# wasabipesto/nice

Hardware: AMD Instinct MI355X
Metric: numbers checked/sec per node, detailed+niceonly, 1e9 @ base 40 field (higher is better)
Workload: dtype u32; 1 GPU; extra-large: 1e+09 @ base 40, detailed + niceonly per step (benchmark.rs:60); base=40, field_start=1916284264916, field_size=1000000000, mode=both, niceonly_chunking=reference client (1e6 * clamp(ceil(size/1e11),1,1000)), parallelism=strong1, pipelined=True, pipeline_depth=2, full=False, probe_lib=False, gpu_max_hw_queues=4, gpu_max_hw_queues_exported=4

## Files before the change

### include/nice_hip.h

```cpp
#ifndef NICE_HIP_H
#define NICE_HIP_H

#include <stddef.h>
#include <stdint.h>

#ifdef __cplusplus
extern "C" {
#endif

#define NICE_OK 0
#define NICE_ERR_INVALID 1
#define NICE_ERR_HIP 2
#define NICE_ERR_CAPACITY 3
#define NICE_ERR_NO_DEVICE 4
#define NICE_ERR_MSD_OVERFLOW 5
#define NICE_ERR_BUSY 6

typedef struct {
    uint64_t number_lo;
    uint64_t number_hi;
    uint32_t num_uniques;
    uint32_t reserved;
} nice_number;

typedef struct nice_ctx nice_ctx;

int nice_ctx_create(const int *devices, int n_devices, nice_ctx **out);
void nice_ctx_destroy(nice_ctx *ctx);
int nice_ctx_synchronize(nice_ctx *ctx);
int nice_device_count(int *out);
const char *nice_last_error(void);

int nice_process_range_detailed(nice_ctx *ctx, uint64_t start_lo, uint64_t start_hi,
                                uint64_t end_lo, uint64_t end_hi, uint32_t base,
                                uint64_t *hist, nice_number *out, size_t cap, size_t *n_out);

#define NICE_FILTER_REFERENCE 0
#define NICE_FILTER_SOUND 1
#define NICE_MSD_FLOOR_ADAPTIVE UINT64_MAX
#define NICE_MSD_AUTO 0
#define NICE_MSD_HOST 1
#define NICE_MSD_DEVICE 2
typedef struct {
    uint64_t msd_floor;
    uint64_t chunk_size;
    int32_t threads;
    uint32_t stride_k;
    int32_t msd_where;
    uint32_t deal_stride;
    uint32_t deal_offset;
    uint32_t filter;
} nice_niceonly_opts;

typedef struct {
    uint64_t ranges;
    uint64_t range_numbers;
    uint64_t candidates;
    uint32_t launches;
    uint32_t square_ok;
    double msd_seconds;
    double total_seconds;
    uint64_t msd_floor;
    uint32_t msd_threads;
    uint32_t reruns;
} nice_niceonly_stats;

double nice_adaptive_floor_step(double floor, double msd_seconds, double total_seconds);
int nice_adaptive_floor(double *floor, uint32_t *warmup);

int nice_process_range_niceonly(nice_ctx *ctx, uint64_t start_lo, uint64_t start_hi,
                                uint64_t end_lo, uint64_t end_hi, uint32_t base,
                                nice_number *out, size_t cap, size_t *n_out);
int nice_process_range_niceonly_ex(nice_ctx *ctx, uint64_t start_lo, uint64_t start_hi,
                                   uint64_t end_lo, uint64_t end_hi, uint32_t base,
                                   const nice_niceonly_opts *opts, nice_number *out,
                                   size_t cap, size_t *n_out, nice_niceonly_stats *stats);
uint64_t nice_niceonly_prefix_rejected(void);

int nice_validate_detailed(uint32_t base, uint64_t size_lo, uint64_t size_hi, const uint64_t *hist,
                           const nice_number *list, size_t n);

int nice_cpu_process_range_detailed(uint64_t start_lo, uint64_t start_hi, uint64_t end_lo,
                                    uint64_t end_hi, uint32_t base, int32_t threads,
                                    uint64_t *hist, nice_number *out, size_t cap, size_t *n_out);
int nice_cpu_process_range_niceonly(uint64_t start_lo, uint64_t start_hi, uint64_t end_lo,
                                    uint64_t end_hi, uint32_t base, uint32_t stride_k,
                                    int32_t threads, nice_number *out, size_t cap, size_t *n_out);
int nice_cpu_process_range_niceonly_ex(uint64_t start_lo, uint64_t start_hi, uint64_t end_lo,
                                       uint64_t end_hi, uint32_t base, uint32_t stride_k,
                                       int32_t threads, uint32_t filter, nice_number *out, size_t cap,
                                       size_t *n_out);

int nice_detailed_submit(nice_ctx *ctx, uint64_t start_lo, uint64_t start_hi, uint64_t end_lo,
                         uint64_t end_hi, uint32_t base, int *ticket);
int nice_detailed_collect(nice_ctx *ctx, int ticket, uint64_t *hist, nice_number *out, size_t cap,
                          size_t *n_out);
int nice_niceonly_submit(nice_ctx *ctx, uint64_t start_lo, uint64_t start_hi, uint64_t end_lo,
                         uint64_t end_hi, uint32_t base, const nice_niceonly_opts *opts, int *ticket);
int nice_niceonly_collect(nice_ctx *ctx, int ticket, nice_number *out, size_t cap, size_t *n_out,
                          nice_niceonly_stats *stats);

typedef struct {
    double kernel_ms;
    uint32_t launches;
    uint32_t fd_kernel;
    uint64_t numbers;
    uint32_t sib_lanes;
    uint32_t sib_stride;
} nice_kernel_stats;
int nice_last_kernel_stats(nice_ctx *ctx, int device_index, nice_kernel_stats *out);
int nice_ctx_set_kernel_timing(nice_ctx *ctx, int enable);

uint32_t nice_host_threads(void);
int nice_debug_force_sib_stride(uint32_t L);
int nice_debug_fd_window(uint32_t base, uint32_t *w0, uint32_t *w);
int nice_debug_set_near_miss_cutoff(uint32_t base, uint32_t cutoff);
int nice_debug_set_nice_min(uint32_t base, uint32_t nice_min);
uint32_t nice_debug_cgroup_cpus(const char *root, const char *cgroup_path);
int nice_base_range(uint32_t base, uint64_t *start_lo, uint64_t *start_hi, uint64_t *end_lo,
                    uint64_t *end_hi);
uint32_t nice_near_miss_cutoff(uint32_t base);
uint64_t nice_gpu_batch_size(void);
uint64_t nice_processing_chunk_size(void);
int nice_gpu_supports_base(uint32_t base);
int nice_fd_kernel_base(uint32_t base);
int nice_niceonly_fast_base(uint32_t base);

int nice_msd_valid_ranges(uint64_t start_lo, uint64_t start_hi, uint64_t end_lo,
                          uint64_t end_hi, uint32_t base, uint64_t floor_size, uint64_t *out,
                          size_t cap, size_t *n_out);
int nice_msd_valid_ranges_ex(uint64_t start_lo, uint64_t start_hi, uint64_t end_lo,
                             uint64_t end_hi, uint32_t base, uint64_t floor_size, uint32_t filter,
                             uint64_t *out, size_t cap, size_t *n_out);
int nice_msd_skippable(uint64_t start_lo, uint64_t start_hi, uint64_t end_lo, uint64_t end_hi,
                       uint32_t base);
int nice_stride_table(uint32_t base, uint32_t k, uint64_t *modulus, uint32_t *residues,
                      size_t cap, size_t *n_out);

int nice_check_is_nice_inrange(uint32_t base, uint64_t n_lo, uint64_t n_hi);
int nice_check_unique_inrange(uint32_t base, uint64_t n_lo, uint64_t n_hi);
int nice_check_msd_skippable_inrange(uint32_t base, uint64_t start_lo, uint64_t start_hi,
                                     uint64_t end_lo, uint64_t end_hi);
int nice_check_prefix_reject_inrange(uint32_t base, uint64_t start_lo, uint64_t start_hi,
                                     uint64_t end_lo, uint64_t end_hi, uint64_t n_lo, uint64_t n_hi);
int nice_fd_segment_cuts(uint32_t base, uint64_t *out, size_t cap, size_t *n_out);

#define NICE_RANGES_PER_RANGE 0
#define NICE_RANGES_SUM 1
int nice_process_ranges_detailed(nice_ctx *ctx, uint32_t base, const uint64_t *bounds,
                                 size_t n_ranges, uint32_t flags, uint64_t *hist,
                                 nice_number *out, uint32_t *out_range, size_t cap,
                                 size_t *n_out);
typedef struct {
    uint32_t launches;
    uint32_t fallback_ranges;
    uint64_t numbers;
    double kernel_ms;
} nice_ranges_stats;
int nice_last_ranges_stats(nice_ctx *ctx, nice_ranges_stats *out);
int nice_cpu_process_ranges_detailed(uint32_t base, const uint64_t *bounds, size_t n_ranges,
                                     uint32_t flags, int32_t threads, uint64_t *hist,
                                     nice_number *out, uint32_t *out_range, size_t cap,
                                     size_t *n_out);
int nice_debug_ranges_plan(uint32_t base, const uint64_t *bounds, size_t n_ranges,
                           uint64_t *units, size_t cap, size_t *n_out);

int nice_debug_unique_counts(nice_ctx *ctx, const uint64_t *n_pairs, uint32_t count,
                             uint32_t base, uint32_t *out);
int nice_debug_is_nice(nice_ctx *ctx, const uint64_t *n_pairs, uint32_t count, uint32_t base,
                       uint32_t *out);
int nice_debug_unique_fast(nice_ctx *ctx, const uint64_t *n_pairs, uint32_t count, uint32_t base,
                           uint32_t *out);
int nice_debug_cube_count(nice_ctx *ctx, const uint64_t *n_pairs, uint32_t count, uint32_t base,
                          uint32_t *out);

#ifdef __cplusplus
}
#endif
#endif
```

### nice_amd/_lib.py

```python
from __future__ import annotations

import ctypes
import os
import subprocess

_HERE = os.path.dirname(os.path.abspath(__file__))
LIB_PATH = os.environ.get("NICE_LIB_PATH") or os.path.join(_HERE, "libnice_hip.so")

NICE_OK = 0
NICE_ERR_INVALID = 1
NICE_ERR_HIP = 2
NICE_ERR_CAPACITY = 3
NICE_ERR_NO_DEVICE = 4
NICE_ERR_MSD_OVERFLOW = 5
NICE_ERR_BUSY = 6
NICE_MSD_FLOOR_ADAPTIVE = (1 << 64) - 1
NICE_FILTER_REFERENCE = 0
NICE_FILTER_SOUND = 1
NICE_RANGES_PER_RANGE = 0
NICE_RANGES_SUM = 1

EXPORTS = (
    "nice_ctx_create", "nice_ctx_destroy", "nice_ctx_synchronize", "nice_device_count", "nice_last_error",
    "nice_process_range_detailed", "nice_process_range_niceonly",
    "nice_process_range_niceonly_ex", "nice_last_kernel_stats", "nice_base_range",
    "nice_near_miss_cutoff", "nice_gpu_batch_size", "nice_processing_chunk_size",
    "nice_gpu_supports_base", "nice_fd_kernel_base", "nice_niceonly_fast_base", "nice_msd_valid_ranges",
    "nice_msd_skippable", "nice_stride_table", "nice_debug_unique_counts",
    "nice_debug_is_nice", "nice_debug_unique_fast", "nice_check_is_nice_inrange", "nice_check_unique_inrange", "nice_check_msd_skippable_inrange",
    "nice_fd_segment_cuts", "nice_validate_detailed", "nice_detailed_submit",
    "nice_detailed_collect", "nice_niceonly_submit", "nice_niceonly_collect",
    "nice_cpu_process_range_detailed", "nice_cpu_process_range_niceonly",
    "nice_adaptive_floor_step", "nice_adaptive_floor", "nice_ctx_set_kernel_timing",
    "nice_host_threads", "nice_debug_cgroup_cpus", "nice_debug_force_sib_stride",
    "nice_niceonly_prefix_rejected", "nice_msd_valid_ranges_ex", "nice_cpu_process_range_niceonly_ex",
    "nice_check_prefix_reject_inrange",
    "nice_process_ranges_detailed", "nice_last_ranges_stats", "nice_cpu_process_ranges_detailed",
    "nice_debug_ranges_plan", "nice_debug_set_near_miss_cutoff", "nice_debug_fd_window",
    "nice_debug_set_nice_min", "nice_debug_cube_count",
)


class NiceLibraryError(RuntimeError):
    pass


class NiceError(RuntimeError):
    def __init__(self, code: int, msg: str):
        super().__init__(f"[{code}] {msg}")
        self.code = code


class nice_number(ctypes.Structure):
    _fields_ = [("number_lo", ctypes.c_uint64), ("number_hi", ctypes.c_uint64),
                ("num_uniques", ctypes.c_uint32), ("reserved", ctypes.c_uint32)]


class nice_niceonly_opts(ctypes.Structure):
    _fields_ = [("msd_floor", ctypes.c_uint64), ("chunk_size", ctypes.c_uint64),
                ("threads", ctypes.c_int32), ("stride_k", ctypes.c_uint32),
                ("msd_where", ctypes.c_int32), ("deal_stride", ctypes.c_uint32),
                ("deal_offset", ctypes.c_uint32), ("filter", ctypes.c_uint32)]


class nice_niceonly_stats(ctypes.Structure):
    _fields_ = [("ranges", ctypes.c_uint64), ("range_numbers", ctypes.c_uint64),
                ("candidates", ctypes.c_uint64), ("launches", ctypes.c_uint32),
                ("square_ok", ctypes.c_uint32), ("msd_seconds", ctypes.c_double),
                ("total_seconds", ctypes.c_double), ("msd_floor", ctypes.c_uint64),
                ("msd_threads", ctypes.c_uint32), ("reruns", ctypes.c_uint32)]


class nice_kernel_stats(ctypes.Structure):
    _fields_ = [("kernel_ms", ctypes.c_double), ("launches", ctypes.c_uint32),
                ("fd_kernel", ctypes.c_uint32), ("numbers", ctypes.c_uint64),
                ("sib_lanes", ctypes.c_uint32), ("sib_stride", ctypes.c_uint32)]


class nice_ranges_stats(ctypes.Structure):
    _fields_ = [("launches", ctypes.c_uint32), ("fallback_ranges", ctypes.c_uint32),
                ("numbers", ctypes.c_uint64), ("kernel_ms", ctypes.c_double)]


_lib = None


def build(force: bool = False) -> str:
    cmd = ["make", "-s", "-C", _HERE] + (["-B"] if force else [])
    subprocess.run(cmd, check=True)
    return LIB_PATH


def lib():
    global _lib
    if _lib is not None:
        return _lib
    if not os.path.exists(LIB_PATH):
        raise NiceLibraryError(
            f"{LIB_PATH} is missing: build it with `make -C nice_amd` "
            "(or __graft_entry__.build()); there is no CPU fallback")
    try:
        L = ctypes.CDLL(LIB_PATH)
    except OSError as e:
        raise NiceLibraryError(f"cannot load {LIB_PATH}: {e}") from e
    u64, u32, i32, sz = ctypes.c_uint64, ctypes.c_uint32, ctypes.c_int, ctypes.c_size_t
    P64, P32, PSZ = ctypes.POINTER(u64), ctypes.POINTER(u32), ctypes.POINTER(sz)
    PN = ctypes.POINTER(nice_number)
    vp = ctypes.c_void_p
    sig = {
        "nice_ctx_create": ([ctypes.POINTER(ctypes.c_int), i32, ctypes.POINTER(vp)], i32),
        "nice_ctx_destroy": ([vp], None),
        "nice_ctx_synchronize": ([vp], i32),
        "nice_device_count": ([ctypes.POINTER(ctypes.c_int)], i32),
        "nice_last_error": ([], ctypes.c_char_p),
        "nice_process_range_detailed": ([vp, u64, u64, u64, u64, u32, P64, PN, sz, PSZ], i32),
        "nice_process_range_niceonly": ([vp, u64, u64, u64, u64, u32, PN, sz, PSZ], i32),
        "nice_process_range_niceonly_ex": ([vp, u64, u64, u64, u64, u32,
                                            ctypes.POINTER(nice_niceonly_opts), PN, sz, PSZ,
                                            ctypes.POINTER(nice_niceonly_stats)], i32),
        "nice_last_kernel_stats": ([vp, i32, ctypes.POINTER(nice_kernel_stats)], i32),
        "nice_ctx_set_kernel_timing": ([vp, i32], i32),
        "nice_base_range": ([u32, P64, P64, P64, P64], i32),
        "nice_near_miss_cutoff": ([u32], u32),
        "nice_gpu_batch_size": ([], u64),
        "nice_processing_chunk_size": ([], u64),
        "nice_gpu_supports_base": ([u32], i32),
        "nice_fd_kernel_base": ([u32], i32),
        "nice_niceonly_fast_base": ([u32], i32),
        "nice_msd_valid_ranges": ([u64, u64, u64, u64, u32, u64, P64, sz, PSZ], i32),
        "nice_msd_valid_ranges_ex": ([u64, u64, u64, u64, u32, u64, u32, P64, sz, PSZ], i32),
        "nice_msd_skippable": ([u64, u64, u64, u64, u32], i32),
        "nice_stride_table": ([u32, u32, P64, P32, sz, PSZ], i32),
        "nice_debug_unique_counts": ([vp, P64, u32, u32, P32], i32),
        "nice_debug_is_nice": ([vp, P64, u32, u32, P32], i32),
        "nice_debug_unique_fast": ([vp, P64, u32, u32, P32], i32),
        "nice_check_is_nice_inrange": ([u32, u64, u64], i32),
        "nice_check_unique_inrange": ([u32, u64, u64], i32),
        "nice_check_msd_skippable_inrange": ([u32, u64, u64, u64, u64], i32),
        "nice_check_prefix_reject_inrange": ([u32, u64, u64, u64, u64, u64, u64], i32),
        "nice_fd_segment_cuts": ([u32, P64, sz, PSZ], i32),
        "nice_validate_detailed": ([u32, u64, u64, P64, PN, sz], i32),
        "nice_detailed_submit": ([vp, u64, u64, u64, u64, u32, ctypes.POINTER(i32)], i32),
        "nice_detailed_collect": ([vp, i32, P64, PN, sz, PSZ], i32),
        "nice_niceonly_submit": ([vp, u64, u64, u64, u64, u32, ctypes.POINTER(nice_niceonly_opts),
                                  ctypes.POINTER(i32)], i32),
        "nice_niceonly_collect": ([vp, i32, PN, sz, PSZ, ctypes.POINTER(nice_niceonly_stats)], i32),
        "nice_cpu_process_range_detailed": ([u64, u64, u64, u64, u32, i32, P64, PN, sz, PSZ], i32),
        "nice_cpu_process_range_niceonly": ([u64, u64, u64, u64, u32, u32, i32, PN, sz, PSZ], i32),
        "nice_cpu_process_range_niceonly_ex": ([u64, u64, u64, u64, u32, u32, i32, u32, PN, sz, PSZ], i32),
        "nice_niceonly_prefix_rejected": ([], u64),
        "nice_adaptive_floor_step": ([ctypes.c_double, ctypes.c_double, ctypes.c_double], ctypes.c_double),
        "nice_adaptive_floor": ([ctypes.POINTER(ctypes.c_double), P32], i32),
        "nice_host_threads": ([], u32),
        "nice_debug_cgroup_cpus": ([ctypes.c_char_p, ctypes.c_char_p], u32),
        "nice_debug_force_sib_stride": ([u32], i32),
        "nice_debug_set_near_miss_cutoff": ([u32, u32], i32),
        "nice_debug_fd_window": ([u32, P32, P32], i32),
        "nice_debug_set_nice_min": ([u32, u32], i32),
        "nice_debug_cube_count": ([vp, P64, u32, u32, P32], i32),
        "nice_process_ranges_detailed": ([vp, u32, P64, sz, u32, P64, PN, P32, sz, PSZ], i32),
        "nice_last_ranges_stats": ([vp, ctypes.POINTER(nice_ranges_stats)], i32),
        "nice_cpu_process_ranges_detailed": ([u32, P64, sz, u32, i32, P64, PN, P32, sz, PSZ], i32),
        "nice_debug_ranges_plan": ([u32, P64, sz, P64, sz, PSZ], i32),
    }
    for name, (args, res) in sig.items():
        fn = getattr(L, name)
        fn.argtypes = args
        fn.restype = res
    _lib = L
    return L


def check(rc: int):
    if rc != NICE_OK:
        msg = lib().nice_last_error()
        raise NiceError(rc, msg.decode() if msg else "")
```

### nice_amd/api.py

```python
from __future__ import annotations

import array
import ctypes
import threading
from dataclasses import dataclass
from typing import List, Optional, Sequence, Tuple

from . import _lib
from ._lib import check, lib
from .types import (DataToClient, DataToServer, FieldResults, FieldSize, NiceNumberSimple,
                    UniquesDistributionSimple)

CLIENT_VERSION = "3.2.15-mi355x"
MASK64 = (1 << 64) - 1


def _split(n: int):
    if n < 0 or n >> 128:
        raise ValueError("value must fit in u128")
    return n & MASK64, n >> 64


def _const(name):
    try:
        return int(getattr(lib(), name)())
    except _lib.NiceLibraryError:
        return None


GPU_BATCH_SIZE = 50_000_000
PROCESSING_CHUNK_SIZE = 1_000_000


def get_base_range_u128(base: int) -> Optional[FieldSize]:
    a, b, c, d = (ctypes.c_uint64() for _ in range(4))
    rc = lib().nice_base_range(base, a, b, c, d)
    if rc < 0:
        raise OverflowError(f"base {base}: range does not fit in u128")
    if rc == 0:
        return None
    return FieldSize(a.value | (b.value << 64), c.value | (d.value << 64))


def get_near_miss_cutoff(base: int) -> int:
    return int(lib().nice_near_miss_cutoff(base))


def gpu_supports_base(base: int) -> bool:
    return bool(lib().nice_gpu_supports_base(base))


def niceonly_fast_base(base: int) -> bool:
    return bool(lib().nice_niceonly_fast_base(base))


@dataclass
class StrideTable:
    base: int
    k: int
    modulus: int
    valid_residues: List[int]

    @classmethod
    def new(cls, base: int, k: int) -> "StrideTable":
        m = ctypes.c_uint64()
        n = ctypes.c_size_t()
        check(lib().nice_stride_table(base, k, m, None, 0, n))
        buf = (ctypes.c_uint32 * max(n.value, 1))()
        check(lib().nice_stride_table(base, k, m, buf, n.value, n))
        return cls(base, k, m.value, list(buf[: n.value]))


def get_valid_ranges(range_: FieldSize, base: int, floor_size: int = 250,
                     filter: str = "reference") -> List[FieldSize]:
    s, e = range_.range_start, range_.range_end
    f = _FILTERS[filter]
    n = ctypes.c_size_t()
    rc = lib().nice_msd_valid_ranges_ex(*_split(s), *_split(e), base, floor_size, f, None, 0, n)
    if rc not in (_lib.NICE_OK, _lib.NICE_ERR_CAPACITY):
        check(rc)
    buf = (ctypes.c_uint64 * (4 * max(n.value, 1)))()
    check(lib().nice_msd_valid_ranges_ex(*_split(s), *_split(e), base, floor_size, f, buf, n.value, n))
    return [FieldSize(buf[4 * i] | (buf[4 * i + 1] << 64), buf[4 * i + 2] | (buf[4 * i + 3] << 64))
            for i in range(n.value)]


def has_duplicate_msd_prefix(range_: FieldSize, base: int) -> bool:
    rc = lib().nice_msd_skippable(*_split(range_.range_start), *_split(range_.range_end), base)
    if rc < 0 or rc > 1:
        check(rc)
    return bool(rc)


@dataclass
class NiceonlyStats:
    ranges: int
    range_numbers: int
    candidates: int
    launches: int
    msd_seconds: float
    total_seconds: float
    square_ok: int = 0
    msd_floor: int = 0
    msd_threads: int = 0
    reruns: int = 0
    prefix_rejected: int = 0


_FILTERS = {"reference": _lib.NICE_FILTER_REFERENCE, "sound": _lib.NICE_FILTER_SOUND}


def _stats(st) -> NiceonlyStats:
    return NiceonlyStats(st.ranges, st.range_numbers, st.candidates, st.launches,
                         st.msd_seconds, st.total_seconds, st.square_ok, st.msd_floor,
                         st.msd_threads, st.reruns, int(lib().nice_niceonly_prefix_rejected()))


def host_threads() -> int:
    return int(lib().nice_host_threads())


def adaptive_floor_step(floor: float, msd_seconds: float, total_seconds: float) -> float:
    return lib().nice_adaptive_floor_step(floor, msd_seconds, total_seconds)


def adaptive_floor() -> Tuple[float, int]:
    f, w = ctypes.c_double(), ctypes.c_uint32()
    check(lib().nice_adaptive_floor(f, w))
    return f.value, w.value


@dataclass
class KernelStats:
    kernel_ms: float
    launches: int
    fd_kernel: bool
    numbers: int
    sib_lanes: int = 0
    sib_stride: int = 0


@dataclass
class RangesStats:
    launches: int
    fallback_ranges: int
    numbers: int
    kernel_ms: float


def _pack_ranges(ranges):
    pairs = [(r.range_start, r.range_end) if isinstance(r, FieldSize) else (int(r[0]), int(r[1]))
             for r in ranges]
    if any(s < 0 or e < 0 or s >> 128 or e >> 128 for s, e in pairs):
        raise ValueError("value must fit in u128")
    flat = array.array("Q", [x for s, e in pairs for x in (s & MASK64, s >> 64, e & MASK64, e >> 64)])
    if not pairs:
        flat = array.array("Q", [0, 0, 0, 0])
    return (ctypes.c_uint64 * len(flat)).from_buffer_copy(flat), len(pairs)


def _ranges_result(hist, nb, nrows, out, idx, n):
    full = memoryview(hist).cast("B").cast("Q").tolist()
    rows = [full[i * nb:(i + 1) * nb] for i in range(nrows)]
    return rows, [(out[i].number_lo | (out[i].number_hi << 64), out[i].num_uniques, idx[i])
                  for i in range(n)]


class GpuContext:

    def __init__(self, devices: Sequence[int] | int = 0):
        if isinstance(devices, int):
            devices = [devices]
        arr = (ctypes.c_int * len(devices))(*devices)
        h = ctypes.c_void_p()
        check(lib().nice_ctx_create(arr, len(devices), ctypes.byref(h)))
        self._h = h
        self.devices = list(devices)
        self._out = None
        self._out_cap = 0
        self._hist = {}

    @classmethod
    def new(cls, device_ordinal: int = 0) -> "GpuContext":
        return cls([device_ordinal])

    def close(self):
        if getattr(self, "_h", None):
            lib().nice_ctx_destroy(self._h)
            self._h = None

    def synchronize(self):
        check(lib().nice_ctx_synchronize(self._h))

    def __del__(self):
        try:
            self.close()
        except Exception:
            pass

    def _out_buf(self, cap):
        if cap > self._out_cap:
            self._out = (_lib.nice_number * cap)()
            self._out_cap = cap
        return self._out

    def set_kernel_timing(self, enable: bool):
        check(lib().nice_ctx_set_kernel_timing(self._h, 1 if enable else 0))

    def kernel_stats(self, device_index: int = 0) -> KernelStats:
        s = _lib.nice_kernel_stats()
        check(lib().nice_last_kernel_stats(self._h, device_index, s))
        return KernelStats(s.kernel_ms, s.launches, bool(s.fd_kernel), s.numbers, s.sib_lanes, s.sib_stride)

    def detailed_raw(self, start: int, end: int, base: int, cap: int = 0):
        hist = self._hist.get(base)
        if hist is None:
            hist = self._hist[base] = (ctypes.c_uint64 * (base + 1))()
        cap = max(cap, self._out_cap, 1024)
        while True:
            out = self._out_buf(cap)
            n = ctypes.c_size_t()
            rc = lib().nice_process_range_detailed(self._h, *_split(start), *_split(end), base,
                                                   hist, out, cap, n)
            if rc == _lib.NICE_ERR_CAPACITY and n.value > cap:
                cap = n.value
                continue
            check(rc)
            lst = [(out[i].number_lo | (out[i].number_hi << 64), out[i].num_uniques)
                   for i in range(n.value)]
            return list(hist), lst

    def detailed_submit(self, start: int, end: int, base: int) -> int:
        t = ctypes.c_int()
        check(lib().nice_detailed_submit(self._h, *_split(start), *_split(end), base, t))
        return t.value

    def detailed_collect(self, ticket: int, base: int, cap: int = 0):
        hist = self._hist.get(base)
        if hist is None:
            hist = self._hist[base] = (ctypes.c_uint64 * (base + 1))()
        cap = max(cap, self._out_cap, 1024)
        while True:
            out = self._out_buf(cap)
            n = ctypes.c_size_t()
            rc = lib().nice_detailed_collect(self._h, ticket, hist, out, cap, n)
            if rc == _lib.NICE_ERR_CAPACITY and n.value > cap:
                cap = n.value
                continue
            check(rc)
            return list(hist), [(out[i].number_lo | (out[i].number_hi << 64), out[i].num_uniques)
                                for i in range(n.value)]

    def detailed_ranges(self, ranges, base: int, sum: bool = False, cap: int = 0):
        bounds, n_ranges = _pack_ranges(ranges)
        nb = base + 1
        hist = (ctypes.c_uint64 * (nb * (1 if sum else max(n_ranges, 1))))()
        flags = _lib.NICE_RANGES_SUM if sum else _lib.NICE_RANGES_PER_RANGE
        cap = max(cap, 1024)
        while True:
            out, idx, n = _cpu_out(cap), (ctypes.c_uint32 * cap)(), ctypes.c_size_t()
            rc = lib().nice_process_ranges_detailed(self._h, base, bounds, n_ranges, flags, hist, out, idx,
                                                    cap, n)
            if rc == _lib.NICE_ERR_CAPACITY and n.value > cap:
                cap = n.value
                continue
            check(rc)
            return _ranges_result(hist, nb, 1 if sum else n_ranges, out, idx, n.value)

    def ranges_stats(self) -> "RangesStats":
        s = _lib.nice_ranges_stats()
        check(lib().nice_last_ranges_stats(self._h, s))
        return RangesStats(s.launches, s.fallback_ranges, s.numbers, s.kernel_ms)

    def niceonly_raw(self, start: int, end: int, base: int, msd_floor: int = 0,
                     chunk_size: int = 0, threads: int = 0, stride_k: int = 0,
                     msd_where: str = "auto", cap: int = 0, deal_stride: int = 0,
                     deal_offset: int = 0, filter: str = "reference"):
        opts = self._nice_opts(msd_floor, chunk_size, threads, stride_k, msd_where, deal_stride,
                               deal_offset, filter)
        st = _lib.nice_niceonly_stats()
        cap = max(cap, self._out_cap, 1024)
        while True:
            out = self._out_buf(cap)
            n = ctypes.c_size_t()
            rc = lib().nice_process_range_niceonly_ex(self._h, *_split(start), *_split(end), base,
                                                      opts, out, cap, n, st)
            if rc == _lib.NICE_ERR_CAPACITY and n.value > cap:
                cap = n.value
                continue
            check(rc)
            lst = [out[i].number_lo | (out[i].number_hi << 64) for i in range(n.value)]
            return lst, _stats(st)

    @staticmethod
    def _nice_opts(msd_floor=0, chunk_size=0, threads=0, stride_k=0, msd_where="auto",
                   deal_stride=0, deal_offset=0, filter="reference"):
        where = {"auto": 0, "host": 1, "device": 2}[msd_where]
        if filter not in _FILTERS:
            raise ValueError(f"filter must be one of {sorted(_FILTERS)}")
        if msd_floor == "adaptive":
            msd_floor = _lib.NICE_MSD_FLOOR_ADAPTIVE
        return _lib.nice_niceonly_opts(msd_floor, chunk_size, threads, stride_k, where,
                                       deal_stride, deal_offset, _FILTERS[filter])

    def niceonly_submit(self, start: int, end: int, base: int, **opts) -> int:
        t = ctypes.c_int()
        check(lib().nice_niceonly_submit(self._h, *_split(start), *_split(end), base,
                                         self._nice_opts(**opts), t))
        return t.value

    def niceonly_collect(self, ticket: int, cap: int = 0):
        st = _lib.nice_niceonly_stats()
        cap = max(cap, self._out_cap, 1024)
        while True:
            out = self._out_buf(cap)
            n = ctypes.c_size_t()
            rc = lib().nice_niceonly_collect(self._h, ticket, out, cap, n, st)
            if rc == _lib.NICE_ERR_CAPACITY and n.value > cap:
                cap = n.value
                continue
            check(rc)
            return ([out[i].number_lo | (out[i].number_hi << 64) for i in range(n.value)],
                    _stats(st))

    def both_raw(self, det_range, nice_range, base: int, **nice_opts):
        det = self.detailed_raw(*det_range, base) if det_range else (None, [])
        nice = self.niceonly_raw(*nice_range, base, **nice_opts) if nice_range else ([], None)
        return det, nice

    def debug_unique_counts(self, ns: Sequence[int], base: int) -> List[int]:
        arr = (ctypes.c_uint64 * (2 * max(len(ns), 1)))()
        for i, n in enumerate(ns):
            arr[2 * i], arr[2 * i + 1] = _split(n)
        out = (ctypes.c_uint32 * max(len(ns), 1))()
        check(lib().nice_debug_unique_counts(self._h, arr, len(ns), base, out))
        return list(out[: len(ns)])

    def debug_unique_fast(self, ns: Sequence[int], base: int) -> List[int]:
        arr = (ctypes.c_uint64 * (2 * max(len(ns), 1)))()
        for i, n in enumerate(ns):
            arr[2 * i], arr[2 * i + 1] = _split(n)
        out = (ctypes.c_uint32 * max(len(ns), 1))()
        check(lib().nice_debug_unique_fast(self._h, arr, len(ns), base, out))
        return list(out[: len(ns)])

    def debug_cube_count(self, ns: Sequence[int], base: int) -> List[int]:
        arr = (ctypes.c_uint64 * (2 * max(len(ns), 1)))()
        for i, n in enumerate(ns):
            arr[2 * i], arr[2 * i + 1] = _split(n)
        out = (ctypes.c_uint32 * max(len(ns), 1))()
        check(lib().nice_debug_cube_count(self._h, arr, len(ns), base, out))
        return list(out[: len(ns)])

    def debug_is_nice(self, ns: Sequence[int], base: int) -> List[bool]:
        arr = (ctypes.c_uint64 * (2 * max(len(ns), 1)))()
        for i, n in enumerate(ns):
            arr[2 * i], arr[2 * i + 1] = _split(n)
        out = (ctypes.c_uint32 * max(len(ns), 1))()
        check(lib().nice_debug_is_nice(self._h, arr, len(ns), base, out))
        return [bool(x) for x in out[: len(ns)]]


class BothModes:

    def __init__(self, device: int = 0, det_ctx: Optional[GpuContext] = None,
                 nice_ctx: Optional[GpuContext] = None):
        self.det = det_ctx if det_ctx is not None else GpuContext([device])
        self.nice = nice_ctx if nice_ctx is not None else GpuContext([device])
        self._own_nice = nice_ctx is None
        self._go = threading.Event()
        self._done = threading.Event()
        self._job = None
        self._res = None
        self._closed = False
        self._thread = threading.Thread(target=self._serve, name="nice-niceonly", daemon=True)
        self._thread.start()

    def _serve(self):
        while True:
            self._go.wait()
            self._go.clear()
            if self._closed:
                return
            args, kw = self._job
            try:
                self._res = (True, self.nice.niceonly_raw(*args, **kw))
            except BaseException as e:
                self._res = (False, e)
            self._done.set()

    def kernel_stats(self, device_index: int = 0) -> KernelStats:
        return self.det.kernel_stats(device_index)

    def detailed_raw(self, *a, **kw):
        return self.det.detailed_raw(*a, **kw)

    def niceonly_raw(self, *a, **kw):
        return self.nice.niceonly_raw(*a, **kw)

    def both_raw(self, det_range, nice_range, base: int, **nice_opts):
        if self._closed:
            raise RuntimeError("BothModes is closed")
        if not nice_range:
            return (self.det.detailed_raw(*det_range, base) if det_range else (None, [])), ([], None)
        self._job = ((*nice_range, base), nice_opts)
        self._done.clear()
        self._go.set()
        try:
            det = self.det.detailed_raw(*det_range, base) if det_range else (None, [])
        finally:
            self._done.wait()
        ok, nice = self._res
        self._res = None
        if not ok:
            raise nice
        return det, nice

    def close(self):
        if not self._closed:
            self._closed = True
            self._go.set()
            self._thread.join()
            if self._own_nice:
                self.nice.close()


def process_range_detailed_gpu(ctx: GpuContext, range_: FieldSize, base: int) -> FieldResults:
    hist, lst = ctx.detailed_raw(range_.range_start, range_.range_end, base)
    return FieldResults(
        distribution=[UniquesDistributionSimple(i, hist[i]) for i in range(1, base + 1)],
        nice_numbers=[NiceNumberSimple(n, u) for n, u in lst])


def process_range_niceonly_gpu(ctx: GpuContext, range_: FieldSize, base: int,
                               **opts) -> FieldResults:
    lst, _ = ctx.niceonly_raw(range_.range_start, range_.range_end, base, **opts)
    return FieldResults(distribution=[], nice_numbers=[NiceNumberSimple(n, base) for n in lst])


def process_detailed_gpu(ctx: GpuContext, claim: DataToClient, username: str) -> DataToServer:
    r = process_range_detailed_gpu(ctx, claim.field(), claim.base)
    return DataToServer(claim.claim_id, username, CLIENT_VERSION, r.distribution, r.nice_numbers)


def process_niceonly_gpu(ctx: GpuContext, claim: DataToClient, username: str) -> DataToServer:
    r = process_range_niceonly_gpu(ctx, claim.field(), claim.base)
    return DataToServer(claim.claim_id, username, CLIENT_VERSION, None, r.nice_numbers)


_default_ctx: Optional[GpuContext] = None
_default_lock = threading.Lock()


def default_context() -> GpuContext:
    global _default_ctx
    with _default_lock:
        if _default_ctx is None:
            _default_ctx = GpuContext(0)
        return _default_ctx


def process_range_detailed(range_: FieldSize, base: int) -> FieldResults:
    return process_range_detailed_gpu(default_context(), range_, base)


def process_range_niceonly(range_: FieldSize, base: int,
                           stride_table: Optional[StrideTable] = None) -> FieldResults:
    k = stride_table.k if stride_table is not None else 2
    size = range_.range_size
    return process_range_niceonly_gpu(default_context(), range_, base, stride_k=k,
                                      chunk_size=min(size, (1 << 64) - 1))


def _cpu_out(cap: int):
    return (_lib.nice_number * max(cap, 1))()


def process_range_detailed_cpu(range_: FieldSize, base: int, threads: int = 1) -> FieldResults:
    hist = (ctypes.c_uint64 * (base + 1))()
    cap = 1024
    while True:
        out, n = _cpu_out(cap), ctypes.c_size_t()
        rc = lib().nice_cpu_process_range_detailed(*_split(range_.range_start), *_split(range_.range_end),
                                                    base, threads, hist, out, cap, n)
        if rc == _lib.NICE_ERR_CAPACITY and n.value > cap:
            cap = n.value
            continue
        check(rc)
        break
    return FieldResults(
        distribution=[UniquesDistributionSimple(i, hist[i]) for i in range(1, base + 1)],
        nice_numbers=[NiceNumberSimple(out[i].number_lo | (out[i].number_hi << 64), out[i].num_uniques)
                      for i in range(n.value)])


def detailed_ranges_cpu(ranges, base: int, sum: bool = False, threads: int = 1):
    bounds, n_ranges = _pack_ranges(ranges)
    nb = base + 1
    hist = (ctypes.c_uint64 * (nb * (1 if sum else max(n_ranges, 1))))()
    flags = _lib.NICE_RANGES_SUM if sum else _lib.NICE_RANGES_PER_RANGE
    cap = 1024
    while True:
        out, idx, n = _cpu_out(cap), (ctypes.c_uint32 * cap)(), ctypes.c_size_t()
        rc = lib().nice_cpu_process_ranges_detailed(base, bounds, n_ranges, flags, threads, hist, out, idx,
                                                     cap, n)
        if rc == _lib.NICE_ERR_CAPACITY and n.value > cap:
            cap = n.value
            continue
        check(rc)
        return _ranges_result(hist, nb, 1 if sum else n_ranges, out, idx, n.value)


def _ranges_field_results(rows, lst, base: int) -> List[FieldResults]:
    per = [[] for _ in rows]
    for n, u, i in lst:
        per[i].append(NiceNumberSimple(n, u))
    return [FieldResults(distribution=[UniquesDistributionSimple(i, row[i]) for i in range(1, base + 1)],
                         nice_numbers=nn) for row, nn in zip(rows, per)]


def process_ranges_detailed_gpu(ctx: GpuContext, ranges, base: int) -> List[FieldResults]:
    return _ranges_field_results(*ctx.detailed_ranges(ranges, base), base)


def process_ranges_detailed_cpu(ranges, base: int, threads: int = 1) -> List[FieldResults]:
    return _ranges_field_results(*detailed_ranges_cpu(ranges, base, threads=threads), base)


def process_range_niceonly_cpu(range_: FieldSize, base: int,
                               stride_table: Optional[StrideTable] = None,
                               threads: int = 1, filter: str = "reference") -> FieldResults:
    k = stride_table.k if stride_table is not None else 2
    cap = 256
    while True:
        out, n = _cpu_out(cap), ctypes.c_size_t()
        rc = lib().nice_cpu_process_range_niceonly_ex(*_split(range_.range_start), *_split(range_.range_end),
                                                       base, k, threads, _FILTERS[filter], out, cap, n)
        if rc == _lib.NICE_ERR_CAPACITY and n.value > cap:
            cap = n.value
            continue
        check(rc)
        break
    return FieldResults(distribution=[], nice_numbers=[
        NiceNumberSimple(out[i].number_lo | (out[i].number_hi << 64), base) for i in range(n.value)])
```

### nice_amd/csrc/abi_detailed.cpp

```cpp
#include <cstring>

#include "abi_internal.hpp"

using namespace nice::abi;
using nice::u128;

namespace {

inline bool spin_wait() { return nice::probe_knob("NICE_SPIN", 1) != 0; }

int enqueue_detailed(Device &d, Slot &sl, u128 s, u128 e, uint32_t base, bool *finished) {
    nice::DetailedLaunch p{};
    p.base = base;
    p.cutoff = effective_cutoff(base);
    p.hist = sl.d_state;
    p.out = nice::NumOut{sl.det.n, sl.det.u, sl.d_count, sl.det.cap};
    p.launches = &sl.launches;
    p.sib = sl.sib;
    for (const Slot &o : d.slot)
        if (&o != &sl && o.inflight) p.overlapped = 1;
    *finished = false;
    uint32_t tag = 0;
    auto launch = [&](u128 a, u128 b, bool fd) -> int {
        if (a >= b) return NICE_OK;
        u128 cnt = b - a;
        while (cnt) {
            uint64_t c = cnt > ((u128)1 << 62) ? (1ull << 62) : (uint64_t)cnt;
            p.start_lo = lo64(a);
            p.start_hi = hi64(a);
            p.count = c;
            const bool last = a + c == e;
            p.fin = last && fd ? nice::FieldFinish{sl.d_fin, sl.d_done, sl.seq, tag}
                               : nice::FieldFinish{nullptr, nullptr, 0, 0};
            if (nice::probe_set("NICE_FD2_NOFIN")) p.fin = nice::FieldFinish{nullptr, nullptr, 0, 0};
            hipError_t err = fd ? nice::launch_detailed_fd2(p, d.num_cus, sl.stream)
                                : nice::launch_detailed_generic(p, d.num_cus, sl.stream);
            if (!fd) sl.launches++;
            if (err != hipSuccess)
                return fail(NICE_ERR_HIP, std::string("detailed launch: ") + hipGetErrorString(err));
            if (last) {
                *finished = fd && p.fin.out_mapped;
                sl.tag = *finished ? p.fin.tag : 0u;
                sl.tag_words = base + 1;
            }
            a += c;
            cnt -= c;
        }
        return NICE_OK;
    };
    u128 rs = 0, re = 0;
    const bool fd_base = nice::fd2_supported(base);
    const bool fd = fd_base && nice::base_range_cached(base, rs, re) == 1;
    const bool small_fd = fd && s >= rs && e <= re && e - s < 20000000;
    p.hist_copies = small_fd ? 16 : nice::kHistCopies;
    if (small_fd && !nice::probe_set("NICE_FD2_UNTAGGED")) tag = (uint32_t)sl.seq | 0x80000000u;
    sl.tag = 0;
    if (!fd) return launch(s, e, false);
    int rc;
    if ((rc = launch(s, std::min(e, rs), false))) return rc;
    if ((rc = launch(std::max(s, rs), std::min(e, re), true))) return rc;
    return launch(std::max(s, re), e, false);
}

bool published(const Slot &sl) {
    if (!sl.tag) return __atomic_load_n(&sl.h_fin[nice::kFinSeq], __ATOMIC_ACQUIRE) == sl.seq;
    if ((uint32_t)(__atomic_load_n(&sl.h_fin[nice::kFinCount], __ATOMIC_ACQUIRE) >> 32) != sl.tag) return false;
    for (uint32_t b = 0; b < sl.tag_words; b++)
        if ((uint32_t)(__atomic_load_n(&sl.h_fin[b], __ATOMIC_ACQUIRE) >> 32) != sl.tag) return false;
    return true;
}

int wait_field(Slot &sl) {
    if (!sl.fin_seq || !spin_wait()) {
        const hipError_t q = field_sync(sl);
        if (q != hipSuccess) return fail(NICE_ERR_HIP, std::string("detailed field: ") + hipGetErrorString(q));
        return NICE_OK;
    }
    for (uint32_t i = 1;; i++) {
        if (published(sl)) return NICE_OK;
        if ((i & 4095) == 0 || i > kSpinPolls) {
            const hipError_t q = field_query(sl);
            if (q == hipSuccess) {
                if (published(sl)) return NICE_OK;
                return fail(NICE_ERR_HIP, "detailed field completed without publishing its results");
            }
            if (q != hipErrorNotReady) return fail(NICE_ERR_HIP, std::string("detailed field: ") + hipGetErrorString(q));
        }
        backoff(i);
    }
}

int enqueue_detailed_shard(Device &d, Slot &sl, u128 s, u128 e, uint32_t base, bool timing) {
    HIPCHK(hipSetDevice(d.id));
    if (d.stats_slot == (int)(&sl - d.slot)) {
        int rc = resolve_stats(d);
        if (rc) return rc;
    }
    sl.seq++;
    sl.launches = 0;
    sl.sib[0] = sl.sib[1] = 0;
    if (sl.dirty) HIPCHK(hipMemsetAsync(sl.d_state, 0, kStateBytes, sl.stream));
    sl.dirty = true;
    sl.timed = timing;
    sl.marked = false;
    if (timing) HIPCHK(hipEventRecord(sl.ev0, sl.stream));
    bool finished = false;
    int rc = enqueue_detailed(d, sl, s, e, base, &finished);
    if (rc) return rc;
    sl.inflight = true;
    if (timing) HIPCHK(hipEventRecord(sl.ev1, sl.stream));
    sl.fin_seq = finished;
    if (!finished) {
        HIPCHK(nice::launch_detailed_finish(sl.d_state, sl.d_count, sl.d_fin, sl.stream));
        HIPCHK(hipEventRecord(sl.ev_done, sl.stream));
    } else if (!timing && !sl.own_stream) {
        HIPCHK(hipEventRecord(sl.ev_done, sl.stream));
        sl.marked = true;
    }
    return NICE_OK;
}

int detailed_submit(nice_ctx *ctx, std::unique_lock<std::mutex> &lock, u128 s, u128 e, uint32_t base,
                    bool wait, int *ticket) {
    int t = -1;
    if (int rc = acquire_slot(ctx, lock, ctx->det, ctx->det_next, wait, "detailed", &t)) return rc;
    DetJob &job = ctx->det[t];
    const size_t nd = ctx->devs.size();
    const u128 size = e - s;
    job.bounds.assign(nd + 1, 0);
    for (size_t i = 0; i <= nd; i++) job.bounds[i] = s + size / nd * i + std::min<u128>(i, size % nd);
    for (size_t i = 0; i < nd; i++) {
        if (job.bounds[i] >= job.bounds[i + 1]) continue;
        int rc = enqueue_detailed_shard(ctx->devs[i], ctx->devs[i].slot[t], job.bounds[i], job.bounds[i + 1], base,
                                        ctx->timing);
        if (rc) return rc;
    }
    job.active = true;
    job.collected = false;
    job.owner = std::this_thread::get_id();
    job.s = s;
    job.e = e;
    job.base = base;
    ctx->det_next = (t + 1) % slots_used();
    *ticket = t;
    return NICE_OK;
}

int detailed_submit_args(nice_ctx *ctx, uint64_t start_lo, uint64_t start_hi, uint64_t end_lo, uint64_t end_hi,
                         uint32_t base, bool wait, int *ticket) {
    if (!ctx || !ticket) return fail(NICE_ERR_INVALID, "null argument");
    if (base < 2 || base > 128) return fail(NICE_ERR_INVALID, "base must be in 2..=128");
    const u128 s = mk(start_lo, start_hi), e = mk(end_lo, end_hi);
    if (s >= e)
        return fail(NICE_ERR_INVALID, "Range has invalid bounds, range_start must be < range_end");
    std::unique_lock<std::mutex> lock(ctx->mu);
    return detailed_submit(ctx, lock, s, e, base, wait, ticket);
}

uint32_t shard_finished(Device &d, Slot &sl, int t) {
    sl.dirty = false;
    sl.inflight = false;
    d.stats_slot = t;
    d.last.launches = sl.launches;
    d.last.sib_lanes = sl.sib[0];
    d.last.sib_stride = sl.sib[1];
    return (uint32_t)sl.h_fin[nice::kFinCount];
}

int recompute_listed(nice_ctx *ctx, const DetJob &job, const std::vector<size_t> &off) {
    const size_t nd = ctx->devs.size();
    std::vector<std::vector<uint32_t>> u(nd);
    std::vector<std::vector<uint64_t>> pairs(nd);
    struct Drain {
        nice_ctx *ctx;
        std::vector<char> q;
        ~Drain() {
            for (size_t j = 0; j < q.size(); j++)
                if (q[j]) {
                    (void)hipSetDevice(ctx->devs[j].id);
                    (void)hipStreamSynchronize(ctx->devs[j].aux);
                }
        }
    } drain{ctx, std::vector<char>(nd, 0)};
    for (size_t i = 0; i < nd; i++) {
        const size_t n = off[i + 1] - off[i];
        if (!n) continue;
        Device &d = ctx->devs[i];
        HIPCHK(hipSetDevice(d.id));
        if (!d.aux) HIPCHK(hipStreamCreateWithFlags(&d.aux, hipStreamNonBlocking));
        pairs[i].resize(2 * n);
        for (size_t q = 0; q < n; q++) {
            pairs[i][2 * q] = lo64(job.all[off[i] + q].n);
            pairs[i][2 * q + 1] = hi64(job.all[off[i] + q].n);
        }
        if (d.chk_cap < n) {
            const size_t c = std::max<size_t>(n, 4096);
            if (int rc = grow_device(d.chk_n, d.chk_cap, c, c * 16)) return rc;
            if (int rc = grow_device(d.chk_u, d.chk_cap, c, c * 4)) return rc;
        }
        u[i].resize(n);
        drain.q[i] = 1;
        hipError_t err = hipMemcpyAsync(d.chk_n, pairs[i].data(), n * 16, hipMemcpyHostToDevice, d.aux);
        if (err == hipSuccess) err = nice::launch_unique_counts(d.chk_n, (uint32_t)n, job.base, d.chk_u, d.aux);
        if (err == hipSuccess) err = hipMemcpyAsync(u[i].data(), d.chk_u, n * 4, hipMemcpyDeviceToHost, d.aux);
        if (err != hipSuccess) return fail(NICE_ERR_HIP, std::string("self-check: ") + hipGetErrorString(err));
    }
    for (size_t i = 0; i < nd; i++) {
        if (u[i].empty()) continue;
        Device &d = ctx->devs[i];
        HIPCHK(hipSetDevice(d.id));
        const hipError_t err = hipStreamSynchronize(d.aux);
        drain.q[i] = 0;
        if (err != hipSuccess) return fail(NICE_ERR_HIP, std::string("self-check: ") + hipGetErrorString(err));
        for (size_t q = 0; q < u[i].size(); q++)
            if (u[i][q] != job.all[off[i] + q].u)
                return fail(NICE_ERR_HIP, "self-check: unique count of a listed number does not recompute");
    }
    return NICE_OK;
}

int detailed_gather(nice_ctx *ctx, DetJob &job, int t) {
    const uint32_t base = job.base;
    const size_t nd = ctx->devs.size();
    job.total.assign(base + 1, 0);
    job.all.clear();
    std::vector<size_t> off(nd + 1, 0);
    for (size_t i = 0; i < nd; i++) {
        off[i] = job.all.size();
        Device &d = ctx->devs[i];
        Slot &sl = d.slot[t];
        d.last = nice_kernel_stats{};
        d.stats_slot = -1;
        if (job.bounds[i] >= job.bounds[i + 1]) continue;
        HIPCHK(hipSetDevice(d.id));
        int rc = wait_field(sl);
        if (rc) return rc;
        d.last.numbers = (uint64_t)(job.bounds[i + 1] - job.bounds[i]);
        d.last.fd_kernel = nice::fd2_supported(base) ? 1u : 0u;
        uint32_t cnt = shard_finished(d, sl, t);
        if (cnt > sl.det.cap) {
            rc = ensure_listbuf(d, sl.det, cnt, true);
            if (!rc) rc = enqueue_detailed_shard(d, sl, job.bounds[i], job.bounds[i + 1], base, sl.timed);
            if (!rc) rc = wait_field(sl);
            if (rc) return rc;
            cnt = shard_finished(d, sl, t);
            if (cnt > sl.det.cap) return fail(NICE_ERR_HIP, "near-miss list overflow after resize");
        }
        for (uint32_t b = 0; b <= base; b++) job.total[b] += sl.tag ? (uint32_t)sl.h_fin[b] : sl.h_fin[b];
        if (cnt) {
            HIPCHK(field_sync(sl));
            std::vector<uint64_t> nbuf((size_t)cnt * 2);
            std::vector<uint32_t> ubuf(cnt);
            HIPCHK(hipMemcpy(nbuf.data(), sl.det.n, (size_t)cnt * 16, hipMemcpyDeviceToHost));
            HIPCHK(hipMemcpy(ubuf.data(), sl.det.u, (size_t)cnt * 4, hipMemcpyDeviceToHost));
            for (uint32_t q = 0; q < cnt; q++) job.all.push_back({mk(nbuf[2 * q], nbuf[2 * q + 1]), ubuf[q]});
        }
    }
    off[nd] = job.all.size();
    int rc = validate_detailed(base, effective_cutoff(base), job.e - job.s, job.total.data(), job.all.size(),
                               [&](size_t i) { return job.all[i]; });
    if (!rc && !job.all.empty()) rc = recompute_listed(ctx, job, off);
    if (rc) return rc;
    std::sort(job.all.begin(), job.all.end(), [](const Entry &a, const Entry &b) { return a.n < b.n; });
    return NICE_OK;
}

void detailed_drop(nice_ctx *ctx, int t) {
    ctx->det[t].active = false;
    for (auto &d : ctx->devs) d.slot[t].dirty = true, d.slot[t].inflight = false;
}

int detailed_collect(nice_ctx *ctx, int t, uint64_t *hist, nice_number *out, size_t cap, size_t *n_out) {
    if (t < 0 || t >= kSlots || !ctx->det[t].active)
        return fail(NICE_ERR_INVALID, "no detailed field in flight under this ticket");
    DetJob &job = ctx->det[t];
    if (!job.collected) {
        int rc = detailed_gather(ctx, job, t);
        if (rc) {
            detailed_drop(ctx, t);
            return rc;
        }
        job.collected = true;
    }
    std::memcpy(hist, job.total.data(), (job.base + 1) * 8);
    int rc = emit_list(job.all, out, cap, n_out);
    if (rc == NICE_ERR_CAPACITY) return rc;
    job.active = false;
    job.all = {};
    return rc;
}

int detailed_collect_locked(nice_ctx *ctx, int ticket, uint64_t *hist, nice_number *out, size_t cap,
                            size_t *n_out) {
    std::unique_lock<std::mutex> lock(ctx->mu);
    if (ticket < 0 || ticket >= kSlots || !ctx->det[ticket].active)
        return fail(NICE_ERR_INVALID, "no detailed field in flight under this ticket");
    DetJob &job = ctx->det[ticket];
    if (job.waiting) return fail(NICE_ERR_INVALID, "another thread is collecting this detailed field");
    if (!job.collected) {
        job.waiting = true;
        lock.unlock();
        int rc = NICE_OK;
        for (size_t i = 0; i < ctx->devs.size() && !rc; i++) {
            if (job.bounds[i] >= job.bounds[i + 1]) continue;
            const hipError_t err = hipSetDevice(ctx->devs[i].id);
            rc = err != hipSuccess ? fail(NICE_ERR_HIP, hipGetErrorString(err)) : wait_field(ctx->devs[i].slot[ticket]);
        }
        lock.lock();
        job.waiting = false;
        if (rc) {
            detailed_drop(ctx, ticket);
            return rc;
        }
    }
    return detailed_collect(ctx, ticket, hist, out, cap, n_out);
}

}

extern "C" {

int nice_detailed_submit(nice_ctx *ctx, uint64_t start_lo, uint64_t start_hi, uint64_t end_lo,
                         uint64_t end_hi, uint32_t base, int *ticket) {
    return detailed_submit_args(ctx, start_lo, start_hi, end_lo, end_hi, base, false, ticket);
}

int nice_detailed_collect(nice_ctx *ctx, int ticket, uint64_t *hist, nice_number *out, size_t cap,
                          size_t *n_out) {
    if (!ctx || !hist) return fail(NICE_ERR_INVALID, "null argument");
    const int rc = detailed_collect_locked(ctx, ticket, hist, out, cap, n_out);
    ctx->freed.notify_all();
    return rc;
}

int nice_process_range_detailed(nice_ctx *ctx, uint64_t start_lo, uint64_t start_hi,
                                uint64_t end_lo, uint64_t end_hi, uint32_t base, uint64_t *hist,
                                nice_number *out, size_t cap, size_t *n_out) {
    int t = -1;
    int rc = detailed_submit_args(ctx, start_lo, start_hi, end_lo, end_hi, base, true, &t);
    if (rc) return rc;
    rc = nice_detailed_collect(ctx, t, hist, out, cap, n_out);
    if (rc == NICE_ERR_CAPACITY) {
        {
            std::lock_guard<std::mutex> lock(ctx->mu);
            ctx->det[t].active = false;
            ctx->det[t].all = {};
        }
        ctx->freed.notify_all();
    }
    return rc;
}

}
```

### nice_amd/csrc/abi_hooks.cpp

```cpp
#include "abi_internal.hpp"
#include "niceonly_bases.h"
#include "radix_fast.hpp"

using namespace nice::abi;
using nice::u128;

namespace {

#define NICE_FAST_BASES(X) NICE_NICEONLY_BASES(X)

bool fast_base_range(uint32_t base, u128 &rs, u128 &re) {
    return nice::niceonly_fast_base(base) && nice::base_range_cached(base, rs, re) == 1;
}

template <int B>
int prefix_reject_host(u128 s, u128 l, u128 n) {
    constexpr int MW = nice::Radix<B>::MW;
    uint32_t pm[MW] = {}, low[MW];
    const uint32_t multi = l > s ? 1u : 0u;
    if (multi && nice::msd_prefix_masks<B>(lo64(s), hi64(s), lo64(l), hi64(l), pm))
        for (int w = 0; w < MW; w++) pm[w] = ~0u;
    const uint32_t dup = nice::low_digit_mask(B, (uint32_t)(n % ((uint32_t)B * B)), low, MW);
    return nice::prefix_rejects<MW>(pm, multi, low, dup) ? 1 : 0;
}

template <class Launch>
int debug_per_n(nice_ctx *ctx, const uint64_t *n_pairs, uint32_t count, uint32_t *out, Launch launch) {
    if (count == 0) return NICE_OK;
    Device &d = ctx->devs[0];
    HIPCHK(hipSetDevice(d.id));
    uint64_t *dn;
    uint32_t *du;
    HIPCHK(hipMalloc(&dn, (size_t)count * 16));
    HIPCHK(hipMalloc(&du, (size_t)count * 4));
    HIPCHK(hipMemcpy(dn, n_pairs, (size_t)count * 16, hipMemcpyHostToDevice));
    HIPCHK(launch(dn, du, d.slot[0].stream));
    HIPCHK(hipStreamSynchronize(d.slot[0].stream));
    HIPCHK(hipMemcpy(out, du, (size_t)count * 4, hipMemcpyDeviceToHost));
    HIPCHK(hipFree(dn));
    HIPCHK(hipFree(du));
    return NICE_OK;
}

}

extern "C" {

int nice_validate_detailed(uint32_t base, uint64_t size_lo, uint64_t size_hi, const uint64_t *hist,
                           const nice_number *list, size_t n) {
    if (base < 2 || base > 128 || !hist || (n && !list)) return fail(NICE_ERR_INVALID, "bad args");
    const int rc = validate_detailed(base, nice::near_miss_cutoff(base), mk(size_lo, size_hi), hist, n, [&](size_t i) {
        return Entry{mk(list[i].number_lo, list[i].number_hi), list[i].num_uniques};
    });
    return rc ? NICE_ERR_INVALID : NICE_OK;
}

int nice_debug_unique_counts(nice_ctx *ctx, const uint64_t *n_pairs, uint32_t count,
                             uint32_t base, uint32_t *out) {
    if (!ctx || base < 2 || base > 128) return fail(NICE_ERR_INVALID, "bad args");
    return debug_per_n(ctx, n_pairs, count, out, [&](const uint64_t *dn, uint32_t *du, hipStream_t s) {
        return nice::launch_unique_counts(dn, count, base, du, s);
    });
}

int nice_debug_is_nice(nice_ctx *ctx, const uint64_t *n_pairs, uint32_t count, uint32_t base,
                       uint32_t *out) {
    if (!ctx || base < 2 || base > 128) return fail(NICE_ERR_INVALID, "bad args");
    return debug_per_n(ctx, n_pairs, count, out, [&](const uint64_t *dn, uint32_t *du, hipStream_t s) {
        return nice::launch_is_nice(dn, count, base, du, s);
    });
}

int nice_debug_unique_fast(nice_ctx *ctx, const uint64_t *n_pairs, uint32_t count, uint32_t base,
                           uint32_t *out) {
    u128 rs, re;
    if (!ctx || !fast_base_range(base, rs, re))
        return fail(NICE_ERR_INVALID, "base without a niceonly fast path");
    for (uint32_t i = 0; i < count; i++) {
        const u128 n = mk(n_pairs[2 * i], n_pairs[2 * i + 1]);
        if (n < rs || n >= re) return fail(NICE_ERR_INVALID, "n outside the base's valid range");
    }
    return debug_per_n(ctx, n_pairs, count, out, [&](const uint64_t *dn, uint32_t *du, hipStream_t s) {
        return nice::launch_unique_fast(dn, count, base, du, s);
    });
}

int nice_debug_cube_count(nice_ctx *ctx, const uint64_t *n_pairs, uint32_t count, uint32_t base,
                          uint32_t *out) {
    u128 rs, re;
    if (!ctx || !fast_base_range(base, rs, re))
        return fail(NICE_ERR_INVALID, "base without a niceonly fast path");
    for (uint32_t i = 0; i < count; i++) {
        const u128 n = mk(n_pairs[2 * i], n_pairs[2 * i + 1]);
        if (n < rs || n >= re) return fail(NICE_ERR_INVALID, "n outside the base's valid range");
    }
    return debug_per_n(ctx, n_pairs, count, out, [&](const uint64_t *dn, uint32_t *du, hipStream_t s) {
        return nice::launch_cube_count(dn, count, base, du, s);
    });
}

int nice_check_is_nice_inrange(uint32_t base, uint64_t lo, uint64_t hi) {
    u128 rs, re;
    const u128 n = mk(lo, hi);
    if (!fast_base_range(base, rs, re) || n < rs || n >= re)
        return fail(NICE_ERR_INVALID, "n outside the base's valid range (or base without a niceonly fast path)");
    switch (base) {
#define X(b) case b: return nice::is_nice_fast<b>(lo, hi) ? 1 : 0;
        NICE_FAST_BASES(X)
#undef X
    default: return NICE_ERR_INVALID;
    }
}

int nice_check_unique_inrange(uint32_t base, uint64_t lo, uint64_t hi) {
    u128 rs, re;
    const u128 n = mk(lo, hi);
    if (!fast_base_range(base, rs, re) || n < rs || n >= re)
        return fail(NICE_ERR_INVALID, "n outside the base's valid range (or base without a niceonly fast path)");
    switch (base) {
#define X(b) case b: return (int)nice::unique_fast<b>(lo, hi);
        NICE_FAST_BASES(X)
#undef X
    default: return NICE_ERR_INVALID;
    }
}

int nice_check_msd_skippable_inrange(uint32_t base, uint64_t slo, uint64_t shi, uint64_t elo,
                                     uint64_t ehi) {
    u128 rs, re;
    const u128 s = mk(slo, shi), e = mk(elo, ehi);
    if (!fast_base_range(base, rs, re) || s < rs || e > re || s >= e)
        return fail(NICE_ERR_INVALID, "range outside the base's valid range (or base without a niceonly fast path)");
    if (e - s == 1) return 0;
    const u128 l = e - 1;
    const uint64_t llo = lo64(l), lhi = hi64(l);
    switch (base) {
#define X(b) case b: return nice::msd_skippable_fast<b>(slo, shi, llo, lhi) ? 1 : 0;
        NICE_FAST_BASES(X)
#undef X
    default: return NICE_ERR_INVALID;
    }
}

int nice_check_prefix_reject_inrange(uint32_t base, uint64_t slo, uint64_t shi, uint64_t elo, uint64_t ehi,
                                     uint64_t nlo, uint64_t nhi) {
    u128 rs, re;
    const u128 s = mk(slo, shi), e = mk(elo, ehi), n = mk(nlo, nhi);
    if (!fast_base_range(base, rs, re) || s < rs || e > re || n < s || n >= e)
        return fail(NICE_ERR_INVALID, "leaf or n outside the base's valid range (or base without a niceonly fast path)");
    switch (base) {
#define X(b) case b: return prefix_reject_host<b>(s, e - 1, n);
        NICE_FAST_BASES(X)
#undef X
    default: return NICE_ERR_INVALID;
    }
}

int nice_fd_segment_cuts(uint32_t base, uint64_t *out, size_t cap, size_t *n_out) {
    std::vector<u128> c(8);
    const size_t n = nice::fd2_cuts(base, c.data(), c.size());
    for (size_t i = 0; i < n && i < cap; i++) {
        out[2 * i] = lo64(c[i]);
        out[2 * i + 1] = hi64(c[i]);
    }
    if (n_out) *n_out = n;
    return NICE_OK;
}

int nice_msd_skippable(uint64_t slo, uint64_t shi, uint64_t elo, uint64_t ehi, uint32_t base) {
    if (base < 2 || base > 128 || mk(slo, shi) >= mk(elo, ehi)) return fail(NICE_ERR_INVALID, "bad args");
    return nice::make_msd(base)->skippable(mk(slo, shi), mk(elo, ehi)) ? 1 : 0;
}

int nice_msd_valid_ranges(uint64_t slo, uint64_t shi, uint64_t elo, uint64_t ehi, uint32_t base,
                          uint64_t floor_size, uint64_t *out, size_t cap, size_t *n_out) {
    return nice_msd_valid_ranges_ex(slo, shi, elo, ehi, base, floor_size, NICE_FILTER_REFERENCE, out, cap, n_out);
}

int nice_msd_valid_ranges_ex(uint64_t slo, uint64_t shi, uint64_t elo, uint64_t ehi, uint32_t base,
                             uint64_t floor_size, uint32_t filter, uint64_t *out, size_t cap, size_t *n_out) {
    if (base < 2 || base > 128 || mk(slo, shi) >= mk(elo, ehi) || filter > NICE_FILTER_SOUND)
        return fail(NICE_ERR_INVALID, "bad args");
    std::vector<std::pair<u128, u128>> rs;
    nice::make_msd(base)->ranges(mk(slo, shi), mk(elo, ehi), floor_size, rs, filter == NICE_FILTER_SOUND);
    size_t n = rs.size();
    for (size_t i = 0; i < n && i < cap; i++) {
        out[4 * i] = lo64(rs[i].first);
        out[4 * i + 1] = hi64(rs[i].first);
        out[4 * i + 2] = lo64(rs[i].second);
        out[4 * i + 3] = hi64(rs[i].second);
    }
    *n_out = n;
    return n > cap ? fail(NICE_ERR_CAPACITY, "range list exceeds capacity") : NICE_OK;
}

int nice_stride_table(uint32_t base, uint32_t k, uint64_t *modulus, uint32_t *residues,
                      size_t cap, size_t *n_out) {
    if (base < 3 || base > 128 || k > 3) return fail(NICE_ERR_INVALID, "bad args");
    auto t = g_stride.get(base, k);
    *modulus = t->modulus;
    *n_out = t->residues.size();
    for (size_t i = 0; i < std::min(cap, t->residues.size()); i++) residues[i] = t->residues[i];
    return t->residues.size() > cap && residues ? fail(NICE_ERR_CAPACITY, "capacity") : NICE_OK;
}

int nice_debug_force_sib_stride(uint32_t L) {
    if (L && (L % 2 == 0 || L > 255))
        return fail(NICE_ERR_INVALID, "sibling lane stride must be odd and <= 255 (0: the production pick)");
    nice::fd2_force_sib_stride(L);
    return NICE_OK;
}

int nice_debug_fd_window(uint32_t base, uint32_t *w0, uint32_t *w) {
    if (!w0 || !w) return fail(NICE_ERR_INVALID, "null argument");
    if (!nice::fd2_window(base, w0, w)) return fail(NICE_ERR_INVALID, "base has no FD kernel");
    return NICE_OK;
}

int nice_debug_set_near_miss_cutoff(uint32_t base, uint32_t cutoff) {
    uint32_t w0 = 0, w = 0;
    if (!nice::fd2_window(base, &w0, &w)) return fail(NICE_ERR_INVALID, "base has no FD kernel");
    if (cutoff && (cutoff + 1 < w0 + w || cutoff >= base))
        return fail(NICE_ERR_INVALID, "cutoff must be 0 (production) or in [" + std::to_string(w0 + w - 1) + ", " +
                                          std::to_string(base - 1) + "]");
    g_cutoff_override[base].store(cutoff, std::memory_order_relaxed);
    return NICE_OK;
}

int nice_debug_set_nice_min(uint32_t base, uint32_t nice_min) {
    if (!nice::niceonly_fast_base(base)) return fail(NICE_ERR_INVALID, "base without a niceonly fast path");
    if (nice_min > base)
        return fail(NICE_ERR_INVALID, "nice_min must be 0 (production) or in [1, " + std::to_string(base) + "]");
    g_nice_min_override[base].store(nice_min, std::memory_order_relaxed);
    return NICE_OK;
}

}
```

### nice_amd/csrc/abi_internal.hpp

```cpp
#pragma once

#include <hip/hip_runtime.h>
#include <sched.h>

#include <algorithm>
#include <atomic>
#include <chrono>
#include <condition_variable>
#include <map>
#include <memory>
#include <mutex>
#include <string>
#include <thread>
#include <vector>

#include "../../include/nice_hip.h"
#include "host_math.hpp"
#include "host_parallel.hpp"
#include "kernels.h"
#include "probe.hpp"

namespace nice {
namespace abi __attribute__((visibility("hidden"))) {

constexpr size_t kStateBytes = (size_t)kHistCopies * kHistBins * 8 + (1 + kDoneWords) * 4;
constexpr int kSlots = 3;

constexpr uint32_t kInitialListCap = 1u << 20;
constexpr uint32_t kNiceCap = 1u << 16;

inline int slots_used() { return std::max(1, std::min(kSlots, (int)probe_knob("NICE_SLOTS", kSlots))); }

int fail(int code, const std::string &msg);

#define HIPCHK(expr)                                                                    \
    do {                                                                                \
        hipError_t e_ = (expr);                                                         \
        if (e_ != hipSuccess)                                                           \
            return fail(NICE_ERR_HIP, std::string(#expr) + ": " + hipGetErrorString(e_)); \
    } while (0)

inline u128 mk(uint64_t lo, uint64_t hi) { return ((u128)hi << 64) | lo; }
inline uint64_t lo64(u128 v) { return (uint64_t)v; }
inline uint64_t hi64(u128 v) { return (uint64_t)(v >> 64); }

struct LeafBuf {
    Leaf *h = nullptr, *d = nullptr;
    uint32_t cap = 0;
    hipEvent_t done = nullptr;
    bool pending = false;
};

struct MsdBuf {
    MsdNode *q[2] = {nullptr, nullptr};
    ChunkNode *scratch = nullptr;
    void *wscratch = nullptr;
    size_t wscratch_bytes = 0;
    Leaf *leaves = nullptr;
    LeafMask *leaf_masks = nullptr;
    uint32_t *counters = nullptr;
    uint32_t q_cap = 0, leaf_cap = 0, mask_cap = 0;
    uint64_t scratch_nodes = 0;
    bool dirty = true;
};

struct ListBuf {
    uint64_t *n = nullptr;
    uint32_t *u = nullptr;
    uint32_t cap = 0;
};

struct Slot {
    hipStream_t stream = nullptr;
    bool own_stream = false, own_nstream = false;
    hipStream_t nstream = nullptr;
    uint64_t *d_state = nullptr;
    uint32_t *d_count = nullptr;
    uint32_t *d_done = nullptr;
    uint32_t *d_nice_count = nullptr;
    uint64_t *h_fin = nullptr;
    uint64_t *d_fin = nullptr;
    ListBuf det, nice;
    hipEvent_t ev0 = nullptr, ev1 = nullptr, ev_done = nullptr, nice_done = nullptr;
    hipEvent_t nt0 = nullptr, nt1 = nullptr;
    uint32_t *h_msd = nullptr;
    uint32_t *h_nice = nullptr;
    uint32_t *d_msd_mapped = nullptr, *d_nice_mapped = nullptr;
    uint32_t *d_nice_done = nullptr;
    bool dirty = true;
    bool inflight = false;
    bool timed = false;
    bool marked = false;
    uint64_t seq = 0;
    uint32_t launches = 0;
    uint32_t sib[2] = {0, 0};
    bool fin_seq = false;
    uint32_t tag = 0;
    uint32_t tag_words = 0;
    MsdBuf msd;
};

struct Device {
    int id = 0;
    int num_cus = 0;
    hipStream_t aux = nullptr;
    uint64_t *chk_n = nullptr;
    uint32_t *chk_u = nullptr;
    size_t chk_cap = 0;
    Slot slot[kSlots];
    std::map<uint32_t, uint32_t *> residues;
    std::map<uint32_t, uint32_t *> ranks;
    std::map<uint32_t, uint32_t *> lowtabs;
    LeafBuf desc[2];
    int desc_next = 0;
    nice_kernel_stats last{};
    int stats_slot = -1;
};

struct Entry {
    u128 n;
    uint32_t u;
};

struct DetJob {
    bool active = false, collected = false;
    bool waiting = false;
    std::thread::id owner;
    u128 s = 0, e = 0;
    uint32_t base = 0;
    std::vector<u128> bounds;
    std::vector<uint64_t> total;
    std::vector<Entry> all;
};
struct NiceJob {
    bool active = false, collected = false;
    bool waiting = false;
    std::thread::id owner;
    u128 s = 0, e = 0;
    uint32_t base = 0;
    nice_niceonly_opts opts{};
    bool has_opts = false;
    bool on_device = false;
    bool empty = false;
    std::vector<char> used;
    nice_niceonly_stats st{};
    std::chrono::steady_clock::time_point t0;
    std::vector<Entry> all;
    bool adapt = false;
    uint32_t reruns = 0;
    uint64_t rejected = 0;
    uint32_t nice_min = 0;
};

struct RangesDev {
    hipStream_t stream = nullptr;
    void *h_desc = nullptr, *d_desc = nullptr;
    size_t desc_cap = 0;
    uint64_t *d_rows = nullptr;
    size_t rows_cap = 0;
    uint32_t *d_count = nullptr;
    ListBuf list;
    uint32_t *chk_u = nullptr;
    uint32_t chk_cap = 0;
    hipEvent_t ev0 = nullptr, ev1 = nullptr;
};
struct RangesState {
    std::vector<RangesDev> dev;
    nice_ranges_stats stats{};
    bool kept = false;
    uint32_t base = 0, flags = 0;
    std::vector<uint64_t> bounds, hist;
    std::vector<Entry> list;
    std::vector<uint32_t> list_range;
};

}
}

struct nice_ctx {
    std::mutex ranges_mu;
    nice::abi::RangesState ranges;
    std::vector<nice::abi::Device> devs;
    std::mutex mu;
    std::condition_variable freed;
    bool timing = true;
    nice::abi::DetJob det[nice::abi::kSlots];
    nice::abi::NiceJob nice[nice::abi::kSlots];
    int det_next = 0, nice_next = 0;
    std::vector<std::thread::id> blocked;
};

namespace nice {
namespace abi __attribute__((visibility("hidden"))) {

template <class Job>
int free_slot(const Job *jobs, int next) {
    const int n = slots_used();
    for (int i = 0; i < n; i++) {
        const int t = (next + i) % n;
        if (!jobs[t].active) return t;
    }
    return -1;
}

template <class Job>
int acquire_slot(nice_ctx *ctx, std::unique_lock<std::mutex> &lock, const Job *jobs, int next, bool wait,
                 const char *mode, int *slot) {
    const std::thread::id me = std::this_thread::get_id();
    auto blocked = [&](std::thread::id id) {
        return id == me || std::find(ctx->blocked.begin(), ctx->blocked.end(), id) != ctx->blocked.end();
    };
    auto unblock = [&] {
        auto it = std::find(ctx->blocked.begin(), ctx->blocked.end(), me);
        if (it != ctx->blocked.end()) {
            ctx->blocked.erase(it);
            ctx->freed.notify_all();
        }
    };
    for (;;) {
        const int t = free_slot(jobs, next);
        if (t >= 0) {
            unblock();
            *slot = t;
            return NICE_OK;
        }
        bool freeable = false;
        for (int i = 0; i < slots_used(); i++)
            freeable |= jobs[i].active && (jobs[i].waiting || !blocked(jobs[i].owner));
        if (!wait || !freeable) {
            unblock();
            return fail(NICE_ERR_BUSY, std::string("three ") + mode +
                                           " fields already in flight on this context; collect one first");
        }
        if (std::find(ctx->blocked.begin(), ctx->blocked.end(), me) == ctx->blocked.end()) {
            ctx->blocked.push_back(me);
            ctx->freed.notify_all();
        }
        ctx->freed.wait(lock);
    }
}

template <class T, class C>
int grow_device(T *&p, C &cap, C new_cap, size_t bytes, hipStream_t drain = nullptr) {
    if (drain) HIPCHK(hipStreamSynchronize(drain));
    if (p) HIPCHK(hipFree(p));
    p = nullptr;
    cap = 0;
    HIPCHK(hipMalloc(&p, bytes));
    cap = new_cap;
    return NICE_OK;
}
template <class T, class C>
int grow_pinned(T *&p, C &cap, C new_cap, size_t bytes) {
    if (p) HIPCHK(hipHostFree(p));
    p = nullptr;
    cap = 0;
    HIPCHK(hipHostMalloc(&p, bytes, hipHostMallocDefault));
    cap = new_cap;
    return NICE_OK;
}

int ensure_listbuf(Device &d, ListBuf &l, uint32_t cap, bool with_u);

inline void put_entry(nice_number &o, const Entry &e) {
    o.number_lo = lo64(e.n);
    o.number_hi = hi64(e.n);
    o.num_uniques = e.u;
    o.reserved = 0;
}

int emit_list(std::vector<Entry> &all, nice_number *out, size_t cap, size_t *n_out);

inline std::atomic<uint32_t> g_cutoff_override[129];

inline uint32_t effective_cutoff(uint32_t base) {
    const uint32_t c = base <= 128 ? g_cutoff_override[base].load(std::memory_order_relaxed) : 0u;
    return c ? c : near_miss_cutoff(base);
}

inline std::atomic<uint32_t> g_nice_min_override[129];

template <class Get>
int validate_detailed(uint32_t base, uint32_t cutoff, u128 size, const uint64_t *hist, size_t n, Get get) {
    u128 sum = 0;
    for (uint32_t b = 0; b <= base; b++) sum += hist[b];
    if (sum != size)
        return fail(NICE_ERR_HIP, "self-check: distribution total does not equal the field size");
    std::vector<uint64_t> per(base + 1, 0);
    for (size_t i = 0; i < n; i++) {
        const uint32_t u = get(i).u;
        if (u <= cutoff || u > base)
            return fail(NICE_ERR_HIP, "self-check: listed number " + std::to_string(i) +
                                          " has num_uniques " + std::to_string(u) +
                                          " at or below the cutoff");
        per[u]++;
    }
    u128 above = 0;
    for (uint32_t u = cutoff + 1; u <= base; u++) {
        if (per[u] != hist[u])
            return fail(NICE_ERR_HIP, "self-check: " + std::to_string(per[u]) +
                                          " listed numbers with " + std::to_string(u) +
                                          " uniques, distribution claims " + std::to_string(hist[u]));
        above += hist[u];
    }
    if (above != (u128)n) return fail(NICE_ERR_HIP, "self-check: list length does not match the distribution");
    return NICE_OK;
}

struct StrideCache {
    std::mutex mu;
    std::map<std::pair<uint32_t, uint32_t>, std::shared_ptr<StrideTable>> tables;
    std::shared_ptr<StrideTable> get(uint32_t base, uint32_t k) {
        std::lock_guard<std::mutex> g(mu);
        auto key = std::make_pair(base, k);
        auto it = tables.find(key);
        if (it != tables.end()) return it->second;
        auto t = std::make_shared<StrideTable>(base, k);
        tables[key] = t;
        return t;
    }
};
inline StrideCache g_stride;

constexpr uint32_t kSpinPolls = 1u << 14, kYieldPolls = 1u << 11;

inline void backoff(uint32_t i) {
    if (i < kSpinPolls) {
        __builtin_ia32_pause();
    } else if (i < kSpinPolls + kYieldPolls) {
        sched_yield();
    } else {
        const uint32_t k = std::min<uint32_t>((i - kSpinPolls - kYieldPolls) / 8, 3);
        std::this_thread::sleep_for(std::chrono::microseconds(std::min(200u, 20u << (2 * k))));
    }
}

inline hipError_t sync_event(hipEvent_t ev) {
    for (uint32_t i = 0;; i++) {
        const hipError_t q = hipEventQuery(ev);
        if (q != hipErrorNotReady) return q;
        backoff(i);
    }
}

inline hipEvent_t done_event(const Slot &sl) {
    if (!sl.fin_seq) return sl.ev_done;
    return sl.timed ? sl.ev1 : (sl.marked ? sl.ev_done : nullptr);
}

inline hipError_t field_query(const Slot &sl) {
    const hipEvent_t ev = done_event(sl);
    return ev ? hipEventQuery(ev) : hipStreamQuery(sl.stream);
}

inline hipError_t field_sync(const Slot &sl) {
    for (uint32_t i = 0;; i++) {
        const hipError_t q = field_query(sl);
        if (q != hipErrorNotReady) return q;
        backoff(i);
    }
}

int resolve_stats(Device &d);

void ranges_dev_free(Device &d, RangesDev &r);

}
}
```

### nice_amd/csrc/fd2_cfg.hpp

```cpp
#pragma once

#include <algorithm>
#include <type_traits>

#include "layout.h"

namespace nice {
namespace fd2 {

constexpr int log2ceil(unsigned v) { int t = 0; while ((1u << t) < v) t++; return t; }
constexpr int ilog2(unsigned v) { int t = 0; while ((2u << t) <= v) t++; return t; }

constexpr bool split_exact(unsigned base, unsigned es, unsigned long long m) {
    for (unsigned v = 0; v < base * base; v++)
        if (((unsigned long long)es * v * m) >> 32 != v / base) return false;
    return true;
}


constexpr int window_w(int b) {
    return b == 40 ? 15 : b == 50 ? 18 : b == 80 ? 28 : b <= 45 ? 15 : b <= 61 ? 18 : b <= 70 ? 20 : 28;
}
constexpr int window_w0(int b) {
    switch (b) {
    case 40: return 18;
    case 42: return 19;
    case 43: return 20;
    case 44: case 45: case 47: return 21;
    case 48: return 22;
    case 49: return 23;
    case 50: return 21;
    case 52: return 24;
    case 53: return 25;
    case 54: case 55: return 26;
    case 57: return 27;
    case 58: return 28;
    case 59: case 60: return 29;
    case 62: case 63: return 30;
    case 64: return 31;
    case 65: return 32;
    case 67: return 33;
    case 68: return 34;
    case 80: return 33;
    default: return b * 61 / 100 - window_w(b) / 2;
    }
}

struct Digits {
    int d2, d3, dn;
};
constexpr Digits digits_of(int base) {
    const int k = base / 5, r5 = base % 5;
    return Digits{r5 == 0 ? 2 * k : (r5 == 4 ? 2 * k + 2 : 2 * k + 1),
                  r5 == 0 ? 3 * k : (r5 == 2 ? 3 * k + 1 : 3 * k + 2), r5 == 0 ? k : k + 1};
}

constexpr int tchunk_of(int base) { return base <= 45 ? 80 : (base <= 58 ? 160 : 240); }

constexpr int state_regs(int base) {
    const Digits d = digits_of(base);
    return (d.d2 + 1) / 2 + (d.d3 + 1) / 2 + 2 * ((d.dn + 1) / 2) + 1 + (base + 31) / 32;
}
constexpr int state_waves(int base) {
    const int r = state_regs(base);
    return r <= 31 ? 8 : (r <= 38 ? 6 : (r <= 46 ? 5 : 4));
}

constexpr bool fits64(unsigned base, int digits) {
    unsigned long long v = 1;
    for (int i = 0; i < digits; i++) {
        if (v > ~0ull / base) return false;
        v *= base;
    }
    return true;
}

constexpr int valu_limbs(int base) {
    switch (base) {
    case 43: case 44: case 45: case 48: case 50: case 54: case 55: return 1;
    case 53: case 58: case 65: return 2;
    case 67: case 68: case 80: return 256;
    case 59: case 63: case 64: return 1024 + 2;
    case 60: return 1024 + 17;
    case 62: return 1024 + 1;
    default: return 0;
    }
}

constexpr int valu_limbs_big(int base, int nd, int ne) {
    if (base == 40) return ne == 8 ? 2048 | 1 : 0;
    if (base == 50 || base == 53 || base == 60) return valu_limbs(base) | 2048;
    if ((base + 31) / 32 != 3) return valu_limbs(base);
    if (base == 80 && ne == 17) return 256 | 2048 | 4;
    return 256 | 2048 | 3;
}

constexpr int lds_bytes(int base, int wg) {
    const int mw = (base + 31) / 32, b2 = base * base;
    const bool split = mw == 3 && (valu_limbs(base) & 512) != 0;
    const int es = mw == 1 ? 4 : (mw == 2 || split ? 8 : 16);
    int t = 0;
    while ((1 << t) < b2) t++;
    const int ebt = es * ((1 << t) - b2);
    if (split) {
        const int a = (4 * (base + 1) + 15) / 16 * 16, h = (ebt / 2 + 15) / 16 * 16;
        const int t2 = a > h ? a : h;
        const int tb0 = (t2 + 4 * b2 + 15) / 16 * 16, tbe = (ebt + 15) / 16 * 16;
        const int tb = tb0 > tbe ? tb0 : tbe;
        return (tb + b2 * es + 15) / 16 * 16 + window_w(base) * (wg / 2) * 4;
    }
    const int tb0 = (window_w(base) * (wg / 2) * 4 + 4 * (base + 1) + 15) / 16 * 16;
    const int tb = tb0 >= ebt ? tb0 : (ebt + 15) / 16 * 16;
    const int db = base - 32;
    const bool lsd_w1 = mw == 2 && db > 0 && db + (db > 20 ? 4 : 10) <= 30;
    const bool lsdx = mw == 2 && db > 0 && !lsd_w1 && (valu_limbs(base) & 1024) != 0;
    return tb + (b2 * es + 15) / 16 * 16 + (lsd_w1 || lsdx ? (2 * b2 * es + 15) / 16 * 16 : 0) +
           (lsdx ? (2 * b2 + 15) / 16 * 16 : 0);
}
constexpr int waves_at(int base, int wg) {
    const int lds = (163840 / lds_bytes(base, wg)) * (wg / 64) / 4;
    const int cap = lds < state_waves(base) ? lds : state_waves(base);
    return cap / (wg / 256) * (wg / 256);
}
constexpr int rounds_wg(int base) { return waves_at(base, 1024) > waves_at(base, 512) ? 1024 : 512; }
constexpr int big_wg(int base) { return waves_at(base, 1024) >= waves_at(base, 512) ? 1024 : 512; }

constexpr bool one_wg_per_cu(int base, int wg) { return waves_at(base, wg) == wg / 256; }

constexpr int sib_waves(int base, int m) { return m <= 1 ? state_waves(base) : (m <= 3 ? 6 : 5); }

template <int BASE_, int ND_, int NE_, int NE2_, int PROBE_ = 0, int WG_ = 512, int VD_ = 0, int LG_ = -1,
          int PERS_ = -1, int SIB_ = 1>
struct Cfg {
    static constexpr int BASE = BASE_;
    static constexpr int PROBE = PROBE_;
    static constexpr int ND = ND_, NE = NE_, NE2 = NE2_;
    static constexpr int D2 = digits_of(BASE).d2, D3 = digits_of(BASE).d3, DN = digits_of(BASE).dn;
    static constexpr bool N64 = fits64(BASE, DN);
    static constexpr bool OLDINIT = (VD_ & 65536) != 0;
    static constexpr bool C64 = !N64 && (WG_ >= 1024 || OLDINIT || PERS_ > 0);
    static constexpr int NS = cdiv(D2, 2), NC = cdiv(D3, 2), NX = cdiv(DN, 2);
    static constexpr int SL = ND + 1, CL = NE + 1, EL = NE2 + 1;
    static constexpr int S_TOPD = D2 - 2 * (NS - 1), C_TOPD = D3 - 2 * (NC - 1);
    static constexpr u32 B = (u32)BASE * BASE;
    static constexpr int T = log2ceil(B);
    static constexpr u32 BT = (1u << T) - B;
    static constexpr int MW = (BASE + 31) / 32;
    static constexpr bool SPLIT = MW == 3 && (VD_ & 512) != 0;
    static constexpr int ES = MW == 1 ? 4 : (MW == 2 || SPLIT ? 8 : 16);
    static constexpr int SH = T + ilog2(ES);
    static constexpr u32 ESB = ES * B, EBT = ES * BT;
    static constexpr int WG = WG_;
    static constexpr int TCHUNK = tchunk_of(BASE);
    static constexpr int NBINS = BASE + 1;
    static constexpr int W = window_w(BASE);
    static constexpr int W0 = window_w0(BASE);
    static constexpr int HQ = 2;
    static constexpr int HROW = WG / HQ;
    static constexpr int HIST_BYTES = W * HROW * 4;
    static constexpr int T2 = SPLIT ? std::max((4 * NBINS + 15) / 16 * 16, ((int)EBT / 2 + 15) / 16 * 16) : 0;
    static constexpr int TB0 = SPLIT ? (T2 + 4 * (int)B + 15) / 16 * 16 : (HIST_BYTES + 4 * NBINS + 15) / 16 * 16;
    static constexpr bool NOTAB = (VD_ & 32768) != 0;
    static constexpr int TB = NOTAB || TB0 >= (int)EBT ? TB0 : ((int)EBT + 15) / 16 * 16;
    static constexpr int OUTL = SPLIT ? 0 : HIST_BYTES;
    static constexpr int TC0 = (SPLIT ? T2 : TB) / 16 * 16;
    static constexpr int DB = BASE - 32;
    static constexpr bool TIGHT = DB > 20;
    static constexpr bool LSD_W1 = MW == 2 && DB > 0 && DB + (TIGHT ? 4 : 10) <= 30 && (VD_ & (16384 | 32768)) == 0;
    static constexpr bool LSDX = MW == 2 && DB > 0 && !LSD_W1 && (VD_ & 1024) != 0;
    static constexpr bool LSD = LSD_W1 || LSDX;
    static constexpr int TL = TB + (NOTAB ? 0 : ((int)(B * ES) + 15) / 16 * 16);
    static constexpr int LDE = (SIB_ > 1 && BASE_ >= 46) ? (int)B + 256 : 2 * (int)B;
    static constexpr int TK = TL + (LSD ? ((int)(LDE * ES) + 15) / 16 * 16 : 0);
    static constexpr int TEND = SPLIT ? (TB + (int)(B * ES) + 15) / 16 * 16
                                      : TK + (LSDX ? ((int)(2 * B) + 15) / 16 * 16 : 0);
    static constexpr int HB = SPLIT ? TEND : 0;
    static constexpr int NCOLD = SIB_ > 1 ? NC - CL : 0;
    static constexpr int COLD = TEND;
    static constexpr int COLD_BYTES = (SIB_ * NCOLD * WG_ * 2 + 15) / 16 * 16;
    static constexpr int LDS_BYTES = SPLIT ? HB + HIST_BYTES : TEND + COLD_BYTES;
    static constexpr int TAB_BYTES = TEND - TC0;
    static constexpr int ZA = SPLIT ? TC0 : TB;
    static constexpr int LO = LSD ? 1 : 0;
    static constexpr u32 DMASK = (1u << (DB > 0 && DB < 32 ? DB : 0)) - 1;
    static constexpr u32 FLAG_D1 = LSDX ? 1u << 6 : 1u << 30, FLAG_N3 = LSDX ? 1u << 7 : 1u << 31;
    static constexpr int F0 = LSDX ? 0 : TIGHT ? DB : (DB + 3) / 4 * 4;
    static constexpr int FC = LSDX ? 1 : TIGHT ? DB + 1 : F0 + 4;
    static constexpr int F0W = TIGHT ? 1 : 4, FCW = TIGHT ? 3 : 6;
    static constexpr int NN = NX + 1;
    static constexpr u32 DC = ES * B;
    static constexpr u32 MAGIC = (u32)(((1ull << 32) + DC - 1) / DC);
    static constexpr unsigned long long TMAX = (unsigned long long)ES * (5ull * B + 4);
    static constexpr bool C1 = ((unsigned long long)MAGIC * DC - (1ull << 32)) * (TMAX / ES) < (1ull << 32);
    static constexpr u32 MAGICB = (u32)(((1ull << 32) + B - 1) / B);
    static constexpr int VD = VD_;
    static constexpr int VDC = VD % 16, VDS = (VD / 16) % 16;
    static constexpr int VDB = (VD & 2048) ? 1 : 0;
    static constexpr bool VDLOW = (VD & 4096) != 0;
    static constexpr bool vd_s(int q) {
        if (NOTAB) return true;
        return VDLOW ? (q > LO && q <= LO + VDS && q < SL) : (q >= SL - VDB - VDS && q < SL - VDB);
    }
    static constexpr bool vd_c(int q) {
        if (NOTAB) return true;
        return VDLOW ? (q > LO && q <= LO + VDC && q < CL) : (q >= CL - VDB - VDC && q < CL - VDB);
    }
    static constexpr int LG = LG_ >= 0 ? LG_ : (SIB_ > 1 ? 100 : (MW == 3 && WG >= 1024 ? 8 : 0));
    static constexpr int SIB = SIB_;
    static constexpr bool PERS = SIB_ > 1 ? false : PERS_ >= 0 ? PERS_ != 0 : (WG >= 1024 && one_wg_per_cu(BASE, WG));
    using NoPers = Cfg<BASE_, ND_, NE_, NE2_, PROBE_, (PERS_ < 0 ? rounds_wg(BASE_) : WG_), VD_, LG_, 0>;
    using NoSib = std::conditional_t<(BASE_ >= 46),
                                     Cfg<BASE_, ND_, NE_, NE2_, PROBE_, big_wg(BASE_), valu_limbs_big(BASE_, ND_, NE_)>,
                                     Cfg<BASE_, ND_, NE_, NE2_, PROBE_, rounds_wg(BASE_), valu_limbs_big(BASE_, ND_, NE_), -1, 0>>;
    static constexpr int LGW = SIB_ > 1 ? 0 : (LG_ >= 0 ? LG_ : (MW == 3 && WG_ >= 1024 ? 8 : 0));
    static constexpr bool VDL = ((VD & 256) != 0 || NOTAB) && !LSD;
    static constexpr u32 MAGIC_D = (u32)(((1ull << 32) + ES * BASE - 1) / (ES * BASE));
    static_assert(VD == 0 || (MW >= 2 && split_exact(BASE, ES, MAGIC_D)), "VALU digit split");
    static_assert(VDC <= NE + 1 - (MW <= 2 ? 1 : 0) && VDS <= ND + 1 && (VD & ~0x1ffff) == 0 &&
                      ((VD & 1024) == 0 || LSDX),
                  "VALU-decoded limbs");
    static constexpr int WPE0 = (163840 / LDS_BYTES) * (WG / 64) / 4;
    static constexpr int WREG = (VD_ & 32768) && MW == 3 ? 2 : (VD_ & (16384 | 32768)) ? 4 : sib_waves(BASE, SIB);
    static constexpr int WPE1 = WPE0 < WREG ? WPE0 : WREG;
    static constexpr int WGK = WPE1 * 256 / WG;
    static constexpr int WPE = WGK > 0 ? (WGK * (WG / 64) + 3) / 4 : (WG / 64 + 3) / 4;
    static_assert(WPE >= 1, "LDS: not even one workgroup fits");
    static_assert(SL < NS && CL < NC && EL <= NE, "FD layout needs cached high limbs");
    static_assert(ND <= NX + 1 && NE2 <= NX + 1 && NE <= NS + 1, "difference limb counts");
    static_assert(S_TOPD >= 1 && C_TOPD >= 1, "top limb");
    static_assert((NOTAB || TB >= (int)EBT) && (NOTAB || TB - (int)EBT < 65536) && (!LSD || LSDX || TL < 65536),
                  "LDS offsets");
    static_assert(!NOTAB || (!LSD && !SPLIT && SIB_ == 1), "table-free kernel: regular lanes, no low-digit table");
    static_assert(!PERS || N64 || C64, "persistent grid: init() only (init_at is the rounds path's)");
    static_assert(!SPLIT || (T2 >= (int)EBT / 2 && T2 < 65536 && T2 + 4 * (int)B <= TB && 4 * NBINS <= TC0 &&
                             ES == 8 && TB < 65536),
                  "split layout");
    static_assert(LDS_BYTES <= 163840, "LDS");
    static_assert(TB % 16 == 0 && TAB_BYTES % 16 == 0 && HB % 16 == 0, "16-byte table copy");
    static_assert(W0 >= 0 && W0 + W <= NBINS, "window");
    static_assert(!LSD || (ES == 8 && (LSDX ? TIGHT && FC + FCW <= 6 : FC + FCW <= 30)), "low-digit entry layout");
    static_assert(C1 || ((unsigned long long)MAGICB * B - (1ull << 32)) * (TMAX / ES) < (1ull << 32),
                  "C-limb carry magic");
    static_assert(NN <= SL && NE >= NS, "C += 3S + N3 layout");
    static_assert(3 * ES <= 64, "inline-constant multiplier");
    static_assert(SIB == 1 || (LSD && MW == 2 && LO == 1 && SL >= 3 && CL >= 3 && ND >= 2 && NN >= 2),
                  "sibling lanes share limb 1: low-digit-table bases only");
    static_assert((unsigned long long)NX * B * B + 2ull * B < (1ull << 32), "32-bit init columns");
};

template <int B_, int ND_, int NE_, int NE2_>
using BatchCfg = std::conditional_t<(valu_limbs(B_) & 1024) == 0,
                                    Cfg<B_, ND_, NE_, NE2_, 0, 512, valu_limbs(B_), 0, 0>,
                                    Cfg<B_, ND_, NE_, NE2_, 0, big_wg(B_), valu_limbs_big(B_, ND_, NE_), 0, 0>>;

}
}
```

### nice_amd/csrc/fd2_detailed.hip

```cpp
#include <stdlib.h>

#include <map>
#include <mutex>

#include "fd2_combos.h"
#include "fd2_launch.hpp"

namespace nice {
namespace fd2 {

NICE_PROBE_ONLY(u64 *g_stamps = nullptr; u64 g_last_launch[6] = {};)
std::atomic<uint32_t> g_force_sib_stride{0};

struct Combo {
    int nd, ne, ne2;
};

static int limbs_of(const Nat &x, const std::vector<Nat> &pw) {
    int k = 0;
    while (k < (int)pw.size() && x.cmp(pw[k]) >= 0) k++;
    return k;
}

static Combo combo_at(uint32_t base, u128 e, const std::vector<Nat> &pw) {
    Nat n = Nat::from(e);
    Nat d1 = n;
    d1.mul_small(2);
    Nat one = Nat::from(1);
    auto add = [](Nat a, const Nat &b) {
        a.l.resize(std::max(a.l.size(), b.l.size()) + 1, 0);
        uint64_t c = 0;
        for (size_t i = 0; i < a.l.size(); i++) {
            uint64_t t = (uint64_t)a.l[i] + (i < b.l.size() ? b.l[i] : 0) + c;
            a.l[i] = (uint32_t)t;
            c = t >> 32;
        }
        a.trim();
        return a;
    };
    d1 = add(d1, one);
    Nat n3 = n;
    n3.mul_small(3);
    Nat e1 = add(add(n3.mul(n), n3), one);
    Nat e2 = n;
    e2.mul_small(6);
    e2 = add(e2, Nat::from(6));
    (void)base;
    return Combo{limbs_of(d1, pw), limbs_of(e1, pw), limbs_of(e2, pw)};
}

struct BaseThresholds {
    std::vector<Nat> pw;
    std::vector<u128> cuts;
    std::vector<Combo> combos;
};

static const BaseThresholds &thresholds(uint32_t base) {
    static std::mutex mu;
    static BaseThresholds cache[129];
    static bool have[129] = {};
    std::lock_guard<std::mutex> g(mu);
    BaseThresholds &t = cache[base];
    if (have[base]) return t;
    const uint32_t B = base * base;
    for (int k = 0; k < 40; k++) t.pw.push_back(Nat::pow(B, k));
    u128 rs = 0, re = 0;
    base_range(base, rs, re);
    u128 a = rs;
    Combo cur = combo_at(base, a + 1, t.pw);
    t.combos.push_back(cur);
    while (true) {
        Combo last = combo_at(base, re, t.pw);
        if (last.nd == cur.nd && last.ne == cur.ne && last.ne2 == cur.ne2) break;
        u128 lo = a + 1, hi = re;
        while (lo < hi) {
            u128 mid = lo + (hi - lo) / 2;
            Combo c = combo_at(base, mid, t.pw);
            if (c.nd == cur.nd && c.ne == cur.ne && c.ne2 == cur.ne2) lo = mid + 1;
            else hi = mid;
        }
        t.cuts.push_back(lo - 1);
        a = lo - 1;
        cur = combo_at(base, lo, t.pw);
        t.combos.push_back(cur);
    }
    have[base] = true;
    return t;
}

hipError_t launch_part0(const DetailedLaunch &, int, int, int, bool, int, hipStream_t);
hipError_t launch_part1(const DetailedLaunch &, int, int, int, bool, int, hipStream_t);
hipError_t launch_part2(const DetailedLaunch &, int, int, int, bool, int, hipStream_t);
hipError_t launch_part3(const DetailedLaunch &, int, int, int, bool, int, hipStream_t);
hipError_t launch_part4(const DetailedLaunch &, int, int, int, bool, int, hipStream_t);
hipError_t launch_part5(const DetailedLaunch &, int, int, int, bool, int, hipStream_t);
static_assert(FD2_NPARTS == 6, "launch_part declarations");

static hipError_t launch_segment(const DetailedLaunch &p, const Combo &c, int num_cus, hipStream_t s) {
    const int probe = (int)probe_knob("NICE_FD2_PROBE", 0);
#include NICE_PROBE_INC("fd2_detailed_probe_dispatch.inc")
    const bool force512 = probe_knob("NICE_FD2_WG512", 0) != 0;
    const u64 small = probe_knob("NICE_FD2_SMALL", 10000000ull);
    const bool wg512 = force512 || p.count < small || (probe == 20 && p.base == 80);
    using Fn = hipError_t (*)(const DetailedLaunch &, int, int, int, bool, int, hipStream_t);
    static const Fn parts[FD2_NPARTS] = {launch_part0, launch_part1, launch_part2,
                                         launch_part3, launch_part4, launch_part5};
    const hipError_t e = parts[fd2_part_of((int)p.base)](p, c.nd, c.ne, c.ne2, wg512, num_cus, s);
    return e == hipErrorNotFound ? hipErrorInvalidValue : e;
}

}

void fd2_force_sib_stride(uint32_t L) { fd2::g_force_sib_stride.store(L, std::memory_order_relaxed); }

bool fd2_supported(uint32_t base) {
    switch (base) {
#define X(b) case b:
        FD2_BASES(X)
#undef X
        return true;
    default: return false;
    }
}

bool fd2_window(uint32_t base, uint32_t *w0, uint32_t *w) {
    switch (base) {
#define X(b) case b: *w0 = fd2::window_w0(b), *w = fd2::window_w(b); return true;
        FD2_BASES(X)
#undef X
    default: return false;
    }
}

size_t fd2_cuts(uint32_t base, unsigned __int128 *out, size_t cap) {
    if (!fd2_supported(base)) return 0;
    const fd2::BaseThresholds &t = fd2::thresholds(base);
    for (size_t i = 0; i < t.cuts.size() && i < cap; i++) out[i] = t.cuts[i];
    return t.cuts.size();
}

hipError_t launch_detailed_fd2(const DetailedLaunch &p, int num_cus, hipStream_t s) {
    if (!fd2_supported(p.base)) return hipErrorInvalidValue;
    const fd2::BaseThresholds &t = fd2::thresholds(p.base);
    u128 a = ((u128)p.start_hi << 64) | p.start_lo;
    const u128 e = a + p.count;
    DetailedLaunch q = p;
    if (p.hist_copies < kHistCopies) q.hist_copies = (uint32_t)probe_knob("NICE_FD2_COPIES", p.hist_copies);
    if (q.hist_copies < 1 || q.hist_copies > kHistCopies) q.hist_copies = kHistCopies;
    for (size_t i = 0; i <= t.cuts.size() && a < e; i++) {
        u128 stop = i < t.cuts.size() && t.cuts[i] < e ? t.cuts[i] : e;
        if (stop <= a) continue;
        q.start_lo = (uint64_t)a;
        q.start_hi = (uint64_t)(a >> 64);
        q.count = (uint64_t)(stop - a);
        q.fin = stop == e ? p.fin : FieldFinish{nullptr, nullptr, 0, 0};
        hipError_t err = fd2::launch_segment(q, t.combos[i], num_cus, s);
        if (err != hipSuccess) return err;
        a = stop;
    }
    return hipSuccess;
}

namespace fd2 {
using BatchFn = hipError_t (*)(const BatchLaunch &, int, int, int, const void *, uint32_t, hipStream_t);
hipError_t launch_batch_part0(const BatchLaunch &, int, int, int, const void *, uint32_t, hipStream_t);
hipError_t launch_batch_part1(const BatchLaunch &, int, int, int, const void *, uint32_t, hipStream_t);
hipError_t launch_batch_part2(const BatchLaunch &, int, int, int, const void *, uint32_t, hipStream_t);
hipError_t launch_batch_part3(const BatchLaunch &, int, int, int, const void *, uint32_t, hipStream_t);
hipError_t launch_batch_part4(const BatchLaunch &, int, int, int, const void *, uint32_t, hipStream_t);
hipError_t launch_batch_part5(const BatchLaunch &, int, int, int, const void *, uint32_t, hipStream_t);
static_assert(FD2_NPARTS == 6, "launch_batch_part declarations");
}

uint32_t fd2_batch_wg(uint32_t base) {
    return (fd2::valu_limbs((int)base) & 1024) ? (uint32_t)fd2::big_wg((int)base) : 512u;
}

uint32_t fd2_batch_chunk(uint32_t base) { return (uint32_t)fd2::tchunk_of((int)base) + 1; }

void fd2_batch_plan(uint32_t base, u128 a, u128 e, uint32_t row, std::vector<BatchUnit> &out) {
    const fd2::BaseThresholds &t = fd2::thresholds(base);
    const u64 wg = fd2_batch_wg(base), tchunk = fd2_batch_chunk(base);
    for (size_t i = 0; i <= t.cuts.size() && a < e; i++) {
        const u128 stop = i < t.cuts.size() && t.cuts[i] < e ? t.cuts[i] : e;
        if (stop <= a) continue;
        const u128 cnt = stop - a;
        const fd2::BatchTile tile = fd2::batch_tile(cnt, wg, tchunk);
        const u64 chunk = tile.chunk, tail = tile.tail;
        u128 units = tile.units;
        u128 n = a;
        while (units) {
            const u64 lanes = units < wg ? (u64)units : wg;
            out.push_back(BatchUnit{(u64)n, (u64)(n >> 64), (uint32_t)lanes, (uint32_t)chunk, row, (uint32_t)i});
            n += (u128)lanes * chunk;
            units -= lanes;
        }
        if (tail) out.push_back(BatchUnit{(u64)n, (u64)(n >> 64), (uint32_t)tail, 1u, row, (uint32_t)i});
        a = stop;
    }
}

hipError_t launch_detailed_fd2_batch(const BatchLaunch &p, hipStream_t s) {
    if (!fd2_supported(p.base) || !p.n_units || p.n_units > 0x7fffffffull) return hipErrorInvalidValue;
    const fd2::BaseThresholds &t = fd2::thresholds(p.base);
    const size_t nc = t.combos.size();
    const u32 B = p.base * p.base;
    const int dn = fd2::digits_of((int)p.base).dn, nx = cdiv(dn, 2);
    const bool digits = !fd2::fits64(p.base, dn) && fd2_batch_wg(p.base) < 1024;
    std::vector<size_t> first(nc + 1, 0);
    for (size_t i = 0; i < p.n_units; i++) {
        if (p.units[i].combo >= nc) return hipErrorInvalidValue;
        first[p.units[i].combo + 1]++;
    }
    for (size_t c = 0; c < nc; c++) first[c + 1] += first[c];
    std::vector<size_t> at(first.begin(), first.end() - 1);
    fd2::Fd2Unit *h = (fd2::Fd2Unit *)p.h_desc;
    static_assert(sizeof(fd2::Fd2Unit) == kBatchDescBytes, "descriptor size");
    for (size_t i = 0; i < p.n_units; i++) {
        const BatchUnit &u = p.units[i];
        fd2::Fd2Unit &d = h[at[u.combo]++];
        d.lo = u.lo;
        d.hi = u.hi;
        d.lanes = u.lanes;
        d.chunk = u.chunk;
        d.row = u.row;
        d.pad = 0;
        for (int k = 0; k < fd2::kXDigits; k++) d.xs[k] = 0;
        if (digits) fd2::host_digits(((u128)u.hi << 64) | u.lo, B, d.xs, nx);
    }
    hipError_t err = hipMemcpyAsync(p.d_desc, p.h_desc, p.n_units * kBatchDescBytes, hipMemcpyHostToDevice, s);
    if (err != hipSuccess) return err;
    static const fd2::BatchFn parts[FD2_NPARTS] = {fd2::launch_batch_part0, fd2::launch_batch_part1,
                                                   fd2::launch_batch_part2, fd2::launch_batch_part3,
                                                   fd2::launch_batch_part4, fd2::launch_batch_part5};
    for (size_t c = 0; c < nc; c++) {
        const size_t n = first[c + 1] - first[c];
        if (!n) continue;
        const fd2::Combo &cb = t.combos[c];
        err = parts[fd2_part_of((int)p.base)](p, cb.nd, cb.ne, cb.ne2,
                                              (const fd2::Fd2Unit *)p.d_desc + first[c], (uint32_t)n, s);
        if (err != hipSuccess) return err == hipErrorNotFound ? hipErrorInvalidValue : err;
    }
    return hipSuccess;
}

}

#include NICE_PROBE_INC("fd2_detailed_probe_exports.inc")
```

### nice_amd/csrc/fd2_kernel.hpp

```cpp
#pragma once
#include "fd2_cfg.hpp"
#include "kernels.h"
#include "nice_device.hpp"
#include "probe.hpp"

namespace nice {
namespace fd2 {
template <u32 K>
__device__ __forceinline__ u32 mad_u24(u32 a, u32 c) {
    static_assert(K <= 64, "inline constant");
    u32 r;
    asm("v_mad_u32_u24 %0, %1, %2, %3" : "=v"(r) : "v"(a), "n"(K), "v"(c));
    return r;
}

template <int K>
__device__ __forceinline__ u32 mad_i24s(u32 a, u32 c) {
    u32 r;
    asm("v_mad_i32_i24 %0, %1, %2, %3" : "=v"(r) : "v"(a), "s"(K), "v"(c));
    return r;
}

__device__ __forceinline__ u32 bcnt_acc(u32 x, u32 acc) {
    u32 r;
    asm("v_bcnt_u32_b32 %0, %1, %2" : "=v"(r) : "v"(x), "s"(acc));
    return r;
}

template <class P>
struct State {
    u32 S[P::NS];
    u32 C[P::NC];
    u32 D1[P::ND];
    u32 N3[P::NN];
    u32 r8;
    u32 rc;
    u32 hi[P::MW];
};

template <class P>
__device__ __forceinline__ void or_entry(const unsigned char *p, u32 (&m)[P::MW]) {
    if constexpr (P::MW == 1) {
        m[0] |= *(const u32 *)p;
    } else if constexpr (P::MW == 2 || P::SPLIT) {
        uint2 v = *(const uint2 *)p;
        m[0] |= v.x;
        m[1] |= v.y;
    } else {
        uint4 v = *(const uint4 *)p;
        m[0] |= v.x;
        m[1] |= v.y;
        m[2] |= v.z;
        asm volatile("" ::"v"(v.w));
    }
}

template <class P, int OFF1, int OFF2>
__device__ __forceinline__ void or_lookup(const unsigned char *smem, u32 stored, u32 (&m)[P::MW]) {
    or_entry<P>(smem + OFF1 + stored, m);
    if constexpr (P::SPLIT) m[2] |= *(const u32 *)(smem + OFF2 + (stored >> 1));
}

template <class P>
__device__ __forceinline__ void lookup_group_end(u32 (&m)[P::MW]) {
#pragma unroll
    for (int w = 0; w < P::MW; w++) asm volatile("" : "+v"(m[w]));
    __builtin_amdgcn_sched_barrier(0);
}

template <class P>
__device__ __forceinline__ void or_valu(u32 vs, u32 (&m)[P::MW]) {
    const u32 q = __umulhi(vs, P::MAGIC_D);
    const u32 r = mad_i24s<-P::BASE>(q, vs / (u32)P::ES);
    if constexpr (P::MW == 2) {
        const u64 bits = (1ull << q) | (1ull << r);
        m[0] |= (u32)bits;
        m[1] |= (u32)(bits >> 32);
    } else {
        const u64 bq = 1ull << (q & 63), br = 1ull << (r & 63);
        const u32 wq = __builtin_amdgcn_ubfe(q, 6, 1) << (q & 31), wr = __builtin_amdgcn_ubfe(r, 6, 1) << (r & 31);
        m[0] |= ((u32)bq ^ wq) | ((u32)br ^ wr);
        m[1] |= (u32)(bq >> 32) | (u32)(br >> 32);
        m[2] |= wq | wr;
    }
}

template <class P>
__device__ __forceinline__ void or_plain(const unsigned char *smem, u32 v, int digits, u32 (&m)[P::MW]) {
    if (digits == 2) {
        if constexpr (P::NOTAB) or_valu<P>(v * P::ES, m);
        else or_lookup<P, P::TB, P::T2>(smem, v * P::ES, m);
    } else {
#pragma unroll
        for (int w = 0; w < P::MW; w++) m[w] |= (v >> 5) == (u32)w ? 1u << (v & 31) : 0u;
    }
}

template <class P>
__device__ __forceinline__ void recompute_hi(State<P> &st, const unsigned char *smem) {
#pragma unroll
    for (int w = 0; w < P::MW; w++) st.hi[w] = 0;
#pragma unroll
    for (int i = P::SL; i < P::NS; i++) or_plain<P>(smem, st.S[i], i == P::NS - 1 ? P::S_TOPD : 2, st.hi);
#pragma unroll
    for (int i = P::CL; i < P::NC; i++) or_plain<P>(smem, st.C[i], i == P::NC - 1 ? P::C_TOPD : 2, st.hi);
}

template <class P, int N, int M>
__device__ __forceinline__ void normalize64(const u64 (&acc)[N], u32 (&out)[M]) {
    u64 cy = 0;
#pragma unroll
    for (int t = 0; t < M; t++) {
        u64 v = (t < N ? acc[t] : 0) + cy;
        out[t] = (u32)(v % P::B);
        cy = v / P::B;
    }
}

template <class P, class A, int N, int M>
__device__ __forceinline__ void normalize(const A (&acc)[N], u32 (&out)[M]) {
    A cy = 0;
#pragma unroll
    for (int t = 0; t < M; t++) {
        const A v = (t < N ? acc[t] : (A)0) + cy;
        cy = v / P::B;
        out[t] = (u32)(v - cy * P::B);
    }
}

template <class P>
__device__ __forceinline__ void init_digits(u32 (&X)[P::NX], u64 n_lo, u64 n_hi) {
    constexpr u32 B = P::B;
    if constexpr (P::N64) {
        (void)n_hi;
        constexpr u64 B2 = (u64)B * B;
        u64 v = n_lo;
#pragma unroll
        for (int j = 0; j < P::NX; j += 2) {
            const u64 q = v / B2;
            const u32 r = (u32)(v - q * B2);
            X[j] = r % B;
            if (j + 1 < P::NX) X[j + 1] = r / B;
            v = q;
        }
    } else {
        u32 w[4] = {(u32)n_lo, (u32)(n_lo >> 32), (u32)n_hi, (u32)(n_hi >> 32)};
#pragma unroll
        for (int j = 0; j < P::NX; j++) {
            u64 rem = 0;
#pragma unroll
            for (int q = 3; q >= 0; q--) {
                u64 cur = (rem << 32) | w[q];
                w[q] = (u32)(cur / B);
                rem = cur % B;
            }
            X[j] = (u32)rem;
        }
    }
}

template <class P>
__device__ __forceinline__ void init_plain(State<P> &st, const u32 (&X)[P::NX]) {
    using A = u32;
    if constexpr (P::C64) {
        st.r8 = X[0] * P::ES + (P::LSDX ? (u32)P::TL : 0u);
        st.rc = X[0] + (u32)P::TK;
        {
            u64 acc[2 * P::NX];
#pragma unroll
            for (int t = 0; t < 2 * P::NX; t++) acc[t] = 0;
#pragma unroll
            for (int i = 0; i < P::NX; i++)
#pragma unroll
                for (int j = 0; j < P::NX; j++) acc[i + j] += (u64)X[i] * X[j];
            normalize64<P>(acc, st.S);
        }
        {
            u64 acc[P::NS + P::NX];
#pragma unroll
            for (int t = 0; t < P::NS + P::NX; t++) acc[t] = 0;
#pragma unroll
            for (int i = 0; i < P::NS; i++)
#pragma unroll
                for (int j = 0; j < P::NX; j++) acc[i + j] += (u64)st.S[i] * X[j];
            normalize64<P>(acc, st.C);
        }
        {
            u64 acc[P::NX];
#pragma unroll
            for (int t = 0; t < P::NX; t++) acc[t] = 2ull * X[t] + (t == 0 ? 1 : 0);
            normalize64<P>(acc, st.D1);
        }
        {
            u64 acc[P::NX];
#pragma unroll
            for (int t = 0; t < P::NX; t++) acc[t] = 3ull * X[t] + (t == 0 ? 1 : 0);
            normalize64<P>(acc, st.N3);
        }
    } else {
        st.r8 = X[0] * P::ES + (P::LSDX ? (u32)P::TL : 0u);
        st.rc = X[0] + (u32)P::TK;
        {
            A acc[2 * P::NX];
#pragma unroll
            for (int t = 0; t < 2 * P::NX; t++) acc[t] = 0;
#pragma unroll
            for (int i = 0; i < P::NX; i++)
#pragma unroll
                for (int j = 0; j < P::NX; j++) acc[i + j] += (A)X[i] * X[j];
            normalize<P>(acc, st.S);
        }
        {
            A acc[P::NS + P::NX];
#pragma unroll
            for (int t = 0; t < P::NS + P::NX; t++) acc[t] = 0;
#pragma unroll
            for (int i = 0; i < P::NS; i++)
#pragma unroll
                for (int j = 0; j < P::NX; j++) acc[i + j] += (A)st.S[i] * X[j];
            normalize<P>(acc, st.C);
        }
        {
            A acc[P::NX];
#pragma unroll
            for (int t = 0; t < P::NX; t++) acc[t] = 2 * (A)X[t] + (t == 0 ? 1 : 0);
            normalize<P>(acc, st.D1);
        }
        {
            A acc[P::NX];
#pragma unroll
            for (int t = 0; t < P::NX; t++) acc[t] = 3 * (A)X[t] + (t == 0 ? 1 : 0);
            normalize<P>(acc, st.N3);
        }
    }
}

template <class P>
__device__ __forceinline__ void init_scale(State<P> &st) {
    if constexpr (P::LSD) st.S[0] = st.C[0] = st.D1[0] = st.N3[0] = 0;
#pragma unroll
    for (int i = 0; i < P::SL; i++) st.S[i] = (st.S[i] + P::BT) * P::ES;
#pragma unroll
    for (int i = 0; i < P::CL; i++) st.C[i] *= P::ES;
#pragma unroll
    for (int i = 0; i < P::ND; i++) st.D1[i] *= P::ES;
#pragma unroll
    for (int i = 0; i < P::NN; i++) st.N3[i] = st.N3[i] * P::ES - (i < P::SL ? 3 * P::EBT : 0u);
}

template <class P>
__device__ __forceinline__ void init(State<P> &st, u64 n_lo, u64 n_hi) {
    u32 X[P::NX];
    init_digits<P>(X, n_lo, n_hi);
    init_plain<P>(st, X);
    init_scale<P>(st);
}

template <class P>
__device__ __forceinline__ void digits_plus(u32 (&X)[P::NX], const u32 *xb, u64 off) {
    constexpr u32 B = P::B;
    constexpr u64 B2 = (u64)B * B;
    const u64 q = off / B2;
    const u32 r = (u32)(off - q * B2), qq = (u32)q;
    const u32 o[4] = {r % B, r / B, qq % B, qq / B};
    u32 c = 0;
#pragma unroll
    for (int i = 0; i < P::NX; i++) {
        const u32 t = xb[i] + (i < 4 ? o[i] : 0u) + c;
        c = t >= B ? 1u : 0u;
        X[i] = t - c * B;
    }
}

template <class P>
__device__ __forceinline__ void init_at(State<P> &st, const u32 *xb, u64 off, u64 n_lo, u64 n_hi) {
    if constexpr (P::N64 || P::C64) {
        (void)xb;
        (void)off;
        init<P>(st, n_lo, n_hi);
    } else {
        (void)n_lo;
        (void)n_hi;
        u32 X[P::NX];
        digits_plus<P>(X, xb, off);
        init_plain<P>(st, X);
        init_scale<P>(st);
    }
}

template <class P, int N>
__device__ __forceinline__ void carry_scaled(u32 (&x)[N], int from) {
    u32 c = 1;
#pragma unroll
    for (int i = 0; i < N; i++) {
        if (i < from) continue;
        u32 v = x[i] + c * P::ES;
        c = v >= P::ESB;
        x[i] = c ? 0u : v;
    }
}
template <class P, int N>
__device__ __forceinline__ void carry_plain(u32 (&x)[N], int from) {
    u32 c = 1;
#pragma unroll
    for (int i = 0; i < N; i++) {
        if (i < from) continue;
        u32 v = x[i] + c;
        c = v == P::B;
        x[i] = c ? 0u : v;
    }
}

template <class P>
__device__ __forceinline__ void carry_n3(State<P> &st) {
    u32 c = 1;
#pragma unroll
    for (int i = 1; i < P::NN; i++) {
        const u32 off = i < P::SL ? 3 * P::EBT : 0u;
        u32 v = st.N3[i] + off + c * P::ES;
        c = v >= P::ESB;
        st.N3[i] = (c ? 0u : v) - off;
    }
}

template <class P>
__device__ __forceinline__ void rare(State<P> &st, const unsigned char *smem, u32 d1w, u32 n3w, bool cS,
                                     bool cC) {
    if (d1w) carry_scaled<P>(st.D1, 1);
    if (n3w) carry_n3<P>(st);
    if (cS) {
        st.S[P::SL - 1] -= P::ESB;
        carry_plain<P>(st.S, P::SL);
    }
    if (cC) {
        st.C[P::CL - 1] -= P::DC;
        carry_plain<P>(st.C, P::CL);
    }
    if (cS | cC) recompute_hi<P>(st, smem);
}

template <class P>
__device__ __forceinline__ void step(State<P> &st, const unsigned char *smem, u32 w1) {
    constexpr u32 ES = P::ES;
    constexpr int L0 = P::LO;
    constexpr int CT = P::CL - 1, ST = P::SL - 1;
    static_assert(CT >= P::NS && CT >= P::NN && ST >= P::ND, "top limbs take carries only");
    u32 cC = 0;
    if constexpr (P::LSD) cC = __builtin_amdgcn_ubfe(w1, P::FC, P::FCW);
#pragma unroll
    for (int i = L0; i < CT; i++) {
        u32 t;
        if (P::TIGHT && i == L0) t = mad_u24<ES>(cC, st.C[i]);
        else t = st.C[i] + cC;
        if (i > L0 && i < P::NN) asm("" : "+v"(t));
        if (i < P::NN) t += st.N3[i];
        else if (i < P::SL) t -= 3 * P::EBT;
        if (i < P::SL) t = mad_u24<3>(st.S[i], t);
        else if (i < P::NS) t = mad_u24<3 * ES>(st.S[i], t);
        const u32 c = P::C1 ? __umulhi(t, P::MAGIC) : __umulhi(t / ES, P::MAGICB);
        st.C[i] = t - c * P::DC;
        cC = c * ES;
    }
    st.C[CT] += cC;
    u32 cS = 0;
    if constexpr (P::LSD) cS = __builtin_amdgcn_ubfe(w1, P::F0, P::F0W);
#pragma unroll
    for (int i = L0; i < ST; i++) {
        u32 t;
        if (P::TIGHT && i == L0) t = mad_u24<ES>(cS, st.S[i] + (i < P::ND ? st.D1[i] : 0u));
        else t = st.S[i] + (i < P::ND ? st.D1[i] : 0u) + cS;
        cS = (t >> P::T) & ES;
        st.S[i] = t - cS * P::B;
    }
    st.S[ST] += cS;
    st.r8 += ES;
    if constexpr (P::LSDX) st.rc += 1;
    const bool topS = st.S[ST] >= (1u << P::SH), topC = st.C[CT] >= P::DC;
    if constexpr (P::LSD) {
        if (w1 >= P::FLAG_D1 || topS || topC)
            rare<P>(st, smem, w1 & P::FLAG_D1, w1 & P::FLAG_N3, topS, topC);
    } else {
        st.D1[0] += 2 * ES;
        st.N3[0] += 3 * ES;
        const u32 d1w = st.D1[0] >= P::ESB, n3w = st.N3[0] + 3 * P::EBT >= P::ESB;
        if (d1w || n3w || topS || topC) {
            if (d1w) st.D1[0] -= P::ESB;
            if (n3w) st.N3[0] -= P::ESB;
            rare<P>(st, smem, d1w, n3w, topS, topC);
        }
    }
}

template <class P>
__global__ void fd2_tables_kernel(unsigned char *tb) {
    const u32 e = blockIdx.x * blockDim.x + threadIdx.x;
    if (e >= P::B) return;
    u32 v[4] = {0, 0, 0, 0};
    auto mark = [&](u32 x) {
        u32 d0 = x % P::BASE, d1 = x / P::BASE;
        v[d0 >> 5] |= 1u << (d0 & 31);
        v[d1 >> 5] |= 1u << (d1 & 31);
    };
    auto put = [&](unsigned char *p) {
        if constexpr (P::ES == 4) *(u32 *)p = v[0];
        else if constexpr (P::ES == 8) *(uint2 *)p = make_uint2(v[0], v[1]);
        else *(uint4 *)p = make_uint4(v[0], v[1], v[2], v[3]);
    };
    mark(e);
    put(tb + (P::TB - P::TC0) + e * P::ES);
    if constexpr (P::SPLIT) *(u32 *)(tb + (P::T2 - P::TC0) + 4 * e) = v[2];
    if constexpr (P::LSD) {
        v[0] = v[1] = v[2] = v[3] = 0;
        const u32 B = P::B;
        const u32 s0 = (u32)((u64)e * e % B), c0 = (u32)((u64)s0 * e % B);
        mark(s0);
        mark(c0);
        const u32 d1 = (2 * e + 1) % B, n3 = (3 * e + 1) % B;
        u32 f = 0;
        f |= d1 + 2 >= B ? P::FLAG_D1 : 0u;
        f |= n3 + 3 >= B ? P::FLAG_N3 : 0u;
        const u32 sc = s0 + d1 >= B ? 1u : 0u, cc = (c0 + 3 * s0 + n3) / B;
        f |= (P::TIGHT ? sc : P::ES * sc) << P::F0;
        f |= (P::TIGHT ? cc : P::ES * cc) << P::FC;
        if constexpr (P::LSDX) {
            tb[(P::TK - P::TC0) + e] = (unsigned char)f;
            tb[(P::TK - P::TC0) + e + P::B] = (unsigned char)f;
        } else {
            v[1] |= f;
        }
        put(tb + (P::TL - P::TC0) + e * P::ES);
        if ((int)(e + P::B) < P::LDE) put(tb + (P::TL - P::TC0) + (e + P::B) * P::ES);
    }
}

constexpr u32 kStampGroups = 65536, kStampWords = 32;
#define FD2_STAMP_P(p, k)                                                                        \
    do {                                                                                         \
        if (kProbes && (p) && threadIdx.x == 0 && blockIdx.x < kStampGroups) {                   \
            (p)[kStampWords * (u64)blockIdx.x + 2 * (k)] = __builtin_amdgcn_s_memrealtime();     \
            (p)[kStampWords * (u64)blockIdx.x + 2 * (k) + 1] = __builtin_amdgcn_s_memtime();     \
        }                                                                                        \
    } while (0)
#define FD2_STAMP(a, k) FD2_STAMP_P((a).stamps, k)

struct Fd2Args {
    u64 *stamps;
    u64 start_lo, start_hi;
    u64 tail_lo, tail_hi;
    u32 nunits, chunk;
    u32 tail_count, main_blocks;
    u32 cutoff;
    u32 ncopies;
    u32 wave_cap;
    u64 sib_lo, sib_hi, edge_lo, edge_hi;
    u32 sib_chunk, sib_upb, sib_units, sib_blocks;
    u32 edge_chunk, edge_units, edge_blocks;
    u32 xs[12], xt[12];
    u64 *hist;
    NumOut out;
    const uint4 *tabs;
    FieldFinish fin;
};

template <int WG>
__device__ __forceinline__ void field_finish(const FieldFinish &fin, u64 *hist, u32 ncopies, u32 nbins, u32 *count,
                                             unsigned char *smem, u64 *stamps) {
    (void)stamps;
    __shared__ u32 last;
    asm volatile("s_waitcnt vmcnt(0)" ::: "memory");
    __syncthreads();
    if (threadIdx.x == 0) last = last_block_arrive(fin.done);
    __syncthreads();
    if (!last) return;
    FD2_STAMP_P(stamps, 7);
    unsigned long long *acc = (unsigned long long *)smem;
    for (u32 b = threadIdx.x; b < kHistBins; b += WG) acc[b] = 0;
    __syncthreads();
    constexpr u32 PER = (kHistCopies * kHistBins + WG - 1) / WG;
    const u32 NE = ncopies * nbins;
    const u32 nmiss = threadIdx.x == 0 ? __hip_atomic_load(count, __ATOMIC_RELAXED, __HIP_MEMORY_SCOPE_AGENT) : 0;
    u64 v[PER];
    u32 at[PER];
#pragma unroll
    for (u32 k = 0; k < PER; k++) {
        const u32 e = threadIdx.x + k * WG;
        const u32 c = e / nbins, b = e - c * nbins;
        at[k] = c * kHistBins + b;
        v[k] = e < NE ? __hip_atomic_load(&hist[at[k]], __ATOMIC_RELAXED, __HIP_MEMORY_SCOPE_AGENT) : 0;
    }
#pragma unroll
    for (u32 k = 0; k < PER; k++) {
        if (v[k]) {
            atomicAdd(&acc[at[k] % kHistBins], (unsigned long long)v[k]);
            __hip_atomic_store(&hist[at[k]], (u64)0, __ATOMIC_RELAXED, __HIP_MEMORY_SCOPE_AGENT);
        }
    }
    __syncthreads();
    FD2_STAMP_P(stamps, 8);
    done_reset(fin.done);
    if (fin.tag) {
        const u64 t = (u64)fin.tag << 32;
        for (u32 b = threadIdx.x; b < nbins; b += WG) fin.out_mapped[b] = t | (u32)acc[b];
        if (threadIdx.x == 0) {
            fin.out_mapped[kFinCount] = t | nmiss;
            __hip_atomic_store(count, 0u, __ATOMIC_RELAXED, __HIP_MEMORY_SCOPE_AGENT);
        }
        FD2_STAMP_P(stamps, 9);
        return;
    }
    for (u32 b = threadIdx.x; b < kHistBins; b += WG) fin.out_mapped[b] = acc[b];
    if (threadIdx.x == 0) {
        fin.out_mapped[kFinCount] = nmiss;
        __hip_atomic_store(count, 0u, __ATOMIC_RELAXED, __HIP_MEMORY_SCOPE_AGENT);
    }
    asm volatile("s_waitcnt vmcnt(0)" ::: "memory");
    __syncthreads();
    FD2_STAMP_P(stamps, 9);
    if (threadIdx.x == 0)
        __hip_atomic_store(&fin.out_mapped[kFinSeq], fin.seq, __ATOMIC_RELEASE, __HIP_MEMORY_SCOPE_SYSTEM);
}

template <class P>
__device__ __forceinline__ void walk_chunk(State<P> &st, const unsigned char *smem, u32 chunk, u64 n0_lo,
                                           u64 n0_hi, u32 hbase, u32 hinc, u32 *outl, u32 cutoff,
                                           const NumOut &out, u32 &probe_acc) {
    recompute_hi<P>(st, smem);
    const u32 r80 = st.r8;
    for (u32 i = 0; i < chunk; i++) {
        u32 m[P::MW], w1 = 0;
#pragma unroll
        for (int w = 0; w < P::MW; w++) m[w] = st.hi[w];
        if constexpr (P::PROBE & 1) {
            m[0] |= st.r8;
            w1 = st.r8 & 0xff;
#pragma unroll
            for (int q = P::LO; q < P::SL; q++) m[q & 1] |= st.S[q];
#pragma unroll
            for (int q = P::LO; q < P::CL; q++) m[q & 1] |= st.C[q];
        } else {
            if constexpr (P::LSD) {
                const uint2 v = *(const uint2 *)(smem + (P::LSDX ? 0 : P::TL) + st.r8);
                m[0] |= v.x;
                if constexpr (P::LSDX) {
                    m[1] |= v.y;
                    w1 = smem[st.rc];
                } else {
                    m[1] |= v.y & P::DMASK;
                    w1 = v.y;
                }
            }
#pragma unroll
            for (int q = P::LO; q < P::SL; q++) {
                if ((P::PROBE & 4) && q == 1) { m[0] |= st.S[q] & 0xffu; continue; }
                if (P::vd_s(q) || (P::VDL && q == 0)) or_valu<P>(st.S[q] - P::EBT, m);
                else or_lookup<P, P::TB - (int)P::EBT, P::T2 - (int)P::EBT / 2>(smem, st.S[q], m);
                if (P::LGW && (q - P::LO + 1) % P::LGW == 0) lookup_group_end<P>(m);
            }
#pragma unroll
            for (int q = P::LO; q < P::CL; q++) {
                if ((P::PROBE & 4) && q == 1) { m[1] |= st.C[q] & 0xffu; continue; }
                if (P::vd_c(q) || (P::VDL && q == 0)) or_valu<P>(st.C[q], m);
                else or_lookup<P, P::TB, P::T2>(smem, st.C[q], m);
                if (P::LGW && (P::SL + q - 2 * P::LO + 1) % P::LGW == 0) lookup_group_end<P>(m);
            }
        }
        u32 uw = bcnt_acc(m[0], (u32)(-P::W0));
#pragma unroll
        for (int w = 1; w < P::MW; w++) uw += __popc(m[w]);
        if (uw < (u32)P::W) {
            if constexpr (P::PROBE & 2) probe_acc++;
            else atomicAdd((u32 *)(smem + uw * (P::HROW * 4) + hbase), hinc);
        } else {
            const u32 u = uw + P::W0;
            atomicAdd(&outl[u], 1u);
            if (u > cutoff) {
                u64 lo = n0_lo, hi = n0_hi;
                add_u128(lo, hi, (st.r8 - r80) / P::ES);
                u32 pos = atomicAdd(out.count, 1u);
                if (pos < out.cap) {
                    out.n[2 * (u64)pos] = lo;
                    out.n[2 * (u64)pos + 1] = hi;
                    out.u[pos] = u;
                }
            }
        }
        step<P>(st, smem, w1);
    }
}


template <class P>
__device__ __forceinline__ u32 c_limb(State<P> &st, int i, u32 cC) {
    u32 t = st.C[i] + cC;
    if (i < P::NN) asm("" : "+v"(t));
    if (i < P::NN) t += st.N3[i];
    else if (i < P::SL) t -= 3 * P::EBT;
    if (i < P::SL) t = mad_u24<3>(st.S[i], t);
    else if (i < P::NS) t += st.S[i];
    const u32 c = P::C1 ? __umulhi(t, P::MAGIC) : __umulhi(t / P::ES, P::MAGICB);
    st.C[i] = t - c * P::DC;
    return c * P::ES;
}

template <class P>
__device__ __forceinline__ u32 s_limb(State<P> &st, int i, u32 cS) {
    const u32 t = st.S[i] + (i < P::ND ? st.D1[i] : 0u) + cS;
    const u32 c = (t >> P::T) & P::ES;
    st.S[i] = t - c * P::B;
    return c;
}

template <class P>
__device__ __forceinline__ unsigned short *cold_slot(const unsigned char *smem, int j, int k) {
    return (unsigned short *)(smem + P::COLD) + ((u32)(j * P::NCOLD + k) * P::WG + threadIdx.x);
}

template <class P>
__device__ __forceinline__ void sib_hi(State<P> &st, int j, const unsigned char *smem) {
#pragma unroll
    for (int w = 0; w < P::MW; w++) st.hi[w] = 0;
#pragma unroll
    for (int i = P::SL; i < P::NS; i++)
        or_plain<P>(smem, st.S[i] / (3 * P::ES), i == P::NS - 1 ? P::S_TOPD : 2, st.hi);
#pragma unroll
    for (int k = 0; k < P::NCOLD; k++)
        or_plain<P>(smem, *cold_slot<P>(smem, j, k), P::CL + k == P::NC - 1 ? P::C_TOPD : 2, st.hi);
}

template <class P>
__device__ __forceinline__ void sib_derive(State<P> &sj, const State<P> &s0, const u32 (&X)[P::NX], u32 j) {
    {
        u32 acc[P::NS];
#pragma unroll
        for (int t = 0; t < P::NS; t++)
            acc[t] = s0.S[t] + (t >= 2 && t - 2 < P::NX ? 2 * j * X[t - 2] : 0u) + (t == 4 ? j * j : 0u);
        normalize<P>(acc, sj.S);
    }
    {
        u32 acc[P::NC];
#pragma unroll
        for (int t = 0; t < P::NC; t++)
            acc[t] = s0.C[t] + (t >= 2 && t - 2 < P::NS ? 3 * j * s0.S[t - 2] : 0u) +
                     (t >= 4 && t - 4 < P::NX ? 3 * j * j * X[t - 4] : 0u) + (t == 6 ? j * j * j : 0u);
        normalize<P>(acc, sj.C);
    }
    {
        u32 acc[P::ND];
#pragma unroll
        for (int t = 0; t < P::ND; t++) acc[t] = s0.D1[t] + (t == 2 ? 2 * j : 0u);
        normalize<P>(acc, sj.D1);
    }
    {
        u32 acc[P::NN];
#pragma unroll
        for (int t = 0; t < P::NN; t++) acc[t] = s0.N3[t] + (t == 2 ? 3 * j : 0u);
        normalize<P>(acc, sj.N3);
    }
    sj.r8 = s0.r8;
    sj.rc = s0.rc;
}

template <class P>
__device__ __forceinline__ void sib_park(State<P> &st, int j, const unsigned char *smem) {
#pragma unroll
    for (int i = P::SL; i < P::NS; i++) st.S[i] *= 3 * P::ES;
#pragma unroll
    for (int k = 0; k < P::NCOLD; k++) *cold_slot<P>(smem, j, k) = (unsigned short)st.C[P::CL + k];
}

template <class P>
__device__ __forceinline__ void rare_sib(State<P> (&st)[P::SIB], const unsigned char *smem,
                                      const bool (&cS)[P::SIB], const bool (&cC)[P::SIB]) {
    constexpr int L = P::LO;
    if (st[0].D1[L] >= P::ESB) {
        st[0].D1[L] -= P::ESB;
#pragma unroll
        for (int j = 0; j < P::SIB; j++) carry_scaled<P>(st[j].D1, L + 1);
    }
    {
        const u32 off1 = L < P::SL ? 3 * P::EBT : 0u;
        if (st[0].N3[L] + off1 >= P::ESB) {
            st[0].N3[L] -= P::ESB;
#pragma unroll
            for (int j = 0; j < P::SIB; j++) {
                u32 cc = 1;
#pragma unroll
                for (int i = L + 1; i < P::NN; i++) {
                    const u32 off = i < P::SL ? 3 * P::EBT : 0u;
                    const u32 w = st[j].N3[i] + off + cc * P::ES;
                    cc = w >= P::ESB;
                    st[j].N3[i] = (cc ? 0u : w) - off;
                }
            }
        }
    }
#pragma unroll
    for (int j = 0; j < P::SIB; j++) {
        if (cS[j]) {
            st[j].S[P::SL - 1] -= P::ESB;
            u32 c = 1;
#pragma unroll
            for (int i = P::SL; i < P::NS; i++) {
                const u32 v = st[j].S[i] + c * 3 * P::ES;
                c = v >= 3 * P::ESB;
                st[j].S[i] = c ? 0u : v;
            }
        }
        if (cC[j]) {
            st[j].C[P::CL - 1] -= P::DC;
            u32 c = 1;
#pragma unroll
            for (int k = 0; k < P::NCOLD; k++) {
                unsigned short *slot = cold_slot<P>(smem, j, k);
                const u32 v = *slot + c;
                c = v == P::B;
                *slot = (unsigned short)(c ? 0u : v);
            }
        }
        if (cS[j] | cC[j]) sib_hi<P>(st[j], j, smem);
    }
}

template <class P>
__device__ __forceinline__ void sib_shared_step(State<P> &s0, u32 w1, u32 &cC, u32 &cS, bool &wrap);

template <class P>
__device__ __forceinline__ void step_sib(State<P> (&st)[P::SIB], const unsigned char *smem, u32 w1) {
    constexpr int L = P::LO;
    constexpr int CT = P::CL - 1, ST = P::SL - 1;
    u32 cC, cS;
    bool any;
    sib_shared_step<P>(st[0], w1, cC, cS, any);
    bool topS[P::SIB], topC[P::SIB];
#pragma unroll
    for (int j = 0; j < P::SIB; j++) {
        u32 c = cC;
#pragma unroll
        for (int i = L + 1; i < CT; i++) c = c_limb<P>(st[j], i, c);
        st[j].C[CT] += c;
        u32 cs = cS;
#pragma unroll
        for (int i = L + 1; i < ST; i++) cs = s_limb<P>(st[j], i, cs);
        st[j].S[ST] += cs;
        topS[j] = st[j].S[ST] >= (1u << P::SH);
        topC[j] = st[j].C[CT] >= P::DC;
        any |= topS[j] | topC[j];
    }
    if (any) rare_sib<P>(st, smem, topS, topC);
}

template <class P>
__device__ __forceinline__ void sib_shared_step(State<P> &s0, u32 w1, u32 &cC, u32 &cS, bool &wrap) {
    constexpr u32 ES = P::ES;
    constexpr int L = P::LO;
    static_assert(L < P::ND && L < P::NN && P::FLAG_D1 == (1u << 30) && P::FLAG_N3 == (1u << 31),
                  "sibling lanes: shared D1 / N3 limb and the low-digit entry's wrap flags");
    cC = __builtin_amdgcn_ubfe(w1, P::FC, P::FCW);
    {
        u32 t = P::TIGHT ? mad_u24<ES>(cC, s0.C[L]) : s0.C[L] + cC;
        if (L < P::NN) t += s0.N3[L];
        else t -= 3 * P::EBT;
        t = mad_u24<3>(s0.S[L], t);
        const u32 c = P::C1 ? __umulhi(t, P::MAGIC) : __umulhi(t / ES, P::MAGICB);
        s0.C[L] = t - c * P::DC;
        cC = c * ES;
    }
    cS = __builtin_amdgcn_ubfe(w1, P::F0, P::F0W);
    {
        const u32 d = L < P::ND ? s0.D1[L] : 0u;
        const u32 t = P::TIGHT ? mad_u24<ES>(cS, s0.S[L] + d) : s0.S[L] + d + cS;
        cS = (t >> P::T) & ES;
        s0.S[L] = t - cS * P::B;
    }
    s0.r8 += ES;
    s0.D1[L] += (w1 >> (30 - ilog2(ES))) & ES;
    s0.N3[L] += (w1 >> (31 - ilog2(ES))) & ES;
    wrap = (s0.D1[L] >= P::ESB) | (s0.N3[L] + (L < P::SL ? 3 * P::EBT : 0u) >= P::ESB);
}

template <class P>
__device__ __forceinline__ bool sib_upper_step(State<P> &st, u32 cC, u32 cS, bool &topS, bool &topC) {
    constexpr int L = P::LO;
    constexpr int CT = P::CL - 1, ST = P::SL - 1;
#pragma unroll
    for (int i = L + 1; i < CT; i++) cC = c_limb<P>(st, i, cC);
    st.C[CT] += cC;
#pragma unroll
    for (int i = L + 1; i < ST; i++) cS = s_limb<P>(st, i, cS);
    st.S[ST] += cS;
    topS = st.S[ST] >= (1u << P::SH);
    topC = st.C[CT] >= P::DC;
    return topS | topC;
}

template <class P>
struct SibLook {
    uint2 s[P::SL], c[P::CL];
};

template <class P>
__device__ __forceinline__ void sib_issue(const State<P> &st, const unsigned char *smem, SibLook<P> &e) {
#pragma unroll
    for (int q = P::LO + 1; q < P::SL; q++)
        if (!P::vd_s(q)) e.s[q] = *(const uint2 *)(smem + (P::TB - (int)P::EBT) + st.S[q]);
#pragma unroll
    for (int q = P::LO + 1; q < P::CL; q++)
        if (!P::vd_c(q)) e.c[q] = *(const uint2 *)(smem + P::TB + st.C[q]);
}

template <class P>
__device__ __forceinline__ void sib_consume(const State<P> &st, const SibLook<P> &e, u32 (&m)[P::MW]) {
#pragma unroll
    for (int q = P::LO + 1; q < P::SL; q++) {
        if (P::vd_s(q)) {
            or_valu<P>(st.S[q] - P::EBT, m);
        } else {
            m[0] |= e.s[q].x;
            m[1] |= e.s[q].y;
        }
    }
#pragma unroll
    for (int q = P::LO + 1; q < P::CL; q++) {
        if (P::vd_c(q)) {
            or_valu<P>(st.C[q], m);
        } else {
            m[0] |= e.c[q].x;
            m[1] |= e.c[q].y;
        }
    }
}

template <class P>
__device__ __forceinline__ void or_limb(const State<P> &st, const unsigned char *smem, bool isS, int q,
                                        u32 (&m)[P::MW]) {
    if (isS) {
        if (P::vd_s(q)) or_valu<P>(st.S[q] - P::EBT, m);
        else or_lookup<P, P::TB - (int)P::EBT, P::T2 - (int)P::EBT / 2>(smem, st.S[q], m);
    } else {
        if (P::vd_c(q)) or_valu<P>(st.C[q], m);
        else or_lookup<P, P::TB, P::T2>(smem, st.C[q], m);
    }
}

struct SibUnit {
    bool active;
    u32 chunk;
    u64 lo, hi;
};
template <class P>
__device__ __forceinline__ SibUnit sib_unit(const Fd2Args &a) {
    const bool edge = blockIdx.x >= a.sib_blocks;
    const u32 sunit = (edge ? blockIdx.x - a.sib_blocks : blockIdx.x) * P::WG + threadIdx.x;
    const u32 upb = edge ? 1u : a.sib_upb;
    SibUnit u;
    u.active = sunit < (edge ? a.edge_units : a.sib_units);
    u.chunk = edge ? a.edge_chunk : a.sib_chunk;
    const u32 q = sunit / upb, k = sunit - q * upb;
    u.lo = edge ? a.edge_lo : a.sib_lo;
    u.hi = edge ? a.edge_hi : a.sib_hi;
    add_u128(u.lo, u.hi, (u64)q * ((u64)P::SIB * P::B * P::B) + (u64)k * u.chunk);
    return u;
}

template <class P>
__device__ __forceinline__ void sib_record(u32 u, int j, u32 i, const Fd2Args &a, u32 *outl, u32 cutoff,
                                           const NumOut &out);

template <class P>
__device__ __forceinline__ void sib_count(const u32 (&m)[P::MW], int j, u32 i, const unsigned char *smem,
                                          const Fd2Args &a, u32 hbase, u32 hinc, u32 *outl, u32 cutoff,
                                          const NumOut &out) {
    u32 uw = bcnt_acc(m[0], (u32)(-P::W0));
#pragma unroll
    for (int w = 1; w < P::MW; w++) uw += __popc(m[w]);
    if (uw < (u32)P::W) {
        atomicAdd((u32 *)(smem + uw * (P::HROW * 4) + hbase), hinc);
    } else {
        sib_record<P>(uw + P::W0, j, i, a, outl, cutoff, out);
    }
}

template <class P>
__device__ __forceinline__ void sib_record(u32 u, int j, u32 i, const Fd2Args &a, u32 *outl, u32 cutoff,
                                           const NumOut &out) {
    {
        atomicAdd(&outl[u], 1u);
        if (u > cutoff) {
            const SibUnit su = sib_unit<P>(a);
            u64 lo = su.lo, hi = su.hi;
            u32 ii = i;
            asm volatile("" : "+v"(ii));
            add_u128(lo, hi, (u64)j * ((u64)P::B * P::B) + ii);
            u32 pos = atomicAdd(out.count, 1u);
            if (pos < out.cap) {
                out.n[2 * (u64)pos] = lo;
                out.n[2 * (u64)pos + 1] = hi;
                out.u[pos] = u;
            }
        }
    }
}

template <class P>
__device__ __forceinline__ void walk_sib_pipe(State<P> (&st)[P::SIB], const unsigned char *smem, const Fd2Args &a,
                                              u32 chunk, u32 hbase, u32 hinc, u32 *outl, u32 cutoff,
                                              const NumOut &out) {
    constexpr int L = P::LO;
    constexpr int M = P::SIB;
#pragma unroll
    for (int j = 0; j < M; j++) sib_hi<P>(st[j], j, smem);
    for (u32 i = 0; i < chunk; i++) {
        SibLook<P> e[M];
        const uint2 vlo = *(const uint2 *)(smem + P::TL + st[0].r8);
        uint2 vs, vc;
        u32 mv[P::MW] = {};
        if (P::vd_s(L)) or_valu<P>(st[0].S[L] - P::EBT, mv);
        else vs = *(const uint2 *)(smem + (P::TB - (int)P::EBT) + st[0].S[L]);
        if (P::vd_c(L)) or_valu<P>(st[0].C[L], mv);
        else vc = *(const uint2 *)(smem + P::TB + st[0].C[L]);
        sib_issue<P>(st[0], smem, e[0]);
        __builtin_amdgcn_sched_barrier(0);
        const u32 w1 = vlo.y;
        u32 cC, cS;
        bool any;
        sib_shared_step<P>(st[0], w1, cC, cS, any);
        if (M > 1) sib_issue<P>(st[1], smem, e[1]);
        __builtin_amdgcn_sched_barrier(0);
        u32 m0[P::MW];
        bool topS[M], topC[M];
#pragma unroll
        for (int j = 0; j < M; j++) {
            if (j == 0) {
                m0[0] = vlo.x | mv[0] | (P::vd_s(L) ? 0u : vs.x) | (P::vd_c(L) ? 0u : vc.x);
                m0[1] = (vlo.y & P::DMASK) | mv[1] | (P::vd_s(L) ? 0u : vs.y) | (P::vd_c(L) ? 0u : vc.y);
            }
            u32 m[P::MW];
#pragma unroll
            for (int w = 0; w < P::MW; w++) m[w] = m0[w] | st[j].hi[w];
            sib_consume<P>(st[j], e[j], m);
            if constexpr ((P::PROBE & 16) != 0) {
                any |= (m[0] ^ m[1]) == 0x5a5a5a5au;
            } else {
                sib_count<P>(m, j, i, smem, a, hbase, hinc, outl, cutoff, out);
            }
            any |= sib_upper_step<P>(st[j], cC, cS, topS[j], topC[j]);
            if (j + 2 < M) sib_issue<P>(st[j + 2], smem, e[j + 2]);
            __builtin_amdgcn_sched_barrier(0);
        }
        if ((P::PROBE & 8) == 0 && any) rare_sib<P>(st, smem, topS, topC);
    }
}

template <class P>
__device__ __forceinline__ void walk_sib(State<P> (&st)[P::SIB], const unsigned char *smem, const Fd2Args &a,
                                         u32 chunk, u32 hbase, u32 hinc, u32 *outl, u32 cutoff, const NumOut &out) {
    if constexpr (P::LG >= 100) {
        walk_sib_pipe<P>(st, smem, a, chunk, hbase, hinc, outl, cutoff, out);
        return;
    }
    constexpr int L = P::LO;
#pragma unroll
    for (int j = 0; j < P::SIB; j++) sib_hi<P>(st[j], j, smem);
    const u32 r80 = st[0].r8;
    for (u32 i = 0; i < chunk; i++) {
        u32 m0[P::MW];
        const uint2 v = *(const uint2 *)(smem + P::TL + st[0].r8);
        const u32 w1 = v.y;
        m0[0] = v.x;
        m0[1] = v.y & P::DMASK;
        or_limb<P>(st[0], smem, true, L, m0);
        or_limb<P>(st[0], smem, false, L, m0);
#pragma unroll
        for (int j = 0; j < P::SIB; j++) {
            u32 m[P::MW];
#pragma unroll
            for (int w = 0; w < P::MW; w++) m[w] = m0[w] | st[j].hi[w];
#pragma unroll
            for (int q = L + 1; q < P::SL; q++) {
                or_limb<P>(st[j], smem, true, q, m);
                if (P::LG > 1 && (q - L) % P::LG == 0) lookup_group_end<P>(m);
            }
#pragma unroll
            for (int q = L + 1; q < P::CL; q++) {
                or_limb<P>(st[j], smem, false, q, m);
                if (P::LG > 1 && (P::SL - L - 1 + q - L) % P::LG == 0) lookup_group_end<P>(m);
            }
            if (P::LG) lookup_group_end<P>(m);
            u32 uw = bcnt_acc(m[0], (u32)(-P::W0));
#pragma unroll
            for (int w = 1; w < P::MW; w++) uw += __popc(m[w]);
            if (uw < (u32)P::W) {
                atomicAdd((u32 *)(smem + uw * (P::HROW * 4) + hbase), hinc);
            } else {
                const u32 u = uw + P::W0;
                atomicAdd(&outl[u], 1u);
                if (u > cutoff) {
                    const SibUnit su = sib_unit<P>(a);
                    u64 lo = su.lo, hi = su.hi;
                    add_u128(lo, hi, (u64)j * ((u64)P::B * P::B) + (st[0].r8 - r80) / P::ES);
                    u32 pos = atomicAdd(out.count, 1u);
                    if (pos < out.cap) {
                        out.n[2 * (u64)pos] = lo;
                        out.n[2 * (u64)pos + 1] = hi;
                        out.u[pos] = u;
                    }
                }
            }
        }
        step_sib<P>(st, smem, w1);
    }
}

template <class P>
__device__ __forceinline__ void fd2_load_tables(unsigned char *smem, const uint4 *tabs, u32 tid) {
    constexpr u32 N16 = (u32)(P::TAB_BYTES / 16);
    const u32 lane = tid & 63, w64 = tid & ~63u;
    for (u32 i0 = w64; i0 < N16; i0 += P::WG)
        if (i0 + lane < N16)
            __builtin_amdgcn_global_load_lds((__attribute__((address_space(1))) void *)(tabs + i0 + lane),
                                             (__attribute__((address_space(3))) void *)(smem + P::TC0 + 16 * i0),
                                             16, 0, 0);
    uint4 *h4 = (uint4 *)smem;
    for (u32 i = tid; i < (u32)(P::ZA / 16); i += P::WG) h4[i] = make_uint4(0, 0, 0, 0);
    if constexpr (P::SPLIT)
        for (u32 i = tid; i < (u32)(P::HIST_BYTES / 16); i += P::WG)
            h4[P::HB / 16 + i] = make_uint4(0, 0, 0, 0);
}

template <class P>
__device__ __forceinline__ void fd2_flush(const unsigned char *smem, u64 *hist_rows, u32 row_out, u32 tid) {
    const u32 *hist = (const u32 *)(smem + P::HB);
    const u32 *outl = (const u32 *)(smem + P::OUTL);
    const u32 lane = tid & 63, wave = tid >> 6;
    u64 *hist_out = hist_rows + row_out * kHistBins;
    constexpr u32 NWAVE = P::WG / 64, RPW = (P::W + NWAVE - 1) / NWAVE;
    u32 rs[RPW];
#pragma unroll
    for (u32 k = 0; k < RPW; k++) {
        const u32 row = wave + k * NWAVE;
        u32 s = 0;
        if (row < (u32)P::W) {
#pragma unroll
            for (int q = 0; q < P::HROW / 64; q++) {
                const u32 v = hist[row * P::HROW + lane + 64 * q];
                if constexpr (P::HQ == 2) s += (v & 0xffffu) + (v >> 16);
                else s += (v & 0xffu) + ((v >> 8) & 0xffu) + ((v >> 16) & 0xffu) + (v >> 24);
            }
        }
        rs[k] = s;
    }
#pragma unroll
    for (int o = 32; o >= 1; o >>= 1)
#pragma unroll
        for (u32 k = 0; k < RPW; k++) rs[k] += __shfl_xor(rs[k], o);
#pragma unroll
    for (u32 k = 0; k < RPW; k++) {
        const u32 row = wave + k * NWAVE;
        if (lane == 0 && row < (u32)P::W && rs[k])
            atomicAdd((unsigned long long *)&hist_out[P::W0 + row], (unsigned long long)rs[k]);
    }
    if (tid < (u32)P::NBINS && outl[tid])
        atomicAdd((unsigned long long *)&hist_out[tid], (unsigned long long)outl[tid]);
}

__device__ __forceinline__ void pers_unit(const Fd2Args &a, u32 b, u32 mb, u32 lane, bool &active, u64 &lo,
                                          u64 &hi, u32 &chunk) {
    if (b < mb) {
        const u32 unit = 64 * b + lane;
        active = unit < a.nunits;
        lo = a.start_lo;
        hi = a.start_hi;
        add_u128(lo, hi, (u64)unit * a.chunk);
        chunk = a.chunk;
    } else {
        const u32 idx = 64 * (b - mb) + lane;
        active = idx < a.tail_count;
        lo = a.tail_lo;
        hi = a.tail_hi;
        add_u128(lo, hi, (u64)idx);
        chunk = 1;
    }
}

template <class P>
__device__ __forceinline__ void fd2_body(const Fd2Args &a) {
    __shared__ __attribute__((aligned(16))) unsigned char smem[P::LDS_BYTES];
    u32 *hist = (u32 *)(smem + P::HB);
    u32 *outl = (u32 *)(smem + P::OUTL);
    const u32 tid = threadIdx.x;
    const NumOut out = a.out;
    const u32 cutoff = a.cutoff;
    const u32 sib_end = P::SIB > 1 ? a.sib_blocks + a.edge_blocks : 0u;
    const bool sib_part = P::SIB > 1 && blockIdx.x < sib_end;
    const u32 bid = blockIdx.x - sib_end;
    const bool main_part = bid < a.main_blocks;
    const u64 start_lo = main_part ? a.start_lo : a.tail_lo;
    const u64 start_hi = main_part ? a.start_hi : a.tail_hi;
    const u32 nunits = main_part ? a.nunits : a.tail_count;
    const u32 chunk = main_part ? a.chunk : 1u;
    const u32 blk = main_part ? bid : bid - a.main_blocks;
    FD2_STAMP(a, 0);

    {
        constexpr u32 N16 = (u32)(P::TAB_BYTES / 16);
        const u32 lane = tid & 63, w64 = tid & ~63u;
        for (u32 i0 = w64; i0 < N16; i0 += P::WG)
            if (i0 + lane < N16)
                __builtin_amdgcn_global_load_lds((__attribute__((address_space(1))) void *)(a.tabs + i0 + lane),
                                                 (__attribute__((address_space(3))) void *)(smem + P::TC0 + 16 * i0),
                                                 16, 0, 0);
        uint4 *h4 = (uint4 *)smem;
        for (u32 i = tid; i < (u32)(P::ZA / 16); i += P::WG) h4[i] = make_uint4(0, 0, 0, 0);
        if constexpr (P::SPLIT)
            for (u32 i = tid; i < (u32)(P::HIST_BYTES / 16); i += P::WG)
                h4[P::HB / 16 + i] = make_uint4(0, 0, 0, 0);
    }
    const u32 lane_id = tid & 63;
    u32 unit = blk * P::WG + tid;
    bool active = unit < nunits;
    u64 n0_lo = start_lo, n0_hi = start_hi;
    u32 chunk_l = chunk;
    __shared__ u32 pers_next;
    u32 pmb = 0, pnk = 0, pk = 0;
    u64 n0_off = 0;
    const bool n0_tail = !main_part;
    if constexpr (P::PERS) {
        pmb = (a.nunits + 63) / 64;
        const u32 nb = pmb + (a.tail_count + 63) / 64, G = gridDim.x;
        pnk = nb > blockIdx.x ? (nb - blockIdx.x + G - 1) / G : 0;
        pk = tid >> 6;
        if (tid == 0) pers_next = P::WG / 64;
        if (pk < pnk) pers_unit(a, blockIdx.x + G * pk, pmb, lane_id, active, n0_lo, n0_hi, chunk_l);
        else active = false;
    } else {
        n0_off = (u64)unit * chunk;
        add_u128(n0_lo, n0_hi, n0_off);
    }
    const u32 hbase = P::HB + tid % P::HROW * 4;
    static_assert(P::HROW % 64 == 0, "window row of whole waves");
    const u32 hinc = __builtin_amdgcn_readfirstlane(1u << (32 / P::HQ * (tid / P::HROW)));
    u32 probe_acc = 0;
    bool sib_done = false;
    if constexpr (P::SIB > 1) {
        if (sib_part) {
            State<P> sst[P::SIB];
            const SibUnit su = sib_unit<P>(a);
            if (su.active) {
                u32 X[P::NX];
                init_digits<P>(X, su.lo, su.hi);
                init_plain<P>(sst[0], X);
#pragma unroll
                for (int j = 1; j < P::SIB; j++) sib_derive<P>(sst[j], sst[0], X, (u32)j);
#pragma unroll
                for (int j = 0; j < P::SIB; j++) {
                    init_scale<P>(sst[j]);
                    sib_park<P>(sst[j], j, smem);
                }
            }
            asm volatile("s_waitcnt vmcnt(0)" ::: "memory");
            __syncthreads();
            if (su.active) walk_sib<P>(sst, smem, a, su.chunk, hbase, hinc, outl, cutoff, out);
            sib_done = true;
        }
    }
    State<P> st;
    if constexpr (P::PERS || P::N64 || P::C64) {
        if (!sib_done && active) init<P>(st, n0_lo, n0_hi);
    } else {
        if (!sib_done && active) init_at<P>(st, n0_tail ? a.xt : a.xs, n0_off, n0_lo, n0_hi);
    }
    if (!sib_done) {
        asm volatile("s_waitcnt vmcnt(0)" ::: "memory");
        __syncthreads();
    }
    FD2_STAMP(a, 1);
    FD2_STAMP(a, 2);
    if constexpr (P::SIB > 1) {
        if (!sib_done && active)
            walk_chunk<P>(st, smem, chunk, n0_lo, n0_hi, hbase, hinc, outl, cutoff, out, probe_acc);
    } else if constexpr (!P::PERS) {
        if (active) {
            walk_chunk<P>(st, smem, chunk, n0_lo, n0_hi, hbase, hinc, outl, cutoff, out, probe_acc);
        }
    } else {
        u32 k = pk, taken = 0;
        bool act = active;
        u64 m_lo = n0_lo, m_hi = n0_hi;
        u32 ch = chunk_l;
        while (k < pnk) {
            if (taken) {
                pers_unit(a, blockIdx.x + gridDim.x * k, pmb, lane_id, act, m_lo, m_hi, ch);
                if (act) init<P>(st, m_lo, m_hi);
            }
            if (act) walk_chunk<P>(st, smem, ch, m_lo, m_hi, hbase, hinc, outl, cutoff, out, probe_acc);
            if (++taken >= a.wave_cap) break;
            u32 nk = 0;
            if (lane_id == 0) nk = atomicAdd(&pers_next, 1u);
            k = __builtin_amdgcn_readfirstlane(__shfl(nk, 0));
        }
    }
    if constexpr ((P::PROBE & 2) != 0) atomicAdd(&outl[P::W0], probe_acc);
    FD2_STAMP(a, 3);
    __syncthreads();
    FD2_STAMP(a, 4);
    const u32 lane = tid & 63, wave = tid >> 6;
    u64 *hist_out = a.hist + (blockIdx.x % a.ncopies) * kHistBins;
    constexpr u32 NWAVE = P::WG / 64, RPW = (P::W + NWAVE - 1) / NWAVE;
    u32 rs[RPW];
#pragma unroll
    for (u32 k = 0; k < RPW; k++) {
        const u32 row = wave + k * NWAVE;
        u32 s = 0;
        if (row < (u32)P::W) {
#pragma unroll
            for (int q = 0; q < P::HROW / 64; q++) {
                const u32 v = hist[row * P::HROW + lane + 64 * q];
                if constexpr (P::HQ == 2) s += (v & 0xffffu) + (v >> 16);
                else s += (v & 0xffu) + ((v >> 8) & 0xffu) + ((v >> 16) & 0xffu) + (v >> 24);
            }
        }
        rs[k] = s;
    }
#pragma unroll
    for (int o = 32; o >= 1; o >>= 1)
#pragma unroll
        for (u32 k = 0; k < RPW; k++) rs[k] += __shfl_xor(rs[k], o);
#pragma unroll
    for (u32 k = 0; k < RPW; k++) {
        const u32 row = wave + k * NWAVE;
        if (lane == 0 && row < (u32)P::W && rs[k])
            atomicAdd((unsigned long long *)&hist_out[P::W0 + row], (unsigned long long)rs[k]);
    }
    if (tid < (u32)P::NBINS && outl[tid])
        atomicAdd((unsigned long long *)&hist_out[tid], (unsigned long long)outl[tid]);
    FD2_STAMP(a, 5);
    if (a.fin.out_mapped) {
        __syncthreads();
        field_finish<P::WG>(a.fin, a.hist, a.ncopies, P::NBINS, out.count, smem, a.stamps);
    }
    FD2_STAMP(a, 6);
}

template <class P>
__global__ void __launch_bounds__(P::WG) __attribute__((amdgpu_waves_per_eu(P::WPE, P::WPE)))
fd2_kernel(Fd2Args a) {
    fd2_body<P>(a);
}

constexpr int kXDigits = 12;
struct Fd2Unit {
    u64 lo, hi;
    u32 lanes;
    u32 chunk;
    u32 row;
    u32 pad;
    u32 xs[kXDigits];
};
static_assert(sizeof(Fd2Unit) == 80, "descriptor layout");

struct Fd2BatchArgs {
    const Fd2Unit *units;
    u64 *hist;
    u32 ncopies;
    u32 cutoff;
    NumOut out;
    const uint4 *tabs;
};

template <class P>
__global__ void __launch_bounds__(P::WG) __attribute__((amdgpu_waves_per_eu(P::WPE, P::WPE)))
fd2_batch_kernel(Fd2BatchArgs a) {
    static_assert(!P::PERS && P::SIB == 1 && P::PROBE == 0, "batch kernel: rounds, regular lanes");
    static_assert(!(P::MW == 3 && P::WG >= 1024) && P::LGW == 0, "BatchCfg spells out the default lookup groups");
    __shared__ __attribute__((aligned(16))) unsigned char smem[P::LDS_BYTES];
    u32 *outl = (u32 *)(smem + P::OUTL);
    const u32 tid = threadIdx.x;
    const Fd2Unit *__restrict__ d = a.units + blockIdx.x;
    const u64 start_lo = d->lo, start_hi = d->hi;
    const u32 lanes = d->lanes, chunk = d->chunk;
    const u32 row = a.ncopies ? blockIdx.x % a.ncopies : d->row;
    u32 xs[P::NX];
    if constexpr (!P::N64 && !P::C64) {
#pragma unroll
        for (int i = 0; i < P::NX; i++) xs[i] = d->xs[i];
    }
    const NumOut out = a.out;
    const u32 cutoff = a.cutoff;
    fd2_load_tables<P>(smem, a.tabs, tid);
    const bool active = tid < lanes;
    const u64 n0_off = (u64)tid * chunk;
    u64 n0_lo = start_lo, n0_hi = start_hi;
    add_u128(n0_lo, n0_hi, n0_off);
    const u32 hbase = P::HB + tid % P::HROW * 4;
    const u32 hinc = __builtin_amdgcn_readfirstlane(1u << (32 / P::HQ * (tid / P::HROW)));
    u32 probe_acc = 0;
    State<P> st;
    if constexpr (P::N64 || P::C64) {
        if (active) init<P>(st, n0_lo, n0_hi);
    } else {
        if (active) init_at<P>(st, xs, n0_off, n0_lo, n0_hi);
    }
    asm volatile("s_waitcnt vmcnt(0)" ::: "memory");
    __syncthreads();
    if (active) walk_chunk<P>(st, smem, chunk, n0_lo, n0_hi, hbase, hinc, outl, cutoff, out, probe_acc);
    __syncthreads();
    fd2_flush<P>(smem, a.hist, row, tid);
}

}
}
```

### nice_amd/csrc/fd2_launch.hpp

```cpp
#pragma once
#include <stdlib.h>

#include <atomic>
#include <map>
#include <mutex>

#include "fd2_kernel.hpp"
#include "fd2_plan.hpp"
#include "host_math.hpp"

namespace nice {
namespace fd2 {

NICE_PROBE_ONLY(extern u64 *g_stamps; extern u64 g_last_launch[6];)
extern std::atomic<uint32_t> g_force_sib_stride;

template <class P>
static hipError_t fd2_tables(hipStream_t s, const uint4 **out) {
    if constexpr (P::TAB_BYTES == 0) {
        (void)s;
        *out = nullptr;
        return hipSuccess;
    }
    static std::mutex mu;
    static std::map<int, unsigned char *> have;
    int dev = 0;
    hipError_t e = hipGetDevice(&dev);
    if (e != hipSuccess) return e;
    std::lock_guard<std::mutex> g(mu);
    auto it = have.find(dev);
    if (it == have.end()) {
        unsigned char *t = nullptr;
        if ((e = hipMalloc(&t, P::TAB_BYTES)) != hipSuccess) return e;
        if ((e = hipMemsetAsync(t, 0, P::TAB_BYTES, s)) != hipSuccess) return e;
        hipLaunchKernelGGL(fd2_tables_kernel<P>, dim3((P::B + 255) / 256), dim3(256), 0, s, t);
        if ((e = hipGetLastError()) != hipSuccess) return e;
        if ((e = hipStreamSynchronize(s)) != hipSuccess) return e;
        it = have.emplace(dev, t).first;
    }
    *out = (const uint4 *)it->second;
    return hipSuccess;
}

template <class P>
static int fd2_occupancy() {
    static const int per_cu_q = [] {
        int v = 0;
        return hipOccupancyMaxActiveBlocksPerMultiprocessor(&v, (const void *)fd2_kernel<P>, P::WG, 0) == hipSuccess
                   ? v : -1;
    }();
    return per_cu_q;
}

template <class P>
static PlanKnobs<P> fd2_knobs() {
    PlanKnobs<P> k;
    k.tchunk = probe_knob("NICE_FD2_TCHUNK", k.tchunk);
    k.min_chunk = probe_knob("NICE_FD2_MINCHUNK", k.min_chunk);
    k.sib_chunk = probe_knob("NICE_FD2_SIBCHUNK", k.sib_chunk);
    k.sib_rounds = probe_knob("NICE_FD2_SIBROUNDS", k.sib_rounds);
    return k;
}

static inline void fd2_regular_parts(Fd2Args &a, u64 lo, u64 hi, u64 nunits, u64 chunk, u64 tail, u64 main_blocks) {
    a.start_lo = a.tail_lo = lo;
    a.start_hi = a.tail_hi = hi;
    add_u128(a.tail_lo, a.tail_hi, nunits * chunk);
    a.nunits = (u32)nunits;
    a.chunk = (u32)chunk;
    a.tail_count = (u32)tail;
    a.main_blocks = (u32)main_blocks;
}

template <class P>
static hipError_t fd2_enqueue(Fd2Args &a, const DetailedLaunch &q, const uint4 *tabs, bool last, u64 grid,
                              hipStream_t s) {
    NICE_PROBE_ONLY(a.stamps = g_stamps;)
    a.cutoff = q.cutoff;
    a.ncopies = q.hist_copies;
    a.hist = q.hist;
    a.out = q.out;
    a.tabs = tabs;
    a.fin = last ? q.fin : FieldFinish{nullptr, nullptr, 0, 0};
    hipLaunchKernelGGL(fd2_kernel<P>, dim3((u32)grid), dim3(P::WG), 0, s, a);
    const hipError_t e = hipGetLastError();
    if (e == hipSuccess && q.launches) ++*q.launches;
    return e;
}

template <class P>
static hipError_t launch_sib(const DetailedLaunch &p, int num_cus, hipStream_t s);

template <class P>
static hipError_t launch_cfg(const DetailedLaunch &p, int num_cus, hipStream_t s) {
    if constexpr (P::SIB > 1) return launch_sib<P>(p, num_cus, s);
    const int per_cu_q = fd2_occupancy<P>();
    if (per_cu_q < 0) return hipErrorInvalidDeviceFunction;
    const int per_cu = per_cu_q < 1 ? 1 : per_cu_q;
    if (p.cutoff + 1 < (u32)(P::W0 + P::W)) return hipErrorInvalidValue;
    const PlanKnobs<P> knobs = fd2_knobs<P>();
    if constexpr (P::PERS) {
        if (!pers_suits<P>(p.count, num_cus, per_cu_q, knobs)) return launch_cfg<typename P::NoPers>(p, num_cus, s);
    }
    const uint4 *tabs = nullptr;
    hipError_t e = fd2_tables<P>(s, &tabs);
    if (e != hipSuccess) return e;
    DetailedLaunch q = p;
    u64 left = p.count;
    while (left) {
        const RegularPlan pl = plan_regular<P>(left, num_cus, per_cu, knobs);
        if (!pl.ok) return hipErrorInvalidValue;
        Fd2Args a{};
        fd2_regular_parts(a, q.start_lo, q.start_hi, pl.nunits, pl.chunk, pl.tail, pl.main_blocks);
        if constexpr (!P::N64 && !P::C64) {
            host_digits(((u128)a.start_hi << 64) | a.start_lo, P::B, a.xs, P::NX);
            host_digits(((u128)a.tail_hi << 64) | a.tail_lo, P::B, a.xt, P::NX);
        }
        a.wave_cap = pl.wave_cap;
        NICE_PROBE_ONLY({
            const u64 v[6] = {pl.grid, (u64)P::WG, pl.chunk, pl.nunits, pl.tail, (u64)per_cu};
            for (int k = 0; k < 6; k++) g_last_launch[k] = v[k];
        })
        if ((e = fd2_enqueue<P>(a, q, tabs, left == pl.cnt, pl.grid, s)) != hipSuccess) return e;
        add_u128(q.start_lo, q.start_hi, pl.cnt);
        left -= pl.cnt;
    }
    return hipSuccess;
}

template <class P>
static hipError_t launch_batch_cfg(const BatchLaunch &p, const Fd2Unit *units, u32 n, hipStream_t s) {
    if (p.cutoff + 1 < (u32)(P::W0 + P::W)) return hipErrorInvalidValue;
    const uint4 *tabs = nullptr;
    hipError_t e = fd2_tables<P>(s, &tabs);
    if (e != hipSuccess) return e;
    Fd2BatchArgs a{};
    a.units = units;
    a.hist = p.hist;
    a.ncopies = p.ncopies;
    a.cutoff = p.cutoff;
    a.out = p.out;
    a.tabs = tabs;
    hipLaunchKernelGGL(fd2_batch_kernel<P>, dim3(n), dim3(P::WG), 0, s, a);
    if ((e = hipGetLastError()) != hipSuccess) return e;
    if (p.launches) ++*p.launches;
    return hipSuccess;
}

template <class P>
static hipError_t launch_sib(const DetailedLaunch &p, int num_cus, hipStream_t s) {
    const int per_cu_q = fd2_occupancy<P>();
    if (per_cu_q < 0) return hipErrorInvalidDeviceFunction;
    const int per_cu = per_cu_q < 1 ? 1 : per_cu_q;
    if (sib_too_short<P>(p.count)) return launch_cfg<typename P::NoSib>(p, num_cus, s);
    if (p.cutoff + 1 < (u32)(P::W0 + P::W)) return hipErrorInvalidValue;
    const uint4 *tabs = nullptr;
    hipError_t e = fd2_tables<P>(s, &tabs);
    if (e != hipSuccess) return e;
    const PlanKnobs<P> knobs = fd2_knobs<P>();
    const u128 seg_start = ((u128)p.start_hi << 64) | p.start_lo;
    const SibShape sh = plan_sib<P>(seg_start, p.count, num_cus, per_cu, p.overlapped != 0,
                                    g_force_sib_stride.load(std::memory_order_relaxed), knobs);
    if (sh.kind == SibShape::kNoSib) return launch_cfg<typename P::NoSib>(p, num_cus, s);
    if (sh.kind == SibShape::kError) return hipErrorInvalidValue;
    if (p.sib) {
        p.sib[0] = (uint32_t)P::SIB;
        p.sib[1] = (uint32_t)sh.L;
    }
    constexpr u64 SB = (u64)P::SIB * P::B * P::B;
    DetailedLaunch q = p;
    u64 left = p.count;
    while (left) {
        const SibLaunchPlan pl = plan_sib_launch<P>(left, sh, num_cus, per_cu, knobs);
        Fd2Args a{};
        a.sib_lo = a.edge_lo = q.start_lo;
        a.sib_hi = a.edge_hi = q.start_hi;
        add_u128(a.edge_lo, a.edge_hi, sh.upb * sh.L);
        a.sib_chunk = (u32)sh.L;
        a.sib_upb = (u32)sh.upb;
        a.sib_units = (u32)pl.sib_units;
        a.sib_blocks = (u32)pl.sib_blocks;
        a.edge_chunk = (u32)sh.r;
        a.edge_units = (u32)pl.edge_units;
        a.edge_blocks = (u32)pl.edge_blocks;
        u64 lo = q.start_lo, hi = q.start_hi;
        add_u128(lo, hi, pl.Q * SB);
        fd2_regular_parts(a, lo, hi, pl.nunits, pl.chunk, pl.tail, pl.main_blocks);
        a.wave_cap = 0;
        NICE_PROBE_ONLY({
            const u64 v[6] = {pl.grid, (u64)P::WG, sh.L, pl.sib_units, pl.R, (u64)per_cu};
            for (int k = 0; k < 6; k++) g_last_launch[k] = v[k];
        })
        if ((e = fd2_enqueue<P>(a, q, tabs, left == pl.cnt, pl.grid, s)) != hipSuccess) return e;
        add_u128(q.start_lo, q.start_hi, pl.cnt);
        left -= pl.cnt;
    }
    return hipSuccess;
}

}
}
```

### nice_amd/csrc/fd2_plan.hpp

```cpp
#pragma once

#include <algorithm>
#include <cmath>
#include <map>
#include <mutex>
#include <vector>

#include "layout.h"

namespace nice {
namespace fd2 {

static inline void host_digits(u128 n, u32 B, u32 *out, int nx) {
    for (int i = 0; i < nx; i++) {
        out[i] = (u32)(n % B);
        n /= B;
    }
}

static const std::vector<float> &progression_cost(int slots) {
    static std::mutex mu;
    static std::map<int, std::vector<float>> tab;
    std::lock_guard<std::mutex> g(mu);
    auto it = tab.find(slots);
    if (it != tab.end()) return it->second;
    std::vector<float> t((size_t)slots * 128);
    for (size_t k = 0; k < t.size(); k++) {
        const double d = (double)k / 64;
        double sum = 0;
        for (int ai = 0; ai < 16; ai++) {
            const double a = ai / 16.0 + 0.03125;
            int cnt[32] = {};
            int best = 0;
            long prev = -1;
            for (int l = 0; l < slots; l++) {
                const long v = (long)(a + d * l);
                if (v == prev) continue;
                prev = v;
                const int sl = (int)(v & (slots - 1));
                best = std::max(best, ++cnt[sl]);
            }
            sum += best;
        }
        t[k] = (float)(sum / 16);
    }
    return tab.emplace(slots, std::move(t)).first->second;
}

template <class P>
struct ConflictModel {
    static constexpr int SLOTS = P::ES == 16 ? 16 : 32;
    static constexpr int NPASS = 64 / SLOTS;
    int n = 0;
    double c[3 * (P::SL + P::CL)], k[3 * (P::SL + P::CL)];
    const std::vector<float> *tab;
    ConflictModel(long double n0, long double span, int first_limb) : tab(&progression_cost(SLOTS)) {
        for (int pt = 0; pt < 3; pt++) {
            const long double x = n0 + span * (long double)pt / 2;
            for (int cube = 0; cube < 2; cube++) {
                const int hi = cube ? P::CL : P::SL;
                long double bq = 1;
                for (int q = 0; q < first_limb; q++) bq *= (long double)P::B;
                for (int q = first_limb; q < hi; q++, bq *= (long double)P::B) {
                    if (cube ? P::vd_c(q) : P::vd_s(q)) continue;
                    const long double f1 = cube ? 3 * x * x : 2 * x;
                    const long double f2 = cube ? 6 * x : 2;
                    c[n] = (double)(f1 / bq);
                    k[n] = (double)(f2 * 4096 / 2 / bq);
                    n++;
                }
            }
        }
    }
    double cost(u64 L) const {
        double sum = 0;
        const double l = (double)L;
        for (int i = 0; i < n; i++) {
            if (k[i] * l * l >= 0.5) continue;
            const double d = c[i] * l;
            const double r = d < SLOTS ? d : SLOTS + (d - SLOTS * std::floor(d / SLOTS));
            sum += NPASS * (*tab)[std::min<size_t>(tab->size() - 1, (size_t)(r * 64))];
        }
        return sum / 3;
    }
};

template <class P>
static u64 pick_lane_stride(u128 start, u64 count, u64 lo, u64 hi, u64 target, int first_limb,
                            double tol = 0.5) {
    const ConflictModel<P> m((long double)start, (long double)count, first_limb);
    double cost[512];
    int nc = 0;
    double min_cost = 1e30;
    for (u64 L = lo | 1; L <= hi && nc < 512; L += 2, nc++) {
        cost[nc] = m.cost(L);
        min_cost = std::min(min_cost, cost[nc]);
    }
    u64 best = target | 1, best_d = ~0ull;
    nc = 0;
    for (u64 L = lo | 1; L <= hi && nc < 512; L += 2, nc++) {
        const u64 d = L > target ? L - target : target - L;
        if (cost[nc] <= min_cost + tol && d < best_d) {
            best = L;
            best_d = d;
        }
    }
    return best;
}

template <class P>
static u64 pick_small_stride(u128 start, u64 count, u64 lo, u64 hi, int first_limb, u64 Q, u64 lanes, u64 D,
                             double &rounds, double init = 6, double tol = 6) {
    const ConflictModel<P> m((long double)start, (long double)count, first_limb);
    double cost[512];
    int nc = 0;
    double min_cost = 1e30;
    for (u64 L = lo | 1; L <= hi && nc < 512; L += 2, nc++) {
        cost[nc] = m.cost(L);
        min_cost = std::min(min_cost, cost[nc]);
    }
    u64 best = lo | 1;
    double best_t = 1e300;
    rounds = 0;
    nc = 0;
    for (u64 L = lo | 1; L <= hi && nc < 512; L += 2, nc++) {
        if (cost[nc] > min_cost + tol) continue;
        const u64 units = Q * ((D + L - 1) / L - 1);
        const double t = (double)((units + lanes - 1) / lanes) * ((double)L + init);
        if (t < best_t) {
            best_t = t;
            best = L;
            rounds = (double)units / (double)lanes;
        }
    }
    return best;
}


template <class P>
struct PlanKnobs {
    u64 tchunk = (u64)P::TCHUNK;
    u64 min_chunk = 4;
    u64 sib_chunk = 0;
    u64 sib_rounds = 15;
};

static inline u64 rounds_chunk(u64 cnt, u64 lanes, u64 tchunk, u64 floor, bool odd, u64 cap) {
    u64 rounds = (cnt + tchunk * lanes - 1) / (tchunk * lanes);
    if (rounds < 1) rounds = 1;
    u64 chunk = (cnt + rounds * lanes - 1) / (rounds * lanes);
    if (chunk < floor) chunk = cnt < floor ? cnt : floor;
    if (chunk < 1) chunk = 1;
    if (chunk > 1 && (odd ? chunk % 2 == 0 : chunk % 16 == 0)) chunk++;
    if (chunk > cap) chunk = cap % 2 ? cap : cap - 1;
    return chunk;
}

struct BatchTile {
    u64 chunk;
    u128 units;
    u64 tail;
};
static inline BatchTile batch_tile(u128 cnt, u64 wg, u64 tchunk) {
    const u128 nwg = (cnt + (u128)wg * tchunk - 1) / ((u128)wg * tchunk);
    u64 chunk = (u64)((cnt + nwg * wg - 1) / (nwg * wg));
    if (chunk > 1 && chunk % 2 == 0) chunk++;
    const u128 units = cnt / chunk;
    return BatchTile{chunk, units, (u64)(cnt - units * chunk)};
}

template <class P>
static bool pers_suits(u64 count, int num_cus, int per_cu_q, const PlanKnobs<P> &k = PlanKnobs<P>{}) {
    return per_cu_q == 1 && count >= 2 * k.tchunk * ((u64)num_cus * P::WG);
}

struct RegularPlan {
    bool ok;
    u64 cnt, chunk, nunits, tail, grid, main_blocks;
    u32 wave_cap;
};
template <class P>
static RegularPlan plan_regular(u64 left, int num_cus, int per_cu, const PlanKnobs<P> &k = PlanKnobs<P>{}) {
    const u64 lanes = (u64)num_cus * per_cu * P::WG;
    const u64 max_count = lanes * 60000ull;
    const u64 nw = P::WG / 64;
    RegularPlan pl{};
    pl.cnt = left < max_count ? left : max_count;
    for (;;) {
        pl.chunk = rounds_chunk(pl.cnt, lanes, k.tchunk, k.min_chunk, P::LSD, P::B);
        if (P::HQ == 4 && pl.chunk > 255) return pl;
        pl.nunits = pl.cnt / pl.chunk;
        pl.tail = pl.cnt - pl.nunits * pl.chunk;
        bool fits = pl.nunits <= 0xffffffffull;
        if constexpr (P::PERS) {
            const u64 nb = (pl.nunits + 63) / 64 + (pl.tail + 63) / 64;
            pl.grid = std::min<u64>((u64)num_cus * per_cu, (nb + nw - 1) / nw);
            fits = fits && pl.nunits <= 0xffffffc0ull && (nb + pl.grid - 1) / pl.grid <= nw * (65535 / pl.chunk);
        } else {
            pl.grid = (pl.nunits + P::WG - 1) / P::WG + (pl.tail + P::WG - 1) / P::WG;
        }
        if (fits) break;
        if (pl.cnt < 2) return pl;
        pl.cnt /= 2;
    }
    pl.main_blocks = (pl.nunits + P::WG - 1) / P::WG;
    pl.wave_cap = (u32)(65535 / pl.chunk);
    pl.ok = true;
    return pl;
}

struct SibShape {
    enum Kind { kNoSib, kError, kSib } kind;
    u64 L;
    u64 U, upb, r;
    bool has_edge;
    u64 qmax;
};
template <class P>
static bool sib_too_short(u64 count) {
    return count < 4 * ((u64)P::SIB * P::B * P::B);
}
template <class P>
static SibShape plan_sib(u128 seg_start, u64 count, int num_cus, int per_cu, bool overlapped, u64 forced,
                         const PlanKnobs<P> &k = PlanKnobs<P>{}) {
    constexpr u64 D = (u64)P::B * P::B, SB = (u64)P::SIB * D;
    const u64 lanes = (u64)num_cus * per_cu * P::WG;
    SibShape sh{};
    sh.kind = SibShape::kNoSib;
    if (sib_too_short<P>(count)) return sh;
    u64 L = k.sib_chunk;
    if (!L) L = forced;
    const u64 Q0 = count / SB;
    if (!L && !overlapped && 10 * Q0 * (D / P::TCHUNK) < 60 * lanes) {
        double rounds = 0;
        L = pick_small_stride<P>(seg_start, count, P::TCHUNK * 3 / 4, P::TCHUNK * 5 / 4, P::LO + 1, Q0, lanes, D,
                                 rounds);
        if (10 * rounds < (double)k.sib_rounds) return sh;
    }
    constexpr u64 T = P::LG >= 100 ? 140 : (u64)P::TCHUNK;
    if (!L && P::LG >= 100 && !overlapped) {
        double rounds = 0;
        L = pick_small_stride<P>(seg_start, count, T * 3 / 4, T * 3 / 2, P::LO + 1, Q0, lanes, D, rounds);
    }
    if (!L) L = pick_lane_stride<P>(seg_start, count, T * 3 / 4, T * 3 / 2, T, P::LO + 1);
    constexpr u64 LMAX = (u64)P::LDE - P::B;
    if (L % 2 == 0) L++;
    if (L > D / 4) L = (D / 4) | 1;
    if (L > LMAX) L = LMAX % 2 ? LMAX : LMAX - 1;
    sh.L = L;
    sh.U = (D + L - 1) / L;
    sh.r = D - (sh.U - 1) * L;
    sh.has_edge = sh.r != L;
    sh.upb = sh.has_edge ? sh.U - 1 : sh.U;
    if ((u64)P::SIB * L > 65535) {
        sh.kind = SibShape::kError;
        return sh;
    }
    sh.qmax = std::max<u64>(1, std::min<u64>(0xffffffffull / sh.upb, ((u64)num_cus * 2048 * 60000ull) / SB));
    sh.kind = SibShape::kSib;
    return sh;
}

struct SibLaunchPlan {
    u64 Q, cnt, R;
    u64 chunk, nunits, tail;
    u64 sib_units, sib_blocks, edge_units, edge_blocks, main_blocks, grid;
};
template <class P>
static SibLaunchPlan plan_sib_launch(u64 left, const SibShape &sh, int num_cus, int per_cu,
                                     const PlanKnobs<P> &k = PlanKnobs<P>{}) {
    constexpr u64 SB = (u64)P::SIB * P::B * P::B, LMAX = (u64)P::LDE - P::B;
    const u64 lanes = (u64)num_cus * per_cu * P::WG;
    SibLaunchPlan pl{};
    pl.Q = left / SB;
    pl.cnt = left;
    if (pl.Q > sh.qmax) {
        pl.Q = sh.qmax;
        pl.cnt = pl.Q * SB;
    }
    pl.R = pl.cnt - pl.Q * SB;
    pl.chunk = 1;
    if (pl.R) {
        pl.chunk = rounds_chunk(pl.R, lanes, k.tchunk, 4, true, LMAX);
        pl.nunits = pl.R / pl.chunk;
        pl.tail = pl.R - pl.nunits * pl.chunk;
    }
    pl.sib_units = pl.Q * sh.upb;
    pl.sib_blocks = (pl.sib_units + P::WG - 1) / P::WG;
    pl.edge_units = sh.has_edge ? pl.Q : 0;
    pl.edge_blocks = (pl.edge_units + P::WG - 1) / P::WG;
    pl.main_blocks = (pl.nunits + P::WG - 1) / P::WG;
    pl.grid = pl.sib_blocks + pl.edge_blocks + pl.main_blocks + (pl.tail + P::WG - 1) / P::WG;
    return pl;
}

}
}
```

### nice_amd/csrc/kernels.h

```cpp
#pragma once

#include <hip/hip_runtime.h>
#include <stdint.h>

#include <vector>

#include "layout.h"

namespace nice {

struct NumOut {
    uint64_t *n;
    uint32_t *u;
    uint32_t *count;
    uint32_t cap;
};

struct FieldFinish {
    uint64_t *out_mapped;
    uint32_t *done;
    uint64_t seq;
    uint32_t tag;
};

struct DetailedLaunch {
    uint64_t start_lo, start_hi;
    uint64_t count;
    uint32_t base;
    uint32_t cutoff;
    uint64_t *hist;
    uint32_t hist_copies;
    NumOut out;
    FieldFinish fin;
    uint32_t *launches;
    uint32_t *sib;
    uint32_t overlapped;
};

bool fd2_supported(uint32_t base);
hipError_t launch_detailed_fd2(const DetailedLaunch &p, int num_cus, hipStream_t s);
size_t fd2_cuts(uint32_t base, unsigned __int128 *out, size_t cap);
struct BatchUnit {
    uint64_t lo, hi;
    uint32_t lanes, chunk;
    uint32_t row, combo;
};
constexpr size_t kBatchDescBytes = 80;
uint32_t fd2_batch_wg(uint32_t base);
uint32_t fd2_batch_chunk(uint32_t base);
void fd2_batch_plan(uint32_t base, unsigned __int128 start, unsigned __int128 end, uint32_t row,
                    std::vector<BatchUnit> &out);
struct BatchLaunch {
    uint32_t base;
    uint32_t cutoff;
    const BatchUnit *units;
    size_t n_units;
    void *h_desc, *d_desc;
    uint64_t *hist;
    uint32_t ncopies;
    NumOut out;
    uint32_t *launches;
};
hipError_t launch_detailed_fd2_batch(const BatchLaunch &p, hipStream_t s);
void fd2_force_sib_stride(uint32_t L);
bool fd2_window(uint32_t base, uint32_t *w0, uint32_t *w);
hipError_t launch_detailed_finish(uint64_t *hist, uint32_t *count, uint64_t *out_mapped, hipStream_t s);
hipError_t launch_detailed_generic(const DetailedLaunch &p, int num_cus, hipStream_t s);

struct Leaf {
    uint64_t b0_lo, b0_hi;
    uint32_t g0;
    uint32_t count;
};

struct NiceFinish {
    uint32_t *msd_mapped;
    uint32_t *count_mapped;
    uint32_t *msd_counters;
    uint32_t *done;
};

struct NiceonlyLaunch {
    const Leaf *leaves;
    const uint32_t *n_leaves_dev;
    uint32_t n_leaves;
    const uint32_t *residues;
    uint32_t R, M;
    uint32_t base;
    uint32_t in_range;
    uint32_t nice_min;
    NumOut out;
    NiceFinish fin;
};
struct LeafMask {
    uint32_t w[3];
    uint32_t multi;
};
struct SoundLaunch {
    const uint32_t *residues;
    const uint32_t *lowmask;
    LeafMask *leaf_masks;
    unsigned long long *rejected;
    uint32_t fast;
    uint32_t prefix_test;
};
hipError_t launch_niceonly(const NiceonlyLaunch &p, int num_cus, hipStream_t s, const SoundLaunch *snd = nullptr);
struct MsdLaunch;
bool sound_prefix_field(const MsdLaunch &p);

struct MsdNode {
    uint64_t off, size;
};
struct MsdLaunch {
    uint64_t start_lo, start_hi;
    uint64_t end_lo, end_hi;
    uint64_t first;
    uint64_t nchunks;
    uint64_t deal_stride, deal_offset;
    uint64_t chunk;
    uint64_t floor_size;
    MsdNode *q[2];
    uint32_t *counters;
    uint32_t q_cap;
    Leaf *leaves;
    uint32_t leaf_cap;
    const uint32_t *residues;
    const uint32_t *ranks;
    uint32_t R, M;
    uint32_t base;
    uint32_t in_range;
    uint32_t first_batch;
    uint32_t *nice_count;
    uint32_t probe;
};
struct ChunkNode {
    uint32_t off, size;
};
hipError_t launch_msd_device(const MsdLaunch &p, int num_cus, hipStream_t s, ChunkNode *scratch = nullptr,
                             uint32_t cap = 0, uint32_t grid = 0, const SoundLaunch *snd = nullptr);

hipError_t launch_msd_wave(const MsdLaunch &p, const NiceonlyLaunch &c, uint32_t level0, void *scratch,
                           uint32_t grid, int num_cus, hipStream_t s, const SoundLaunch *snd = nullptr);

hipError_t launch_unique_counts(const uint64_t *n_pairs, uint32_t count, uint32_t base,
                                uint32_t *out, hipStream_t s);
hipError_t launch_is_nice(const uint64_t *n_pairs, uint32_t count, uint32_t base,
                          uint32_t *out, hipStream_t s);
hipError_t launch_unique_fast(const uint64_t *n_pairs, uint32_t count, uint32_t base,
                              uint32_t *out, hipStream_t s);
hipError_t launch_cube_count(const uint64_t *n_pairs, uint32_t count, uint32_t base,
                             uint32_t *out, hipStream_t s);

}
```

Before: 539.5 billion numbers/s.

## Add persistent sibling-walk kernel variant with per-wave work stealing for base 40

Adds a persistent twin of the sibling-walk detailed kernel for base 40 (ND=4). It launches about one resident grid of workgroups, and each wave pulls 64-lane sibling batches through a shared-memory atomic counter instead of getting one batch per block. It is used by default only when the launch overlaps another stream and the batch count is large compared with resident waves. The goal is to cut tail imbalance and block launch overhead in large sibling launches. The cost is a new kernel instantiation, caps on launch size, and extra planning logic.

```diff
diff --git a/include/nice_hip.h b/include/nice_hip.h
--- a/include/nice_hip.h
+++ b/include/nice_hip.h
@@ -107,12 +107,14 @@
     uint64_t numbers;
     uint32_t sib_lanes;
     uint32_t sib_stride;
+    uint32_t sib_grid;
 } nice_kernel_stats;
 int nice_last_kernel_stats(nice_ctx *ctx, int device_index, nice_kernel_stats *out);
 int nice_ctx_set_kernel_timing(nice_ctx *ctx, int enable);
 
 uint32_t nice_host_threads(void);
 int nice_debug_force_sib_stride(uint32_t L);
+int nice_debug_force_sib_persistent(uint32_t mode, uint32_t max_workgroups);
 int nice_debug_fd_window(uint32_t base, uint32_t *w0, uint32_t *w);
 int nice_debug_set_near_miss_cutoff(uint32_t base, uint32_t cutoff);
 int nice_debug_set_nice_min(uint32_t base, uint32_t nice_min);
diff --git a/nice_amd/_lib.py b/nice_amd/_lib.py
--- a/nice_amd/_lib.py
+++ b/nice_amd/_lib.py
@@ -37,7 +37,7 @@
     "nice_check_prefix_reject_inrange",
     "nice_process_ranges_detailed", "nice_last_ranges_stats", "nice_cpu_process_ranges_detailed",
     "nice_debug_ranges_plan", "nice_debug_set_near_miss_cutoff", "nice_debug_fd_window",
-    "nice_debug_set_nice_min", "nice_debug_cube_count",
+    "nice_debug_set_nice_min", "nice_debug_cube_count", "nice_debug_force_sib_persistent",
 )
 
 
@@ -74,7 +74,8 @@
 class nice_kernel_stats(ctypes.Structure):
     _fields_ = [("kernel_ms", ctypes.c_double), ("launches", ctypes.c_uint32),
                 ("fd_kernel", ctypes.c_uint32), ("numbers", ctypes.c_uint64),
-                ("sib_lanes", ctypes.c_uint32), ("sib_stride", ctypes.c_uint32)]
+                ("sib_lanes", ctypes.c_uint32), ("sib_stride", ctypes.c_uint32),
+                ("sib_grid", ctypes.c_uint32)]
 
 
 class nice_ranges_stats(ctypes.Structure):
@@ -154,6 +155,7 @@
         "nice_host_threads": ([], u32),
         "nice_debug_cgroup_cpus": ([ctypes.c_char_p, ctypes.c_char_p], u32),
         "nice_debug_force_sib_stride": ([u32], i32),
+        "nice_debug_force_sib_persistent": ([u32, u32], i32),
         "nice_debug_set_near_miss_cutoff": ([u32, u32], i32),
         "nice_debug_fd_window": ([u32, P32, P32], i32),
         "nice_debug_set_nice_min": ([u32, u32], i32),
diff --git a/nice_amd/api.py b/nice_amd/api.py
--- a/nice_amd/api.py
+++ b/nice_amd/api.py
@@ -138,6 +138,7 @@
     numbers: int
     sib_lanes: int = 0
     sib_stride: int = 0
+    sib_grid: int = 0
 
 
 @dataclass
@@ -210,7 +211,8 @@
     def kernel_stats(self, device_index: int = 0) -> KernelStats:
         s = _lib.nice_kernel_stats()
         check(lib().nice_last_kernel_stats(self._h, device_index, s))
-        return KernelStats(s.kernel_ms, s.launches, bool(s.fd_kernel), s.numbers, s.sib_lanes, s.sib_stride)
+        return KernelStats(s.kernel_ms, s.launches, bool(s.fd_kernel), s.numbers, s.sib_lanes, s.sib_stride,
+                           s.sib_grid)
 
     def detailed_raw(self, start: int, end: int, base: int, cap: int = 0):
         hist = self._hist.get(base)
diff --git a/nice_amd/csrc/abi_detailed.cpp b/nice_amd/csrc/abi_detailed.cpp
--- a/nice_amd/csrc/abi_detailed.cpp
+++ b/nice_amd/csrc/abi_detailed.cpp
@@ -98,7 +98,7 @@
     }
     sl.seq++;
     sl.launches = 0;
-    sl.sib[0] = sl.sib[1] = 0;
+    sl.sib[0] = sl.sib[1] = sl.sib[2] = 0;
     if (sl.dirty) HIPCHK(hipMemsetAsync(sl.d_state, 0, kStateBytes, sl.stream));
     sl.dirty = true;
     sl.timed = timing;
@@ -164,6 +164,7 @@
     d.last.launches = sl.launches;
     d.last.sib_lanes = sl.sib[0];
     d.last.sib_stride = sl.sib[1];
+    d.last.sib_grid = sl.sib[2];
     return (uint32_t)sl.h_fin[nice::kFinCount];
 }
 
diff --git a/nice_amd/csrc/abi_hooks.cpp b/nice_amd/csrc/abi_hooks.cpp
--- a/nice_amd/csrc/abi_hooks.cpp
+++ b/nice_amd/csrc/abi_hooks.cpp
@@ -211,6 +211,12 @@
     return NICE_OK;
 }
 
+int nice_debug_force_sib_persistent(uint32_t mode, uint32_t max_workgroups) {
+    if (mode > 2) return fail(NICE_ERR_INVALID, "mode must be 0 (production), 1 (persistent) or 2 (rounds)");
+    nice::fd2_force_sib_persistent(mode, max_workgroups);
+    return NICE_OK;
+}
+
 int nice_debug_fd_window(uint32_t base, uint32_t *w0, uint32_t *w) {
     if (!w0 || !w) return fail(NICE_ERR_INVALID, "null argument");
     if (!nice::fd2_window(base, w0, w)) return fail(NICE_ERR_INVALID, "base has no FD kernel");
diff --git a/nice_amd/csrc/abi_internal.hpp b/nice_amd/csrc/abi_internal.hpp
--- a/nice_amd/csrc/abi_internal.hpp
+++ b/nice_amd/csrc/abi_internal.hpp
@@ -93,7 +93,7 @@
     bool marked = false;
     uint64_t seq = 0;
     uint32_t launches = 0;
-    uint32_t sib[2] = {0, 0};
+    uint32_t sib[3] = {0, 0, 0};
     bool fin_seq = false;
     uint32_t tag = 0;
     uint32_t tag_words = 0;
diff --git a/nice_amd/csrc/fd2_cfg.hpp b/nice_amd/csrc/fd2_cfg.hpp
--- a/nice_amd/csrc/fd2_cfg.hpp
+++ b/nice_amd/csrc/fd2_cfg.hpp
@@ -207,7 +207,11 @@
     }
     static constexpr int LG = LG_ >= 0 ? LG_ : (SIB_ > 1 ? 100 : (MW == 3 && WG >= 1024 ? 8 : 0));
     static constexpr int SIB = SIB_;
+    static constexpr bool SIBPERS = SIB_ > 1 && (VD_ & 131072) != 0;
     static constexpr bool PERS = SIB_ > 1 ? false : PERS_ >= 0 ? PERS_ != 0 : (WG >= 1024 && one_wg_per_cu(BASE, WG));
+    using SibPers = Cfg<BASE_, ND_, NE_, NE2_, PROBE_, WG_, VD_ | 131072, LG_, PERS_, SIB_>;
+    static constexpr bool HAS_SIBPERS =
+        SIB_ > 1 && (VD_ & 131072) == 0 && PROBE_ == 0 && BASE_ == 40 && ND_ == 4 && LG >= 100;
     using NoPers = Cfg<BASE_, ND_, NE_, NE2_, PROBE_, (PERS_ < 0 ? rounds_wg(BASE_) : WG_), VD_, LG_, 0>;
     using NoSib = std::conditional_t<(BASE_ >= 46),
                                      Cfg<BASE_, ND_, NE_, NE2_, PROBE_, big_wg(BASE_), valu_limbs_big(BASE_, ND_, NE_)>,
@@ -216,7 +220,7 @@
     static constexpr bool VDL = ((VD & 256) != 0 || NOTAB) && !LSD;
     static constexpr u32 MAGIC_D = (u32)(((1ull << 32) + ES * BASE - 1) / (ES * BASE));
     static_assert(VD == 0 || (MW >= 2 && split_exact(BASE, ES, MAGIC_D)), "VALU digit split");
-    static_assert(VDC <= NE + 1 - (MW <= 2 ? 1 : 0) && VDS <= ND + 1 && (VD & ~0x1ffff) == 0 &&
+    static_assert(VDC <= NE + 1 - (MW <= 2 ? 1 : 0) && VDS <= ND + 1 && (VD & ~0x3ffff) == 0 &&
                       ((VD & 1024) == 0 || LSDX),
                   "VALU-decoded limbs");
     static constexpr int WPE0 = (163840 / LDS_BYTES) * (WG / 64) / 4;
diff --git a/nice_amd/csrc/fd2_detailed.hip b/nice_amd/csrc/fd2_detailed.hip
--- a/nice_amd/csrc/fd2_detailed.hip
+++ b/nice_amd/csrc/fd2_detailed.hip
@@ -11,6 +11,7 @@
 
 NICE_PROBE_ONLY(u64 *g_stamps = nullptr; u64 g_last_launch[6] = {};)
 std::atomic<uint32_t> g_force_sib_stride{0};
+std::atomic<uint32_t> g_force_sib_pers[2] = {{0}, {0}};
 
 struct Combo {
     int nd, ne, ne2;
@@ -112,6 +113,10 @@
 }
 
 void fd2_force_sib_stride(uint32_t L) { fd2::g_force_sib_stride.store(L, std::memory_order_relaxed); }
+void fd2_force_sib_persistent(uint32_t mode, uint32_t max_workgroups) {
+    fd2::g_force_sib_pers[1].store(max_workgroups, std::memory_order_relaxed);
+    fd2::g_force_sib_pers[0].store(mode, std::memory_order_relaxed);
+}
 
 bool fd2_supported(uint32_t base) {
     switch (base) {
diff --git a/nice_amd/csrc/fd2_kernel.hpp b/nice_amd/csrc/fd2_kernel.hpp
--- a/nice_amd/csrc/fd2_kernel.hpp
+++ b/nice_amd/csrc/fd2_kernel.hpp
@@ -442,6 +442,13 @@
         }                                                                                        \
     } while (0)
 #define FD2_STAMP(a, k) FD2_STAMP_P((a).stamps, k)
+#define FD2_WAVE_STAMP(a)                                                                        \
+    do {                                                                                         \
+        if (kProbes && (a).stamps && (threadIdx.x & 63) == 0 && threadIdx.x < 512 &&             \
+            blockIdx.x < kStampGroups)                                                           \
+            (a).stamps[kStampWords * (u64)blockIdx.x + 20 + (threadIdx.x >> 6)] =                \
+                __builtin_amdgcn_s_memtime();                                                    \
+    } while (0)
 
 struct Fd2Args {
     u64 *stamps;
@@ -848,7 +855,28 @@
     u64 lo, hi;
 };
 template <class P>
+__device__ __forceinline__ u32 *sib_batch_slot() {
+    __shared__ u32 cur[P::WG / 64];
+    return &cur[threadIdx.x >> 6];
+}
+template <class P>
+__device__ __forceinline__ SibUnit sib_unit_at(const Fd2Args &a, u32 b, u32 lane) {
+    const u32 nsb = (a.sib_units + 63) / 64;
+    const bool edge = b >= nsb;
+    const u32 sunit = 64 * (edge ? b - nsb : b) + lane;
+    const u32 upb = edge ? 1u : a.sib_upb;
+    SibUnit u;
+    u.active = sunit < (edge ? a.edge_units : a.sib_units);
+    u.chunk = edge ? a.edge_chunk : a.sib_chunk;
+    const u32 q = sunit / upb, k = sunit - q * upb;
+    u.lo = edge ? a.edge_lo : a.sib_lo;
+    u.hi = edge ? a.edge_hi : a.sib_hi;
+    add_u128(u.lo, u.hi, (u64)q * ((u64)P::SIB * P::B * P::B) + (u64)k * u.chunk);
+    return u;
+}
+template <class P>
 __device__ __forceinline__ SibUnit sib_unit(const Fd2Args &a) {
+    if constexpr (P::SIBPERS) return sib_unit_at<P>(a, *sib_batch_slot<P>(), threadIdx.x & 63);
     const bool edge = blockIdx.x >= a.sib_blocks;
     const u32 sunit = (edge ? blockIdx.x - a.sib_blocks : blockIdx.x) * P::WG + threadIdx.x;
     const u32 upb = edge ? 1u : a.sib_upb;
@@ -1142,7 +1170,45 @@
     u32 probe_acc = 0;
     bool sib_done = false;
     if constexpr (P::SIB > 1) {
-        if (sib_part) {
+        if constexpr (P::SIBPERS) {
+            if (sib_part) {
+                __shared__ u32 sib_next;
+                const u32 G = a.sib_blocks;
+                const u32 nb = (a.sib_units + 63) / 64 + (a.edge_units + 63) / 64;
+                const u32 nk = nb > blockIdx.x ? (nb - blockIdx.x + G - 1) / G : 0;
+                if (tid == 0) sib_next = P::WG / 64;
+                asm volatile("s_waitcnt vmcnt(0)" ::: "memory");
+                __syncthreads();
+                FD2_STAMP(a, 14);
+                u32 k = __builtin_amdgcn_readfirstlane(tid >> 6), taken = 0;
+                while (k < nk) {
+                    const u32 b = blockIdx.x + G * k;
+                    if (lane_id == 0) *sib_batch_slot<P>() = b;
+                    const SibUnit su = sib_unit_at<P>(a, b, lane_id);
+                    if (su.active) {
+                        State<P> sst[P::SIB];
+                        u32 X[P::NX];
+                        init_digits<P>(X, su.lo, su.hi);
+                        init_plain<P>(sst[0], X);
+#pragma unroll
+                        for (int j = 1; j < P::SIB; j++) sib_derive<P>(sst[j], sst[0], X, (u32)j);
+#pragma unroll
+                        for (int j = 0; j < P::SIB; j++) {
+                            init_scale<P>(sst[j]);
+                            sib_park<P>(sst[j], j, smem);
+                        }
+                        walk_sib<P>(sst, smem, a, su.chunk, hbase, hinc, outl, cutoff, out);
+                    }
+                    if (++taken >= a.wave_cap) break;
+                    u32 next = 0;
+                    if (lane_id == 0) next = atomicAdd(&sib_next, 1u);
+                    k = __builtin_amdgcn_readfirstlane(__shfl(next, 0));
+                }
+                FD2_STAMP(a, 15);
+                FD2_WAVE_STAMP(a);
+                sib_done = true;
+            }
+        } else if (sib_part) {
             State<P> sst[P::SIB];
             const SibUnit su = sib_unit<P>(a);
             if (su.active) {
@@ -1159,7 +1225,10 @@
             }
             asm volatile("s_waitcnt vmcnt(0)" ::: "memory");
             __syncthreads();
+            FD2_STAMP(a, 14);
             if (su.active) walk_sib<P>(sst, smem, a, su.chunk, hbase, hinc, outl, cutoff, out);
+            FD2_STAMP(a, 15);
+            FD2_WAVE_STAMP(a);
             sib_done = true;
         }
     }
diff --git a/nice_amd/csrc/fd2_launch.hpp b/nice_amd/csrc/fd2_launch.hpp
--- a/nice_amd/csrc/fd2_launch.hpp
+++ b/nice_amd/csrc/fd2_launch.hpp
@@ -14,6 +14,7 @@
 
 NICE_PROBE_ONLY(extern u64 *g_stamps; extern u64 g_last_launch[6];)
 extern std::atomic<uint32_t> g_force_sib_stride;
+extern std::atomic<uint32_t> g_force_sib_pers[2];
 
 template <class P>
 static hipError_t fd2_tables(hipStream_t s, const uint4 **out) {
@@ -59,6 +60,8 @@
     k.min_chunk = probe_knob("NICE_FD2_MINCHUNK", k.min_chunk);
     k.sib_chunk = probe_knob("NICE_FD2_SIBCHUNK", k.sib_chunk);
     k.sib_rounds = probe_knob("NICE_FD2_SIBROUNDS", k.sib_rounds);
+    k.sib_pers_min = probe_knob("NICE_FD2_SIBPERS_MIN", k.sib_pers_min);
+    k.sib_pers_k = probe_knob("NICE_FD2_SIBPERS_K", k.sib_pers_k);
     return k;
 }
 
@@ -90,6 +93,9 @@
 
 template <class P>
 static hipError_t launch_sib(const DetailedLaunch &p, int num_cus, hipStream_t s);
+template <class K, class P>
+static hipError_t launch_sib_shape(const DetailedLaunch &p, const SibShape &sh, const uint4 *tabs,
+                                   const PlanKnobs<P> &knobs, int num_cus, int per_cu, hipStream_t s);
 
 template <class P>
 static hipError_t launch_cfg(const DetailedLaunch &p, int num_cus, hipStream_t s) {
@@ -157,21 +163,42 @@
     const uint4 *tabs = nullptr;
     hipError_t e = fd2_tables<P>(s, &tabs);
     if (e != hipSuccess) return e;
-    const PlanKnobs<P> knobs = fd2_knobs<P>();
+    PlanKnobs<P> knobs = fd2_knobs<P>();
+    if constexpr (P::HAS_SIBPERS) {
+        knobs.sib_pers_mode = g_force_sib_pers[0].load(std::memory_order_relaxed);
+        knobs.sib_pers_max_wg = g_force_sib_pers[1].load(std::memory_order_relaxed);
+    }
     const u128 seg_start = ((u128)p.start_hi << 64) | p.start_lo;
-    const SibShape sh = plan_sib<P>(seg_start, p.count, num_cus, per_cu, p.overlapped != 0,
-                                    g_force_sib_stride.load(std::memory_order_relaxed), knobs);
+    SibShape sh = plan_sib<P>(seg_start, p.count, num_cus, per_cu, p.overlapped != 0,
+                              g_force_sib_stride.load(std::memory_order_relaxed), knobs);
     if (sh.kind == SibShape::kNoSib) return launch_cfg<typename P::NoSib>(p, num_cus, s);
     if (sh.kind == SibShape::kError) return hipErrorInvalidValue;
     if (p.sib) {
         p.sib[0] = (uint32_t)P::SIB;
         p.sib[1] = (uint32_t)sh.L;
-    }
+        p.sib[2] = 0;
+    }
+    if constexpr (P::HAS_SIBPERS) {
+        const int pq = fd2_occupancy<typename P::SibPers>();
+        if (pq >= 1) {
+            plan_sib_pers<P>(sh, p.count, num_cus, pq, p.overlapped != 0, knobs);
+            if (sh.pers) return launch_sib_shape<typename P::SibPers, P>(p, sh, tabs, knobs, num_cus, pq, s);
+        }
+    }
+    return launch_sib_shape<P, P>(p, sh, tabs, knobs, num_cus, per_cu, s);
+}
+
+template <class K, class P>
+static hipError_t launch_sib_shape(const DetailedLaunch &p, const SibShape &sh, const uint4 *tabs,
+                                   const PlanKnobs<P> &knobs, int num_cus, int per_cu, hipStream_t s) {
+    static_assert(K::SIBPERS || std::is_same<K, P>::value, "the rounds kernel or its persistent twin");
     constexpr u64 SB = (u64)P::SIB * P::B * P::B;
+    hipError_t e;
     DetailedLaunch q = p;
     u64 left = p.count;
     while (left) {
         const SibLaunchPlan pl = plan_sib_launch<P>(left, sh, num_cus, per_cu, knobs);
+        if (K::SIBPERS && p.sib && pl.sib_blocks) p.sib[2] = (uint32_t)pl.sib_blocks;
         Fd2Args a{};
         a.sib_lo = a.edge_lo = q.start_lo;
         a.sib_hi = a.edge_hi = q.start_hi;
@@ -186,12 +213,12 @@
         u64 lo = q.start_lo, hi = q.start_hi;
         add_u128(lo, hi, pl.Q * SB);
         fd2_regular_parts(a, lo, hi, pl.nunits, pl.chunk, pl.tail, pl.main_blocks);
-        a.wave_cap = 0;
+        a.wave_cap = pl.wave_cap;
         NICE_PROBE_ONLY({
             const u64 v[6] = {pl.grid, (u64)P::WG, sh.L, pl.sib_units, pl.R, (u64)per_cu};
             for (int k = 0; k < 6; k++) g_last_launch[k] = v[k];
         })
-        if ((e = fd2_enqueue<P>(a, q, tabs, left == pl.cnt, pl.grid, s)) != hipSuccess) return e;
+        if ((e = fd2_enqueue<K>(a, q, tabs, left == pl.cnt, pl.grid, s)) != hipSuccess) return e;
         add_u128(q.start_lo, q.start_hi, pl.cnt);
         left -= pl.cnt;
     }
diff --git a/nice_amd/csrc/fd2_plan.hpp b/nice_amd/csrc/fd2_plan.hpp
--- a/nice_amd/csrc/fd2_plan.hpp
+++ b/nice_amd/csrc/fd2_plan.hpp
@@ -143,6 +143,9 @@
     u64 min_chunk = 4;
     u64 sib_chunk = 0;
     u64 sib_rounds = 15;
+    u64 sib_pers_min = 40;
+    u64 sib_pers_k = 1;
+    u32 sib_pers_mode = 0, sib_pers_max_wg = 0;
 };
 
 static inline u64 rounds_chunk(u64 cnt, u64 lanes, u64 tchunk, u64 floor, bool odd, u64 cap) {
@@ -215,6 +218,9 @@
     u64 U, upb, r;
     bool has_edge;
     u64 qmax;
+    bool pers;
+    u64 pers_grid;
+    u32 wave_cap;
 };
 template <class P>
 static bool sib_too_short(u64 count) {
@@ -235,7 +241,7 @@
         double rounds = 0;
         L = pick_small_stride<P>(seg_start, count, P::TCHUNK * 3 / 4, P::TCHUNK * 5 / 4, P::LO + 1, Q0, lanes, D,
                                  rounds);
-        if (10 * rounds < (double)k.sib_rounds) return sh;
+        if (10 * rounds < (double)k.sib_rounds && k.sib_pers_mode != 1) return sh;
     }
     constexpr u64 T = P::LG >= 100 ? 140 : (u64)P::TCHUNK;
     if (!L && P::LG >= 100 && !overlapped) {
@@ -265,17 +271,47 @@
     u64 Q, cnt, R;
     u64 chunk, nunits, tail;
     u64 sib_units, sib_blocks, edge_units, edge_blocks, main_blocks, grid;
-};
+    u64 batches;
+    u32 wave_cap;
+};
+
+template <class P>
+static void plan_sib_pers(SibShape &sh, u64 count, int num_cus, int per_cu, bool overlapped,
+                          const PlanKnobs<P> &k = PlanKnobs<P>{}) {
+    constexpr u64 SB = (u64)P::SIB * P::B * P::B, NW = P::WG / 64;
+    sh.pers = false;
+    sh.pers_grid = 0;
+    sh.wave_cap = 0;
+    if (sh.kind != SibShape::kSib || k.sib_pers_mode == 2) return;
+    const u64 resident = (u64)num_cus * per_cu, Q = count / SB;
+    const u64 nb = (Q * sh.upb + 63) / 64 + (sh.has_edge ? (Q + 63) / 64 : 0);
+    if (k.sib_pers_mode != 1 && (!overlapped || 10 * nb < k.sib_pers_min * resident * NW)) return;
+    u64 G = resident * std::max<u64>(1, k.sib_pers_k);
+    if (k.sib_pers_mode == 1 && k.sib_pers_max_wg) G = std::min<u64>(G, k.sib_pers_max_wg);
+    const u64 cap = 65535 / ((u64)P::SIB * sh.L);
+    if (cap < 1 || (sh.upb + 63) / 64 + 1 > G * NW * cap) return;
+    sh.pers = true;
+    sh.pers_grid = G;
+    sh.wave_cap = (u32)cap;
+}
+
 template <class P>
 static SibLaunchPlan plan_sib_launch(u64 left, const SibShape &sh, int num_cus, int per_cu,
                                      const PlanKnobs<P> &k = PlanKnobs<P>{}) {
-    constexpr u64 SB = (u64)P::SIB * P::B * P::B, LMAX = (u64)P::LDE - P::B;
+    constexpr u64 SB = (u64)P::SIB * P::B * P::B, LMAX = (u64)P::LDE - P::B, NW = P::WG / 64;
     const u64 lanes = (u64)num_cus * per_cu * P::WG;
     SibLaunchPlan pl{};
     pl.Q = left / SB;
     pl.cnt = left;
-    if (pl.Q > sh.qmax) {
-        pl.Q = sh.qmax;
+    u64 qmax = sh.qmax;
+    if (sh.pers) {
+        const u64 room = sh.pers_grid * NW * sh.wave_cap;
+        const u64 per = sh.upb + (sh.has_edge ? 1 : 0);
+        qmax = std::min<u64>(qmax, std::max<u64>(1, room > 2 ? (room - 2) * 64 / per : 0));
+        qmax = std::min<u64>(qmax, std::max<u64>(1, 0xffffffc0ull / sh.upb));
+    }
+    if (pl.Q > qmax) {
+        pl.Q = qmax;
         pl.cnt = pl.Q * SB;
     }
     pl.R = pl.cnt - pl.Q * SB;
@@ -289,6 +325,12 @@
     pl.sib_blocks = (pl.sib_units + P::WG - 1) / P::WG;
     pl.edge_units = sh.has_edge ? pl.Q : 0;
     pl.edge_blocks = (pl.edge_units + P::WG - 1) / P::WG;
+    if (sh.pers) {
+        pl.batches = (pl.sib_units + 63) / 64 + (pl.edge_units + 63) / 64;
+        pl.sib_blocks = std::min<u64>(sh.pers_grid, (pl.batches + NW - 1) / NW);
+        pl.edge_blocks = 0;
+        pl.wave_cap = sh.wave_cap;
+    }
     pl.main_blocks = (pl.nunits + P::WG - 1) / P::WG;
     pl.grid = pl.sib_blocks + pl.edge_blocks + pl.main_blocks + (pl.tail + P::WG - 1) / P::WG;
     return pl;
diff --git a/nice_amd/csrc/kernels.h b/nice_amd/csrc/kernels.h
--- a/nice_amd/csrc/kernels.h
+++ b/nice_amd/csrc/kernels.h
@@ -63,6 +63,7 @@
 };
 hipError_t launch_detailed_fd2_batch(const BatchLaunch &p, hipStream_t s);
 void fd2_force_sib_stride(uint32_t L);
+void fd2_force_sib_persistent(uint32_t mode, uint32_t max_workgroups);
 bool fd2_window(uint32_t base, uint32_t *w0, uint32_t *w);
 hipError_t launch_detailed_finish(uint64_t *hist, uint32_t *count, uint64_t *out_mapped, hipStream_t s);
 hipError_t launch_detailed_generic(const DetailedLaunch &p, int num_cus, hipStream_t s);
```

New measurement: 555.7 billion numbers/s (median of 6 runs). +3.0%, better.
